# AIBluefisher/DReg-NeRF

Measured on AMD Instinct MI355X. Metric: nerf_pairs_per_sec_regtr_fwd_bwd_128, higher is better.
Workload: dtype bf16; 1 GPU; RegTR fwd+bwd+AdamW, shell-R synthetic pairs, 128^3 grids, 4 pairs (8 grids) per GPU per step, random-init weights; global_batch_pairs=4, resolution=128, fpn_head=active-set (identical results; rows around occupied voxels), parallelism=dp1

## Files before the change

### dreg_nerf_amd/csrc/executor.hip

```cpp
#include <hip/hip_runtime.h>
#include <cstdint>
#include <cstring>
#include <algorithm>
#include <vector>
#include <string>
#include <cstdio>
#include "../../include/dreg_nerf.h"
#ifndef DREG_ELAUNCH
#define DREG_ELAUNCH (-2)
#endif

namespace {

enum { OP_CONV = 0, OP_BN = 1, OP_MAXPOOL = 2, OP_CONV_ROWS = 3 };
constexpr int OP_INTS = 16;
constexpr int TENSOR_INTS = 5;
constexpr int RL = 8;
constexpr int PARAM_I64 = 5;

struct Tensor { int B, D, H, W, C; size_t bytes, off, goff; };
struct Param {
    float* val; float* grad; int d0, d1, ksz;
    size_t pk_fwd = SIZE_MAX, pk_dgrad = SIZE_MAX, pk_cls = SIZE_MAX;
    size_t pk_halo_fwd = SIZE_MAX, pk_halo_dgrad = SIZE_MAX;
    size_t pk_brick_fwd = SIZE_MAX, pk_brick_dgrad = SIZE_MAX;
    int cin_pad = 0;
};
struct Op {
    int kind, in, out, in2, w, b, p2, p3, p4, ksz, stride, pad, relu, add_same, rows_out, rows_in;
    size_t aux0 = 0, aux1 = 0;
    size_t wg_off = 0, wg_bytes = 0;
    int rd = -1;
    int ds_rows = -1;
    int sparse_gx = 0;
    size_t cl_off = 0;
    int cl_count = 0;
    int ds_sparse = 0;
    size_t cl2_off = 0;
    int cl2_count = 0;
    int pool = -1;
    int sstem = 0;
    int sstem_conv = -1, sstem_lat = -1;
    size_t xam_off = 0, pmask_off = 0;
    int halo = 0;
    int stats_bn = -1;
    size_t stats_off = 0;
    int stats_conv = -1;
    int grp = 0;
    int fold_sk_fwd = 0, fold_sk_bwd = 0;
    int fold_into = -1, res_from = -1;
    int bt = -1;
    size_t keep_var = 0, keep_sums = 0;
};
struct HaloPack { const float* w; size_t off; int Cout, Cin, transposed, brick; };
struct PackRec { const float* w; void* out; int Cout, Cin_real, inner, ntaps, for_dgrad, Kpad, dtype, row0; };
static_assert(sizeof(PackRec) == 48, "matches PackDesc of conv.hip");

struct ReduceRec { const float* part; float* dw; int nsplit, Cout, Kpad, ntaps, Cin, Cin_real, accumulate, block0; };
static_assert(sizeof(ReduceRec) == 48, "matches WgradReduceDesc of conv.hip");

struct BnTailRec { const float* a; const float* b; float* o0; float* o1; int B, V, C, block0; };
static_assert(sizeof(BnTailRec) == 48, "matches BnTailDesc of fpn_ops.hip");

struct TimedLaunch { hipEvent_t e0, e1; int op, kind, variant; };

struct Exec {
    std::vector<Tensor> t;
    std::vector<Op> ops;
    std::vector<Param> prm;
    std::vector<char> needs_grad;
    size_t act_bytes = 0, arena_bytes = 0, pack_bytes = 0;
    size_t off_bn_ws = 0, off_coef = 0, off_ks = 0, off_rd = 0, off_cs = 0, off_tmp = 0;
    size_t sz_ks = 0;
    std::vector<ReduceRec> reduce;
    const void* sparse_arena = nullptr;
    std::vector<ReduceRec> reduce_abs;
    int reduce_blocks = 0;
    const void* reduce_arena = nullptr;
    std::vector<BnTailRec> bn_fwd, bn_bwd;
    size_t off_bnf = 0, off_bnb = 0;
    int bn_blocks = 0;
    std::vector<PackRec> packs;
    std::vector<HaloPack> halo_packs;
    int pack_rows = 0, pack_max_floats = 0;
    int out_slot = -1;
    bool timing = false;
    std::vector<TimedLaunch> timed;
    size_t timed_used = 0;
    hipStream_t aux = nullptr;
    std::vector<hipEvent_t> ev;
    hipEvent_t ev_done = nullptr;
    bool use_aux = true;
    const uint8_t* in_rowocc = nullptr;
    char* pack_base = nullptr;
    std::vector<char> written;
    bool aux_used = false;
    struct GrpLaunch { size_t off; int n, variant, blocks; };
    std::vector<int> grp_ops;
    std::vector<GrpLaunch> grp_launch;
    size_t off_grp = 0;
    bool grp_ready = false;
    int pend_sk_bn = -1, pend_sk_n = 0;
    size_t pend_sk_slice = 0;
    const void* fwd_rows_arena = nullptr;
    struct Band { size_t off; const char* tag; int idx; };
    std::vector<Band> bands;
    size_t off_guard_tab = 0, off_guard_res = 0;
    const void* guard_arena = nullptr;
    int guard_op = -1, guard_pass = 0; long long guard_band = -1;
    dreg_exec_opts opt;
};

inline size_t align256(size_t v) { return (v + 255) / 256 * 256; }
constexpr size_t GUARD_BYTES = 64 * 1024;
struct Bump {
    size_t v = 0;
    std::vector<Exec::Band>* bands = nullptr;
    const char* tag = "?"; int idx = -1;
    operator size_t() const { return v; }
    Bump& operator+=(size_t n) { v += n; if (bands && n) { bands->push_back(Exec::Band{v, tag, idx}); v += GUARD_BYTES; } return *this; }
    void name(const char* t, int i) { tag = t; idx = i; }
};
inline int out_dim(int i, int k, int s, int p) { return (i + 2 * p - k) / s + 1; }

struct Scope {
    Exec* e; hipStream_t st; TimedLaunch* tl = nullptr;
    Scope(Exec* ex, hipStream_t s, int op, int kind) : e(ex), st(s) {
        if (!e->timing) return;
        if (e->timed_used == e->timed.size()) {
            TimedLaunch n{}; n.op = op; n.kind = kind;
            if (hipEventCreate(&n.e0) != hipSuccess || hipEventCreate(&n.e1) != hipSuccess) return;
            e->timed.push_back(n);
        }
        tl = &e->timed[e->timed_used++];
        tl->op = op; tl->kind = kind; tl->variant = 0;
        (void)hipEventRecord(tl->e0, st);
    }
    ~Scope() { if (tl) (void)hipEventRecord(tl->e1, st); }
    void variant(int v) { if (tl) tl->variant = v; }
};

#define CK(expr) do { int rc_ = (expr); if (rc_) return rc_; } while (0)

bool s2_class_ok(const Param& p, int ksz, int stride, int pad)
{
    return stride == 2 && ((ksz == 3 && pad == 1) || (ksz == 1 && pad == 0)) && p.d0 % 64 == 0 && p.d1 % 64 == 0 && dreg_conv_get_glds();
}

}

extern "C" {

void dreg_exec_default_opts(dreg_exec_opts* o)
{
    std::memset(o, 0, sizeof(*o));
    o->sparse_grads = 1; o->bn_batch_tails = 1; o->fuse_stem = 1; o->sparse_stem = 1; o->fold_res_bn = 1; o->fold_splitk = 1;
    o->group_wgrad = 1; o->s2_accumulate = 1; o->fuse_bn_stats = 1; o->brick = 1; o->defer_head_pg = 0;
}
void* dreg_exec_create(const int* tensors, int nt, const int* ops, int nops, const int64_t* params, int np)
{
    return dreg_exec_create_opts(tensors, nt, ops, nops, params, np, nullptr);
}
void* dreg_exec_create_opts(const int* tensors, int nt, const int* ops, int nops, const int64_t* params, int np, const dreg_exec_opts* opts)
{
    Exec* e = new Exec();
    if (opts) e->opt = *opts; else dreg_exec_default_opts(&e->opt);
    e->opt.brick &= 3;
    const int g_sparse_grads = e->opt.sparse_grads, g_bn_batch_tails = e->opt.bn_batch_tails, g_fuse_stem = e->opt.fuse_stem, g_sparse_stem = e->opt.sparse_stem,
              g_fold_res_bn = e->opt.fold_res_bn, g_fold_splitk = e->opt.fold_splitk, g_group_wgrad = e->opt.group_wgrad, g_fuse_bn_stats = e->opt.fuse_bn_stats,
              g_brick = e->opt.brick;
    e->t.resize(nt);
    for (int i = 0; i < nt; ++i) {
        Tensor& t = e->t[i];
        t.B = tensors[i * TENSOR_INTS]; t.D = tensors[i * TENSOR_INTS + 1]; t.H = tensors[i * TENSOR_INTS + 2];
        t.W = tensors[i * TENSOR_INTS + 3]; t.C = tensors[i * TENSOR_INTS + 4];
        t.bytes = align256((size_t)t.B * t.D * t.H * t.W * t.C * 2);
    }
    e->prm.resize(np);
    for (int i = 0; i < np; ++i) {
        Param& p = e->prm[i];
        p.val = (float*)params[i * PARAM_I64]; p.grad = (float*)params[i * PARAM_I64 + 1];
        p.d0 = (int)params[i * PARAM_I64 + 2]; p.d1 = (int)params[i * PARAM_I64 + 3]; p.ksz = (int)params[i * PARAM_I64 + 4];
    }
    e->ops.resize(nops);
    for (int i = 0; i < nops; ++i) {
        const int* r = ops + i * OP_INTS;
        Op& o = e->ops[i];
        o.kind = r[0]; o.in = r[1]; o.out = r[2]; o.in2 = r[3]; o.w = r[4]; o.b = r[5]; o.p2 = r[6]; o.p3 = r[7]; o.p4 = r[8];
        o.ksz = r[9]; o.stride = r[10]; o.pad = r[11]; o.relu = r[12]; o.add_same = r[13]; o.rows_out = r[14]; o.rows_in = r[15];
        if (o.in < 0 || o.in >= nt || o.out <= 0 || o.out >= nt || o.in2 >= nt) { delete e; return nullptr; }
    }
    e->out_slot = nops ? e->ops.back().out : -1;

    e->needs_grad.assign(nt, 0);
    for (const Op& o : e->ops) {
        bool g = e->needs_grad[o.in] || (o.in2 >= 0 && e->needs_grad[o.in2]);
        if (o.kind == OP_CONV || o.kind == OP_CONV_ROWS) g = g || e->prm[o.w].grad || (o.b >= 0 && e->prm[o.b].grad);
        if (o.kind == OP_BN) g = g || e->prm[o.w].grad || e->prm[o.b].grad;
        e->needs_grad[o.out] = g;
    }

    for (size_t i = 0; i + 1 < e->ops.size(); ++i) {
        Op& o = e->ops[i];
        if (o.kind != OP_BN || o.in2 >= 0 || o.out == e->out_slot) continue;
        int users = 0, pool = -1;
        for (size_t j = 0; j < e->ops.size(); ++j) {
            const Op& q = e->ops[j];
            if (q.in == o.out || q.in2 == o.out) { ++users; if (q.kind == OP_MAXPOOL && q.in == o.out && j > i) pool = (int)j; }
        }
        if (users == 1 && pool >= 0 && e->t[o.out].C % 8 == 0 && g_fuse_stem) { o.pool = pool; e->ops[pool].pool = (int)i; }
        if (o.pool < 0 && pool >= 0 && o.relu && e->t[o.out].C % 8 == 0 && g_sparse_stem && g_fuse_stem) {
            int prod = -1, writers = 0, lat = -1, others = 0;
            for (size_t j = 0; j < e->ops.size(); ++j) {
                const Op& q = e->ops[j];
                if (q.out == o.in) { prod = (int)j; ++writers; }
                if ((int)j == pool) continue;
                if (q.in2 == o.out) ++others;
                else if (q.in == o.out) { if (q.kind == OP_CONV_ROWS && q.rows_in >= 0 && lat < 0) lat = (int)j; else ++others; }
            }
            if (writers == 1 && others == 0 && e->ops[prod].kind == OP_CONV && e->ops[prod].rows_out >= 0 && o.b >= 0) {
                o.pool = pool; e->ops[pool].pool = (int)i; o.sstem = 1; o.sstem_conv = prod; o.sstem_lat = lat;
            }
        }
    }

    if (g_fold_res_bn)
        for (size_t j = 0; j < e->ops.size(); ++j) {
            Op& bj = e->ops[j];
            const Tensor& xj = e->t[bj.in];
            if (bj.kind != OP_BN || bj.in2 >= 0 || bj.relu || bj.pool >= 0 || bj.out == e->out_slot || dreg_bn_small(xj.B, xj.D * xj.H * xj.W, xj.C, 0)) continue;
            int users = 0, k = -1;
            for (size_t q = 0; q < e->ops.size(); ++q) {
                const Op& o = e->ops[q];
                if (o.in == bj.out) ++users;
                if (o.in2 == bj.out) { ++users; if (o.kind == OP_BN && q > j && o.pool < 0) k = (int)q; }
            }
            if (users != 1 || k < 0 || e->ops[k].res_from >= 0) continue;
            bj.fold_into = k; e->ops[k].res_from = (int)j;
        }

    if (g_fold_splitk)
        for (size_t i = 0; i < e->ops.size(); ++i) {
            Op& o = e->ops[i];
            if (o.kind != OP_CONV || o.b >= 0 || o.in2 >= 0 || o.relu || o.rows_out >= 0) continue;
            auto users = [&](int slot) { int u = 0; for (const Op& q : e->ops) u += (q.in == slot) + (q.in2 == slot); return u; };
            const Tensor& y = e->t[o.out];
            if (i + 1 < e->ops.size() && o.out != e->out_slot) {
                const Op& bn = e->ops[i + 1];
                if (bn.kind == OP_BN && bn.in == o.out && bn.pool < 0 && users(o.out) == 1 && dreg_bn_small_in_regs(y.B, y.D * y.H * y.W, y.C, 0)) o.fold_sk_fwd = 1;
            }
            const Tensor& x = e->t[o.in];
            if (i >= 1 && o.in != 0) {
                const Op& bn = e->ops[i - 1];
                if (bn.kind == OP_BN && bn.out == o.in && bn.pool < 0 && users(o.in) == 1 && dreg_bn_small_in_regs(x.B, x.D * x.H * x.W, x.C, 0) && o.stride == 1) o.fold_sk_bwd = 1;
            }
        }

    Bump off;
    if (e->opt.guard) { off.bands = &e->bands; off.name("arena start", 0); off += 256; }
    for (int i = 1; i < nt; ++i) { off.name("activation", i); e->t[i].off = off; off += e->t[i].bytes; }
    size_t max_tensor = 0, bn_ws = 0, coef = 0, cs = 0;
    for (Op& o : e->ops) {
        const Tensor& x = e->t[o.in];
        off.name(o.kind == OP_BN ? "BatchNorm statistics / stem scratch of op" : (o.kind == OP_MAXPOOL ? "max-pool argmax of op" : "conv op"), (int)(&o - e->ops.data()));
        if (o.kind == OP_BN) {
            const size_t sb = align256((size_t)x.B * x.C * 2 * sizeof(float));
            o.aux0 = off; off += sb; o.aux1 = off; off += sb;
            const size_t V = (size_t)x.D * x.H * x.W;
            size_t w = (size_t)x.B * dreg_bn_num_chunks((int)V) * x.C * 2 * sizeof(float);
            if (o.sstem) {
                const Tensor& p = e->t[e->ops[o.pool].out];
                const size_t w2 = dreg_sparse_stem_workspace_floats(p.B, p.D, p.H, p.W, p.C) * sizeof(float);
                if (w2 > w) w = w2;
                o.xam_off = off; off += align256((size_t)p.B * p.D * p.H * p.W * p.C * 2);
                o.pmask_off = off; off += align256((size_t)p.B * p.D * p.H * p.W);
            }
            if (w > bn_ws) bn_ws = w;
            if (sb > coef) coef = sb;
            bool shared = false;
            for (const Op& q : e->ops) shared = shared || (&q != &o && q.kind == OP_BN && (q.w == o.w || q.b == o.b || q.p2 == o.p2 || q.p3 == o.p3));
            if (g_bn_batch_tails && o.pool < 0 && !shared && dreg_bn_small(x.B, (int)V, x.C, 0)) {
                o.keep_var = off; off += align256((size_t)x.B * x.C * sizeof(float));
                o.keep_sums = off; off += sb;
                BnTailRec f{}, b{};
                f.a = (const float*)o.aux1; f.b = (const float*)o.keep_var; f.o0 = e->prm[o.p2].val; f.o1 = e->prm[o.p3].val;
                b.a = (const float*)o.keep_sums; b.b = nullptr; b.o0 = e->prm[o.w].grad; b.o1 = e->prm[o.b].grad;
                f.B = b.B = x.B; f.V = b.V = (int)V; f.C = b.C = x.C; f.block0 = b.block0 = e->bn_blocks;
                e->bn_blocks += (x.C + 255) / 256;
                o.bt = (int)e->bn_fwd.size();
                e->bn_fwd.push_back(f); e->bn_bwd.push_back(b);
            }
        } else if (o.kind == OP_MAXPOOL) {
            const Tensor& y = e->t[o.out];
            o.aux0 = off; off += align256((size_t)y.B * y.D * y.H * y.W * y.C);
        } else {
            const Param& w = e->prm[o.w];
            const Tensor& y = e->t[o.out];
            const size_t k1 = dreg_conv3d_igemm_workspace_bytes(x.B, x.D, x.H, x.W, x.C, y.D, y.H, y.W, w.d0, o.ksz, o.stride, o.pad, 0, o.in2 >= 0, 0);
            const size_t k2 = dreg_conv3d_igemm_workspace_bytes(x.B, y.D, y.H, y.W, w.d0, x.D, x.H, x.W, w.d1, o.ksz, o.stride, o.pad, 1, 0, 0);
            if (k1 > e->sz_ks) e->sz_ks = k1;
            if (k2 > e->sz_ks) e->sz_ks = k2;
            if (w.grad) {
                o.wg_bytes = dreg_conv3d_wgrad_workspace_bytes(x.B, y.D, y.H, y.W, x.C, w.d0, o.ksz, 0);
                bool shared = false;
                for (const ReduceRec& q : e->reduce) shared = shared || q.dw == w.grad;
                if (shared) o.rd = -2;
                else {
                    ReduceRec r{};
                    r.dw = w.grad; r.nsplit = dreg_conv3d_wgrad_splits(x.B, y.D, y.H, y.W, x.C, w.d0, o.ksz, 0);
                    r.Cout = w.d0; r.Kpad = dreg_conv3d_kpad(o.ksz, x.C, 0); r.ntaps = o.ksz * o.ksz * o.ksz; r.Cin = x.C; r.Cin_real = w.d1;
                    r.accumulate = (o.kind == OP_CONV_ROWS || o.rows_out >= 0) ? 3 : 1;
                    r.block0 = e->reduce_blocks;
                    e->reduce_blocks += dreg_wgrad_reduce_blocks(w.d0, w.d1, o.ksz, r.nsplit);
                    o.rd = (int)e->reduce.size();
                    e->reduce.push_back(r);
                }
            }
            const size_t c = dreg_colsum_workspace_bytes((size_t)y.B * y.D * y.H * y.W, w.d0);
            if (c > cs) cs = c;
        }
    }
    if (g_fuse_bn_stats) {
        for (size_t j = 0; j < e->ops.size(); ++j) {
            Op& bn = e->ops[j];
            if (bn.kind != OP_BN || bn.pool >= 0) continue;
            const Tensor& x = e->t[bn.in];
            const int V = x.D * x.H * x.W;
            if (V % 128 != 0 || dreg_bn_small(x.B, V, x.C, 0)) continue;
            int prod = -1, writers = 0;
            for (size_t i = 0; i < j; ++i) if (e->ops[i].out == bn.in) { prod = (int)i; ++writers; }
            if (writers != 1 || e->ops[prod].kind != OP_CONV || e->ops[prod].stats_bn >= 0) continue;
            {
                const Op& pc = e->ops[prod];
                const Tensor& px = e->t[pc.in];
                const Param& pp = e->prm[pc.w];
                if (!pc.relu && pp.d1 == px.C && pp.d0 != 64 && dreg_conv3_halo_use(px.B, px.D, px.H, px.W, px.C, pp.d0, pc.ksz, pc.stride, pc.pad)) continue;
            }
            e->ops[prod].stats_bn = (int)j;
            bn.stats_conv = prod;
            off.name("epilogue chunk sums of BatchNorm op", (int)j);
            bn.stats_off = off; off += align256((size_t)x.B * (V / 128) * x.C * 2 * sizeof(float));
        }
    }
    e->act_bytes = off;
    for (int i = 1; i < nt; ++i) {
        if (e->t[i].bytes > max_tensor) max_tensor = e->t[i].bytes;
        off.name("gradient of activation", i);
        if (e->needs_grad[i] && i != e->out_slot) { e->t[i].goff = off; off += e->t[i].bytes; } else e->t[i].goff = SIZE_MAX;
    }
    for (Op& o : e->ops) {
        if (o.kind != OP_CONV_ROWS || o.in2 < 0 || o.add_same || !e->needs_grad[o.in2] || !g_sparse_grads) continue;
        for (const Op& q : e->ops) if (q.out == o.in2 && q.kind == OP_CONV_ROWS) o.ds_rows = q.rows_out;
    }
    for (Op& o : e->ops) {
        if (o.kind != OP_CONV_ROWS || !e->needs_grad[o.in] || o.in == 0 || e->t[o.in].goff == SIZE_MAX) continue;
        int writers = 0;
        for (const Op& q : e->ops) {
            if (q.kind == OP_MAXPOOL && q.pool >= 0 && e->ops[q.pool].sstem) continue;
            if ((q.in == o.in || q.in2 == o.in) && e->needs_grad[q.out]) ++writers;
        }
        if (writers != 1 || !g_sparse_grads) continue;
        const Tensor& x = e->t[o.in];
        off.name("row-list copy (sparse_gx) of op", (int)(&o - e->ops.data()));
        o.sparse_gx = 1; o.cl_off = off; off += align256((size_t)x.B * x.D * x.H * x.W * sizeof(int));
    }
    for (Op& o : e->ops) {
        if (o.kind != OP_CONV_ROWS || o.ds_rows < 0 || e->t[o.in2].goff == SIZE_MAX || !g_sparse_grads) continue;
        int writers = 0;
        for (const Op& q : e->ops) if ((q.in == o.in2 || q.in2 == o.in2) && e->needs_grad[q.out]) ++writers;
        if (writers != 1) continue;
        const Tensor& ta = e->t[o.in2];
        off.name("row-list copy (ds_sparse) of op", (int)(&o - e->ops.data()));
        o.ds_sparse = 1; o.cl2_off = off; off += align256((size_t)ta.B * ta.D * ta.H * ta.W * sizeof(int));
    }
    for (Op& o : e->ops) {
        if (o.kind != OP_CONV || o.rows_out < 0) continue;
        const Tensor& y = e->t[o.out];
        off.name("row-list copy (stem output) of op", (int)(&o - e->ops.data()));
        o.cl_off = off; off += align256((size_t)y.B * y.D * y.H * y.W * sizeof(int));
    }
    off.name("BatchNorm workspace", 0);
    e->off_bn_ws = off; off += align256(bn_ws);
    off.name("BatchNorm coefficients", 0);
    e->off_coef = off; off += align256(coef);
    off.name("split-K workspace", 0);
    e->off_ks = off; off += align256(e->sz_ks);
    for (Op& o : e->ops) if (o.rd != -1) { off.name("weight-gradient partials of op", (int)(&o - e->ops.data())); o.wg_off = off; off += align256(o.wg_bytes); if (o.rd >= 0) e->reduce[o.rd].part = (const float*)o.wg_off; }
    if (g_group_wgrad)
        for (size_t i = 0; i < e->ops.size(); ++i) {
            Op& o = e->ops[i];
            const Tensor& y = e->t[o.out];
            if (o.kind != OP_CONV || o.rd < 0 || o.rows_out >= 0 || o.in == 0 || o.b >= 0 || o.out == e->out_slot || !e->prm[o.w].grad) continue;
            if ((long)y.D * y.H * y.W > 4096) continue;
            o.grp = 1; e->grp_ops.push_back((int)i);
        }
    if (e->grp_ops.size() < 4) { for (int i : e->grp_ops) e->ops[i].grp = 0; e->grp_ops.clear(); }
    off.name("descriptor tables", 0);
    e->off_grp = off; off += align256(e->grp_ops.size() * (size_t)dreg_wgrad_group_desc_bytes() + 16);
    e->off_rd = off; off += align256(e->reduce.size() * sizeof(ReduceRec) + 16);
    e->off_bnf = off; off += align256(e->bn_fwd.size() * sizeof(BnTailRec) + 16);
    e->off_bnb = off; off += align256(e->bn_bwd.size() * sizeof(BnTailRec) + 16);
    off.name("column-sum workspace", 0);
    e->off_cs = off; off += align256(cs);
    off.name("gradient temporary", 0);
    e->off_tmp = off; off += max_tensor;
    if (e->opt.guard) {
        off.bands = nullptr;
        e->off_guard_tab = off; off += align256((e->bands.size() + 1) * sizeof(unsigned long long));
        e->off_guard_res = off; off += 256;
    }
    e->arena_bytes = off + 256;

    size_t poff = 0;
    auto add_pack = [&](Param& p, int kind, int cin_pad) {
        PackRec r{};
        const int ntaps = p.ksz * p.ksz * p.ksz;
        r.w = p.val; r.Cout = p.d0; r.Cin_real = p.d1; r.ntaps = ntaps; r.for_dgrad = kind; r.dtype = 0; r.row0 = e->pack_rows;
        int rows;
        if (kind == 0) { r.inner = cin_pad; r.Kpad = dreg_conv3d_kpad(p.ksz, cin_pad, 0); rows = p.d0; }
        else if (kind == 1) { r.inner = p.d0; r.Kpad = dreg_conv3d_kpad(p.ksz, p.d0, 0); rows = p.d1; }
        else { r.inner = p.d0; r.Kpad = dreg_conv3d_kpad(p.ksz == 1 ? 1 : 2, p.d0, 0); rows = (p.ksz == 1 ? 1 : 8) * p.d1; }
        r.out = (void*)poff;
        const size_t o = poff;
        poff += align256((size_t)rows * r.Kpad * 2);
        e->pack_rows += rows;
        const int ch = kind ? p.d0 : p.d1;
        const int fl = ntaps > 1 ? (ch < 64 ? ch : 64) * ntaps : 0;
        if (fl > e->pack_max_floats) e->pack_max_floats = fl;
        e->packs.push_back(r);
        return o;
    };
    auto add_halo_pack = [&](Param& p, int transposed) {
        HaloPack hp{p.val, poff, p.d0, p.d1, transposed, 0};
        poff += align256(dreg_conv3_halo_pack_bytes_n(transposed ? p.d0 : p.d1, transposed ? p.d1 : p.d0));
        e->halo_packs.push_back(hp);
        return hp.off;
    };
    auto add_brick_pack = [&](Param& p, int transposed) {
        HaloPack hp{p.val, poff, p.d0, p.d1, transposed, 1};
        poff += align256(dreg_conv3_brick_pack_bytes(transposed ? p.d1 : p.d0, transposed ? p.d0 : p.d1));
        e->halo_packs.push_back(hp);
        return hp.off;
    };
    for (Op& o : e->ops) {
        if (o.kind != OP_CONV && o.kind != OP_CONV_ROWS) continue;
        Param& p = e->prm[o.w];
        const Tensor& x = e->t[o.in];
        const Tensor& y = e->t[o.out];
        if (o.kind == OP_CONV && !o.relu) {
            if (dreg_conv3_halo_use(x.B, x.D, x.H, x.W, x.C, p.d0, o.ksz, o.stride, o.pad) && p.d1 == x.C) o.halo |= 1;
            if (e->needs_grad[o.in] && dreg_conv3_halo_use(y.B, y.D, y.H, y.W, p.d0, p.d1, o.ksz, o.stride, o.pad) && p.d0 % 32 == 0) o.halo |= 2;
        }
        if (o.kind == OP_CONV_ROWS && o.ksz == 3 && o.pad == 1 && p.d1 == x.C && dreg_brick_supported(x.B, x.D, x.H, x.W, 16, 256)) {
            auto on = [&](int nout) { return (nout == 64 && (g_brick & 1)) || (nout == 256 && (g_brick & 2)); };
            if (on(p.d0) && p.d1 % 16 == 0 && p.pk_brick_fwd == SIZE_MAX) p.pk_brick_fwd = add_brick_pack(p, 0);
            if (e->needs_grad[o.in] && on(p.d1) && p.d0 % 16 == 0 && p.pk_brick_dgrad == SIZE_MAX) p.pk_brick_dgrad = add_brick_pack(p, 1);
        }
        if (o.halo & 1) { if (p.pk_halo_fwd == SIZE_MAX) p.pk_halo_fwd = add_halo_pack(p, 0); }
        else if (p.pk_fwd == SIZE_MAX) { p.cin_pad = x.C; p.pk_fwd = add_pack(p, 0, x.C); }
        if (e->needs_grad[o.in]) {
            if (o.halo & 2) { if (p.pk_halo_dgrad == SIZE_MAX) p.pk_halo_dgrad = add_halo_pack(p, 1); }
            else if (o.kind == OP_CONV && s2_class_ok(p, o.ksz, o.stride, o.pad)) { if (p.pk_cls == SIZE_MAX) p.pk_cls = add_pack(p, 2, x.C); }
            else if (p.pk_dgrad == SIZE_MAX) p.pk_dgrad = add_pack(p, 1, x.C);
        }
    }
    e->pack_bytes = poff + 256;
    return e;
}

void dreg_exec_destroy(void* h)
{
    Exec* e = (Exec*)h;
    if (!e) return;
    for (auto& t : e->timed) { (void)hipEventDestroy(t.e0); (void)hipEventDestroy(t.e1); }
    for (auto& v : e->ev) if (v) (void)hipEventDestroy(v);
    if (e->ev_done) (void)hipEventDestroy(e->ev_done);
    delete e;
}

size_t dreg_exec_arena_bytes(void* h) { return ((Exec*)h)->arena_bytes; }
size_t dreg_exec_pack_bytes(void* h) { return ((Exec*)h)->pack_bytes; }
int dreg_exec_num_packs(void* h) { return (int)((Exec*)h)->packs.size(); }
size_t dreg_exec_tensor_offset(void* h, int slot) { return ((Exec*)h)->t[slot].off; }
int dreg_exec_output_slot(void* h) { return ((Exec*)h)->out_slot; }

int dreg_exec_pack_rows(void* h) { return ((Exec*)h)->pack_rows; }
int dreg_exec_export_pack_table(void* h, void* host_out, int* host_row_desc, void* pack_base)
{
    Exec* e = (Exec*)h;
    e->pack_base = (char*)pack_base;
    PackRec* o = (PackRec*)host_out;
    for (size_t i = 0; i < e->packs.size(); ++i) {
        o[i] = e->packs[i]; o[i].out = (char*)pack_base + (size_t)e->packs[i].out;
        const int end = i + 1 < e->packs.size() ? e->packs[i + 1].row0 : e->pack_rows;
        for (int r = e->packs[i].row0; r < end; ++r) host_row_desc[r] = (int)i;
    }
    return DREG_OK;
}
int dreg_exec_repack(void* h, const void* descs_dev, const int* row_desc_dev, void* stream)
{
    Exec* e = (Exec*)h;
    CK(dreg_pack_conv_weights_batched(descs_dev, (int)e->packs.size(), e->pack_rows, e->pack_max_floats, row_desc_dev, stream));
    for (const HaloPack& hp : e->halo_packs) {
        if (hp.brick) CK(dreg_pack_conv_weight_brick(hp.w, e->pack_base + hp.off, hp.Cout, hp.Cin, hp.transposed, stream));
        else CK(dreg_pack_conv_weight_halo(hp.w, e->pack_base + hp.off, hp.Cout, hp.Cin, hp.transposed, stream));
    }
    return DREG_OK;
}
int dreg_exec_op_halo(void* h, int op) { Exec* e = (Exec*)h; return op >= 0 && op < (int)e->ops.size() ? e->ops[op].halo : 0; }

void dreg_exec_set_overlap(void* h, int enable) { ((Exec*)h)->use_aux = enable != 0; }
void dreg_exec_set_input_row_occupancy(void* h, const uint8_t* rowocc) { ((Exec*)h)->in_rowocc = rowocc; }
void dreg_exec_set_timing(void* h, int enable) { ((Exec*)h)->timing = enable != 0; }
int dreg_exec_read_timings(void* h, int* op_kind, float* ms, int max)
{
    Exec* e = (Exec*)h;
    int n = 0;
    for (size_t i = 0; i < e->timed_used && n < max; ++i) {
        float v = 0.f;
        if (hipEventElapsedTime(&v, e->timed[i].e0, e->timed[i].e1) != hipSuccess) continue;
        op_kind[3 * n] = e->timed[i].op; op_kind[3 * n + 1] = e->timed[i].kind; op_kind[3 * n + 2] = e->timed[i].variant; ms[n] = v; ++n;
    }
    e->timed_used = 0;
    return n;
}

static int guard_setup(Exec* e, char* A, hipStream_t st)
{
    if (!e->opt.guard || e->guard_arena == (const void*)A) return DREG_OK;
    std::vector<unsigned long long> offs(e->bands.size());
    for (size_t i = 0; i < offs.size(); ++i) offs[i] = e->bands[i].off;
    if (!offs.empty() && hipMemcpyAsync(A + e->off_guard_tab, offs.data(), offs.size() * sizeof(unsigned long long), hipMemcpyHostToDevice, st) != hipSuccess) return DREG_ELAUNCH;
    if (hipStreamSynchronize(st) != hipSuccess) return DREG_ELAUNCH;
    int rc = dreg_guard_fill(A, A + e->off_guard_tab, (int)offs.size(), (int)GUARD_BYTES, (void*)st);
    if (rc) return rc;
    e->guard_arena = A;
    return DREG_OK;
}
static int guard_scan(Exec* e, char* A, long long* out4, hipStream_t st)
{
    int rc = dreg_guard_scan(A, A + e->off_guard_tab, (int)e->bands.size(), (int)GUARD_BYTES, A + e->off_guard_res, (void*)st);
    if (rc) return rc;
    if (hipMemcpyAsync(out4, A + e->off_guard_res, 4 * sizeof(long long), hipMemcpyDeviceToHost, st) != hipSuccess) return DREG_ELAUNCH;
    if (hipStreamSynchronize(st) != hipSuccess) return DREG_ELAUNCH;
    return DREG_OK;
}
static int guard_after_op(Exec* e, char* A, int op, int pass, hipStream_t st, hipStream_t aux)
{
    if (e->opt.guard < 2) return DREG_OK;
    if (aux && hipStreamSynchronize(aux) != hipSuccess) return DREG_ELAUNCH;
    long long r[4];
    int rc = guard_scan(e, A, r, st);
    if (rc) return rc;
    if (r[0] > 0) { e->guard_op = op; e->guard_pass = pass; e->guard_band = r[1]; return DREG_EGUARD; }
    return DREG_OK;
}
static int upload_tables(Exec* e, char* A, hipStream_t st)
{
    { int rc = guard_setup(e, A, st); if (rc) return rc; }
    if (e->reduce_arena == (const void*)A) return DREG_OK;
    e->reduce_abs = e->reduce;
    for (ReduceRec& r : e->reduce_abs) r.part = (const float*)(A + (size_t)r.part);
    std::vector<BnTailRec> f = e->bn_fwd, b = e->bn_bwd;
    for (BnTailRec& r : f) { r.a = (const float*)(A + (size_t)r.a); r.b = (const float*)(A + (size_t)r.b); }
    for (BnTailRec& r : b) r.a = (const float*)(A + (size_t)r.a);
    if (!e->reduce_abs.empty() && hipMemcpyAsync(A + e->off_rd, e->reduce_abs.data(), e->reduce_abs.size() * sizeof(ReduceRec), hipMemcpyHostToDevice, st) != hipSuccess) return DREG_ELAUNCH;
    if (!f.empty() && (hipMemcpyAsync(A + e->off_bnf, f.data(), f.size() * sizeof(BnTailRec), hipMemcpyHostToDevice, st) != hipSuccess ||
                       hipMemcpyAsync(A + e->off_bnb, b.data(), b.size() * sizeof(BnTailRec), hipMemcpyHostToDevice, st) != hipSuccess)) return DREG_ELAUNCH;
    const int gd = dreg_wgrad_group_desc_bytes();
    struct Rec { std::vector<char> d; int variant, nblocks, op; };
    std::vector<Rec> recs;
    e->grp_launch.clear(); e->grp_ready = false;
    bool all_ok = !e->grp_ops.empty();
    for (int i : e->grp_ops) {
        const Op& o = e->ops[i];
        const Tensor& x = e->t[o.in];
        const Tensor& y = e->t[o.out];
        const Param& w = e->prm[o.w];
        Rec r; r.d.resize(gd); r.op = i;
        if (e->t[o.out].goff == SIZE_MAX ||
            dreg_conv3d_wgrad_group_fill(r.d.data(), A + y.goff, A + x.off, A + o.wg_off, o.wg_bytes, x.B, x.D, x.H, x.W, x.C, y.D, y.H, y.W, w.d0,
                                         o.ksz, o.stride, o.pad, &r.variant, &r.nblocks) != DREG_OK || w.d1 != x.C) { all_ok = false; break; }
        recs.push_back(std::move(r));
    }
    std::vector<char> gtab;
    if (all_ok) {
        std::stable_sort(recs.begin(), recs.end(), [](const Rec& a, const Rec& b) { return a.variant < b.variant; });
        gtab.resize(recs.size() * (size_t)gd);
        for (size_t k = 0; k < recs.size(); ++k) {
            if (e->grp_launch.empty() || e->grp_launch.back().variant != recs[k].variant) e->grp_launch.push_back(Exec::GrpLaunch{e->off_grp + k * (size_t)gd, 0, recs[k].variant, 0});
            const int b0 = e->grp_launch.back().blocks;
            std::memcpy(recs[k].d.data() + gd - (int)sizeof(int), &b0, sizeof(int));
            std::memcpy(gtab.data() + k * (size_t)gd, recs[k].d.data(), (size_t)gd);
            e->grp_launch.back().n += 1; e->grp_launch.back().blocks += recs[k].nblocks;
        }
        if (hipMemcpyAsync(A + e->off_grp, gtab.data(), gtab.size(), hipMemcpyHostToDevice, st) != hipSuccess) return DREG_ELAUNCH;
        e->grp_ready = true;
    }
    if (hipStreamSynchronize(st) != hipSuccess) return DREG_ELAUNCH;
    e->reduce_arena = A;
    return DREG_OK;
}
static int flush_bn_tails(Exec* e, char* A, std::vector<char>& done, int what, hipStream_t st)
{
    for (int lo = 0, nrec = (int)done.size(); lo < nrec;) {
        if (!done[lo]) { ++lo; continue; }
        int hi = lo;
        while (hi + 1 < nrec && done[hi + 1]) ++hi;
        Scope sc(e, st, -1, 4 + what);
        const int b0 = e->bn_fwd[lo].block0;
        const int b1 = hi + 1 < nrec ? e->bn_fwd[hi + 1].block0 : e->bn_blocks;
        if (what == 0) CK(dreg_bn_running_update_batched((const BnTailRec*)(A + e->off_bnf) + lo, hi - lo + 1, b0, b1 - b0, 0.1f, (void*)st));
        else CK(dreg_bn_param_grad_batched((const BnTailRec*)(A + e->off_bnb) + lo, hi - lo + 1, b0, b1 - b0, 1, (void*)st));
        for (int q = lo; q <= hi; ++q) done[q] = 0;
        lo = hi + 1;
    }
    return DREG_OK;
}

int dreg_exec_forward(void* h, void* arena, size_t arena_bytes, const void* pack_base, const void* x_in,
                      const int64_t* rowlists, int nlists, int train, void* stream)
{
    Exec* e = (Exec*)h;
    if (arena_bytes < e->arena_bytes) return DREG_EINVAL;
    char* A = (char*)arena;
    const char* PK = (const char*)pack_base;
    hipStream_t st = (hipStream_t)stream;
    CK(upload_tables(e, (char*)arena, st));
    std::vector<char> bn_done(e->bn_fwd.size(), 0);
    std::vector<int> sums_rpc(e->ops.size(), 0);
    int fwd_sk_bn = -1, fwd_sk_n = 0;
    size_t fwd_sk_slice = 0;
    struct ArenaMark { Exec* e; const void* a; bool ok = false;
                       ~ArenaMark() { if (ok) e->fwd_rows_arena = a; else { e->fwd_rows_arena = nullptr; for (Op& o : e->ops) if (o.kind == OP_CONV && o.rows_out >= 0) o.cl_count = 0; } } } arena_mark{e, arena};
    auto act = [&](int s) -> void* { return s == 0 ? (void*)x_in : (void*)(A + e->t[s].off); };
    for (size_t i = 0; i < e->ops.size(); ++i) {
        if (i > 0) CK(guard_after_op(e, A, (int)i - 1, 0, st, nullptr));
        const Op& o = e->ops[i];
        const Tensor& x = e->t[o.in];
        const Tensor& y = e->t[o.out];
        if (o.kind == OP_CONV) {
            const Param& w = e->prm[o.w];
            const float* bias = o.b >= 0 ? e->prm[o.b].val : nullptr;
            const void* add = o.in2 >= 0 ? act(o.in2) : nullptr;
            const Tensor* ta = o.in2 >= 0 ? &e->t[o.in2] : nullptr;
            if (o.rows_out >= 0) {
                if (o.rows_out >= nlists || bias || add) return DREG_EINVAL;
                const int64_t* rl = rowlists + RL * o.rows_out;
                const int* r = (const int*)rl[0];
                const int n = (int)rl[1];
                Op& om = const_cast<Op&>(o);
                if (e->fwd_rows_arena != arena) CK(dreg_fill_zero(act(o.out), y.bytes, stream));
                else if (om.cl_count > 0) CK(dreg_zero_rows(act(o.out), (const int*)(A + o.cl_off), om.cl_count, y.C, 0, stream));
                if (n > 0 && hipMemcpyAsync(A + o.cl_off, r, (size_t)n * sizeof(int), hipMemcpyDeviceToDevice, st) != hipSuccess) return DREG_ELAUNCH;
                om.cl_count = n;
                if (n > 0) {
                    Scope sc(e, st, (int)i, 0);
                    CK(dreg_conv3d_igemm_rows(act(o.in), PK + w.pk_fwd, act(o.out), nullptr, nullptr, r, n, x.B, x.D, x.H, x.W, x.C, y.D, y.H, y.W, w.d0,
                                              o.ksz, o.stride, o.pad, 0, o.relu, 0, 0, 0, 0, 0, stream));
                }
                continue;
            }
            Scope sc(e, st, (int)i, 0);
            if (o.halo & 1) {
                if (train && o.stats_bn >= 0)
                    CK(dreg_conv3_halo_n_bnstats(act(o.in), PK + w.pk_halo_fwd, act(o.out), bias, add, x.B, x.D, x.H, x.W, x.C, w.d0, ta ? ta->D : 0, ta ? ta->H : 0,
                                                 ta ? ta->W : 0, o.add_same, (float*)(A + e->ops[o.stats_bn].stats_off), &sums_rpc[o.stats_bn], stream));
                else
                    CK(dreg_conv3_halo_n(act(o.in), PK + w.pk_halo_fwd, act(o.out), bias, add, x.B, x.D, x.H, x.W, x.C, w.d0, ta ? ta->D : 0, ta ? ta->H : 0, ta ? ta->W : 0,
                                         o.add_same, 0, stream));
                continue;
            }
            if (train && o.stats_bn >= 0 && !(o.in == 0 && e->in_rowocc)) {
                CK(dreg_conv3d_igemm_bnstats(act(o.in), PK + w.pk_fwd, act(o.out), bias, add, x.B, x.D, x.H, x.W, x.C, y.D, y.H, y.W, w.d0,
                                             o.ksz, o.stride, o.pad, o.relu, ta ? ta->D : 0, ta ? ta->H : 0, ta ? ta->W : 0, o.add_same,
                                             A + e->off_ks, e->sz_ks, (float*)(A + e->ops[o.stats_bn].stats_off), &sums_rpc[o.stats_bn], stream));
                continue;
            }
            if (train && o.fold_sk_fwd && !(o.halo & 1)) {
                int ns = 0; size_t sl = 0;
                CK(dreg_conv3d_igemm_defer(act(o.in), PK + w.pk_fwd, act(o.out), bias, add, x.B, x.D, x.H, x.W, x.C, y.D, y.H, y.W, w.d0,
                                           o.ksz, o.stride, o.pad, 0, o.relu, ta ? ta->D : 0, ta ? ta->H : 0, ta ? ta->W : 0, o.add_same,
                                           A + e->off_ks, e->sz_ks, o.in == 0 ? e->in_rowocc : nullptr, &ns, &sl, stream));
                if (ns > 0) { fwd_sk_bn = (int)i + 1; fwd_sk_n = ns; fwd_sk_slice = sl; }
                continue;
            }
            CK(dreg_conv3d_igemm_occ(act(o.in), PK + w.pk_fwd, act(o.out), bias, add, x.B, x.D, x.H, x.W, x.C, y.D, y.H, y.W, w.d0,
                                     o.ksz, o.stride, o.pad, 0, o.relu, ta ? ta->D : 0, ta ? ta->H : 0, ta ? ta->W : 0, o.add_same, 0, 0,
                                     A + e->off_ks, e->sz_ks, o.in == 0 ? e->in_rowocc : nullptr, stream));
        } else if (o.kind == OP_CONV_ROWS) {
            const Param& w = e->prm[o.w];
            if (o.rows_out < 0 || o.rows_out >= nlists) return DREG_EINVAL;
            const float* bias = o.b >= 0 ? e->prm[o.b].val : nullptr;
            const void* add = o.in2 >= 0 ? act(o.in2) : nullptr;
            const Tensor* ta = o.in2 >= 0 ? &e->t[o.in2] : nullptr;
            Scope sc(e, st, (int)i, 0);
            const int64_t* rl = rowlists + RL * o.rows_out;
            if ((e->opt.brick & (w.d0 == 64 ? 1 : 2)) && w.pk_brick_fwd != SIZE_MAX && rl[2] && rl[3] > 0) {
                sc.variant(2);
                CK(dreg_conv3_brick(act(o.in), PK + w.pk_brick_fwd, act(o.out), bias, add, (const void*)rl[2], (int)rl[3], (const int*)rl[4], (const void*)rl[5],
                                    (const int*)rl[6], x.B, x.D, x.H, x.W, x.C, w.d0, ta ? ta->D : 0, ta ? ta->H : 0, ta ? ta->W : 0, 0, 0, stream));
                continue;
            }
            CK(dreg_conv3d_igemm_rows(act(o.in), PK + w.pk_fwd, act(o.out), bias, add, (const int*)rl[0], (int)rl[1],
                                      x.B, x.D, x.H, x.W, x.C, y.D, y.H, y.W, w.d0, o.ksz, 1, o.pad, 0, 0, ta ? ta->D : 0, ta ? ta->H : 0, ta ? ta->W : 0,
                                      0, 0, stream));
        } else if (o.kind == OP_BN && o.pool >= 0 && o.sstem) {
            const Op& q = e->ops[o.pool];
            const Tensor& p = e->t[q.out];
            const Op& cv = e->ops[o.sstem_conv];
            if (cv.rows_out >= nlists) return DREG_EINVAL;
            const int64_t* rl = rowlists + RL * cv.rows_out;
            const int* ra = nullptr; int na = 0;
            if (o.sstem_lat >= 0) {
                const int li = e->ops[o.sstem_lat].rows_in;
                if (li < 0 || li >= nlists) return DREG_EINVAL;
                ra = (const int*)rowlists[RL * li]; na = (int)rowlists[RL * li + 1];
            }
            CK(dreg_sparse_stem_fwd(act(o.in), (const int*)rl[0], (int)rl[1], ra, na, act(o.out), act(q.out), (uint8_t*)(A + q.aux0), A + o.xam_off, (uint8_t*)(A + o.pmask_off),
                                    e->prm[o.w].val, e->prm[o.b].val, e->prm[o.p2].val, e->prm[o.p3].val, (float*)(A + o.aux0), (float*)(A + o.aux1),
                                    (float*)(A + e->off_bn_ws), x.B, x.D, x.H, x.W, p.D, p.H, p.W, x.C, 1e-5f, 0.1f, train, o.relu, stream));
        } else if (o.kind == OP_BN && o.pool >= 0) {
            const Op& q = e->ops[o.pool];
            const Tensor& p = e->t[q.out];
            CK(dreg_bn_relu_maxpool_fwd(act(o.in), act(q.out), (uint8_t*)(A + q.aux0), e->prm[o.w].val, e->prm[o.b].val, e->prm[o.p2].val, e->prm[o.p3].val,
                                        (float*)(A + o.aux0), (float*)(A + o.aux1), (float*)(A + e->off_bn_ws), x.B, x.D, x.H, x.W, p.D, p.H, p.W, x.C,
                                        1e-5f, 0.1f, train, o.relu, stream));
        } else if (o.kind == OP_MAXPOOL && o.pool >= 0) {
        } else if (o.kind == OP_BN) {
            const int V = x.D * x.H * x.W;
            const void* res_p = o.in2 >= 0 ? act(o.in2) : nullptr;
            void* out_p = o.fold_into >= 0 ? nullptr : act(o.out);
            dreg_bn_extra ex{};
            if (o.res_from >= 0) { res_p = act(e->ops[o.res_from].in); ex.res_scale_shift = (const float*)(A + e->ops[o.res_from].aux0); }
            if (train && sums_rpc[i] > 0) {
                CK(dreg_bn3d_fwd_ex(act(o.in), res_p, out_p, e->prm[o.w].val, e->prm[o.b].val, e->prm[o.p2].val, e->prm[o.p3].val,
                                    (float*)(A + o.aux0), (float*)(A + o.aux1), (float*)(A + o.stats_off), x.B, V, x.C, 1e-5f, 0.1f, 1, o.relu, 0,
                                    nullptr, nullptr, sums_rpc[i], &ex, stream));
                continue;
            }
            int deferred = 0;
            if (fwd_sk_bn == (int)i) { ex.splitk_part = (const float*)(A + e->off_ks); ex.splitk_nsplit = fwd_sk_n; ex.splitk_slice = fwd_sk_slice; fwd_sk_bn = -1; }
            CK(dreg_bn3d_fwd_ex(act(o.in), res_p, out_p, e->prm[o.w].val, e->prm[o.b].val, e->prm[o.p2].val, e->prm[o.p3].val,
                                (float*)(A + o.aux0), (float*)(A + o.aux1), (float*)(A + e->off_bn_ws), x.B, V, x.C, 1e-5f, 0.1f, train, o.relu, 0,
                                o.bt >= 0 ? (float*)(A + o.keep_var) : nullptr, &deferred, 0, &ex, stream));
            if (deferred) bn_done[o.bt] = 1;
        } else if (o.kind == OP_MAXPOOL) {
            CK(dreg_maxpool3d_fwd(act(o.in), act(o.out), (uint8_t*)(A + o.aux0), x.B, x.D, x.H, x.W, y.D, y.H, y.W, x.C, 0, stream));
        } else return DREG_EINVAL;
    }
    CK(guard_after_op(e, A, (int)e->ops.size() - 1, 0, st, nullptr));
    CK(flush_bn_tails(e, A, bn_done, 0, st));
    CK(guard_after_op(e, A, (int)e->ops.size(), 0, st, nullptr));
    arena_mark.ok = true;
    return DREG_OK;
}
int dreg_exec_guard_bands(void* h) { return (int)((Exec*)h)->bands.size(); }
int dreg_exec_guard_check(void* h, void* arena, long long* out4, void* stream)
{
    Exec* e = (Exec*)h;
    if (!e->opt.guard || !out4) return DREG_EINVAL;
    if (e->guard_arena != arena) { out4[0] = 0; out4[1] = (long long)e->bands.size(); out4[2] = 0; out4[3] = 0; return DREG_OK; }
    return guard_scan(e, (char*)arena, out4, (hipStream_t)stream);
}
int dreg_exec_guard_describe(void* h, int band, char* buf, int buf_bytes)
{
    Exec* e = (Exec*)h;
    if (band < 0 || band >= (int)e->bands.size() || !buf || buf_bytes <= 0) return DREG_EINVAL;
    const Exec::Band& b = e->bands[band];
    std::snprintf(buf, (size_t)buf_bytes, "band %d at arena offset %zu, behind: %s %d", band, b.off, b.tag, b.idx);
    return DREG_OK;
}
int dreg_exec_guard_last(void* h, int* op, int* pass, long long* band)
{
    Exec* e = (Exec*)h;
    if (op) *op = e->guard_op;
    if (pass) *pass = e->guard_pass;
    if (band) *band = e->guard_band;
    return DREG_OK;
}

int dreg_exec_backward_range(void* h, void* arena, size_t arena_bytes, const void* pack_base, const void* x_in, const void* grad_out,
                             const int64_t* rowlists, int nlists, void* stream, void* aux_stream, int op_begin, int op_end, int flags);
int dreg_exec_backward(void* h, void* arena, size_t arena_bytes, const void* pack_base, const void* x_in, const void* grad_out,
                       const int64_t* rowlists, int nlists, void* stream, void* aux_stream)
{
    return dreg_exec_backward_range(h, arena, arena_bytes, pack_base, x_in, grad_out, rowlists, nlists, stream, aux_stream,
                                    0, (int)((Exec*)h)->ops.size(), 3);
}
int dreg_exec_backward_range(void* h, void* arena, size_t arena_bytes, const void* pack_base, const void* x_in, const void* grad_out,
                             const int64_t* rowlists, int nlists, void* stream, void* aux_stream, int op_begin, int op_end, int flags)
{
    Exec* e = (Exec*)h;
    if (arena_bytes < e->arena_bytes || op_begin < 0 || op_end > (int)e->ops.size() || op_begin > op_end) return DREG_EINVAL;
    char* A = (char*)arena;
    const char* PK = (const char*)pack_base;
    hipStream_t st = (hipStream_t)stream;
    auto act = [&](int s) -> void* { return s == 0 ? (void*)x_in : (void*)(A + e->t[s].off); };
    if (flags & 1) { e->written.assign(e->t.size(), 0); e->aux_used = false; e->pend_sk_bn = -1; }
    if (e->written.size() != e->t.size()) return DREG_EINVAL;
    std::vector<char>& written = e->written;
    auto grad = [&](int s) -> void* { return s == e->out_slot ? (void*)grad_out : (void*)(A + e->t[s].goff); };
    auto dst_for = [&](int s) -> void* { return written[s] ? (void*)(A + e->off_tmp) : grad(s); };
    auto commit = [&](int s) -> int {
        if (written[s]) {
            const Tensor& t = e->t[s];
            return dreg_add_inplace(grad(s), A + e->off_tmp, (size_t)t.B * t.D * t.H * t.W * t.C, 0, stream);
        }
        written[s] = 1;
        return DREG_OK;
    };
    written[e->out_slot] = 1;
    bool aux_on = e->use_aux && aux_stream != nullptr && aux_stream != stream;
    e->aux = (hipStream_t)aux_stream;
    if (aux_on && e->ev.empty()) {
        e->ev.assign(e->ops.size(), nullptr);
        if (hipEventCreateWithFlags(&e->ev_done, hipEventDisableTiming) != hipSuccess) aux_on = false;
    }
    bool& aux_used = e->aux_used;
    CK(upload_tables(e, A, st));
    std::vector<char> bn_done(e->bn_bwd.size(), 0);
    if (flags & 1) {
        const bool fresh = e->sparse_arena != arena;
        for (Op& o : e->ops) {
            if (!o.sparse_gx) continue;
            const Tensor& x = e->t[o.in];
            if (fresh) { if (hipMemsetAsync(A + x.goff, 0, (size_t)x.B * x.D * x.H * x.W * x.C * 2, st) != hipSuccess) return DREG_ELAUNCH; }
            else if (o.cl_count > 0) CK(dreg_zero_rows(A + x.goff, (const int*)(A + o.cl_off), o.cl_count, x.C, 0, stream));
            o.cl_count = 0;
        }
        for (Op& o : e->ops) {
            if (!o.ds_sparse) continue;
            const Tensor& ta = e->t[o.in2];
            if (fresh) { if (hipMemsetAsync(A + ta.goff, 0, (size_t)ta.B * ta.D * ta.H * ta.W * ta.C * 2, st) != hipSuccess) return DREG_ELAUNCH; }
            else if (o.cl2_count > 0) CK(dreg_zero_rows(A + ta.goff, (const int*)(A + o.cl2_off), o.cl2_count, ta.C, 0, stream));
            o.cl2_count = 0;
        }
        e->sparse_arena = arena;
    }
    const int g_s2_accumulate = e->opt.s2_accumulate, g_group_wgrad = e->opt.group_wgrad, g_brick = e->opt.brick, g_defer_head_pg = e->opt.defer_head_pg;
    std::vector<char> rd_done(e->reduce.size(), 0);
    hipStream_t rd_stream = st;
    size_t rd_pending = 0;
    auto flush_reduce = [&]() -> int {
        for (int lo = 0, nrec = (int)rd_done.size(); lo < nrec;) {
            if (!rd_done[lo]) { ++lo; continue; }
            int hi = lo;
            while (hi + 1 < nrec && rd_done[hi + 1]) ++hi;
            Scope sc(e, rd_stream, -1, 3);
            const int b0 = e->reduce[lo].block0;
            const int b1 = hi + 1 < nrec ? e->reduce[hi + 1].block0 : e->reduce_blocks;
            CK(dreg_wgrad_reduce_batched((const ReduceRec*)(A + e->off_rd) + lo, hi - lo + 1, b0, b1 - b0, (void*)rd_stream));
            for (int q = lo; q <= hi; ++q) rd_done[q] = 0;
            lo = hi + 1;
        }
        return DREG_OK;
    };
    const bool grp_active = g_group_wgrad && e->grp_ready && aux_on && !e->timing && op_begin == 0 && op_end == (int)e->ops.size() && (flags & 3) == 3;
    std::vector<int> grp_seen;
    auto param_grads = [&](int i, bool event_recorded) -> int {
        const Op& o = e->ops[i];
        const Tensor& x = e->t[o.in];
        const Tensor& y = e->t[o.out];
        const Param& w = e->prm[o.w];
        const void* gy = grad(o.out);
        const bool rows = o.kind == OP_CONV_ROWS;
        const bool lrows = rows || (o.kind == OP_CONV && o.rows_out >= 0 && o.rows_out < nlists);
        const int* r_out = lrows ? (const int*)rowlists[RL * o.rows_out] : nullptr;
        const int n_out = lrows ? (int)rowlists[RL * o.rows_out + 1] : 0;
        hipStream_t ws = st;
        if (aux_on && !(grp_active && o.grp && !(o.b >= 0 && e->prm[o.b].grad))) {
            if (!e->ev[i] && hipEventCreateWithFlags(&e->ev[i], hipEventDisableTiming) != hipSuccess) return DREG_ELAUNCH;
            if (!event_recorded && hipEventRecord(e->ev[i], st) != hipSuccess) return DREG_ELAUNCH;
            if (hipStreamWaitEvent(e->aux, e->ev[i], 0) != hipSuccess) return DREG_ELAUNCH;
            ws = e->aux;
            aux_used = true;
        }
        hipStream_t bs = ws;
        bool flush_now = false;
        if (w.grad && grp_active && o.grp) {
            grp_seen.push_back(i);
        } else
        if (w.grad) {
            Scope sc(e, ws, i, 2);
            if (o.rd >= 0) {
                CK(dreg_conv3d_wgrad_partials(gy, act(o.in), A + o.wg_off, o.wg_bytes, lrows ? r_out : nullptr, n_out, x.B, x.D, x.H, x.W, x.C, w.d1,
                                              y.D, y.H, y.W, w.d0, o.ksz, rows ? 1 : o.stride, o.pad, (!lrows && o.in == 0) ? e->in_rowocc : nullptr, (void*)ws));
                rd_done[o.rd] = 1;
                rd_stream = ws;
                rd_pending += o.wg_bytes;
                flush_now = rd_pending >= ((size_t)192 << 20);
            } else if (lrows) {
                CK(dreg_conv3d_wgrad_rows(gy, act(o.in), w.grad, A + o.wg_off, o.wg_bytes, r_out, n_out, x.B, x.D, x.H, x.W, x.C, w.d1,
                                          y.D, y.H, y.W, w.d0, o.ksz, rows ? 1 : o.stride, o.pad, 1, (void*)ws));
            } else {
                CK(dreg_conv3d_wgrad_occ(gy, act(o.in), w.grad, A + o.wg_off, o.wg_bytes, x.B, x.D, x.H, x.W, x.C, w.d1, y.D, y.H, y.W, w.d0,
                                         o.ksz, o.stride, o.pad, 1, 0, 1, o.in == 0 ? e->in_rowocc : nullptr, (void*)ws));
            }
        }
        if (flush_now) { CK(flush_reduce()); rd_pending = 0; }
        if (o.b >= 0 && e->prm[o.b].grad) {
            if (rows) CK(dreg_colsum_rows(gy, r_out, n_out, e->prm[o.b].grad, (float*)(A + e->off_cs), w.d0, 1, 0, (void*)bs));
            else CK(dreg_colsum(gy, e->prm[o.b].grad, (float*)(A + e->off_cs), (size_t)y.B * y.D * y.H * y.W, w.d0, 1, 0, (void*)bs));
        }
        return DREG_OK;
    };
    auto flush_group = [&](int ev_op) -> int {
        if (grp_seen.empty()) return DREG_OK;
        if (!e->ev[ev_op] && hipEventCreateWithFlags(&e->ev[ev_op], hipEventDisableTiming) != hipSuccess) return DREG_ELAUNCH;
        if (hipEventRecord(e->ev[ev_op], st) != hipSuccess || hipStreamWaitEvent(e->aux, e->ev[ev_op], 0) != hipSuccess) return DREG_ELAUNCH;
        aux_used = true;
        if (grp_seen.size() == e->grp_ops.size()) {
            for (const Exec::GrpLaunch& q : e->grp_launch) CK(dreg_wgrad_group_launch(A + q.off, q.n, q.variant, q.blocks, (void*)e->aux));
        } else {
            for (int j : grp_seen) {
                const Op& oj = e->ops[j]; const Tensor& xj = e->t[oj.in]; const Tensor& yj = e->t[oj.out]; const Param& wj = e->prm[oj.w];
                CK(dreg_conv3d_wgrad_partials(grad(oj.out), act(oj.in), A + oj.wg_off, oj.wg_bytes, nullptr, 0, xj.B, xj.D, xj.H, xj.W, xj.C, wj.d1,
                                              yj.D, yj.H, yj.W, wj.d0, oj.ksz, oj.stride, oj.pad, nullptr, (void*)e->aux));
            }
        }
        for (int j : grp_seen) { rd_done[e->ops[j].rd] = 1; rd_pending += e->ops[j].wg_bytes; }
        rd_stream = e->aux;
        grp_seen.clear();
        return DREG_OK;
    };
    std::vector<int> deferred_pg;
    bool deep_reached = false;
    auto run_deferred = [&]() -> int {
        for (int j : deferred_pg) CK(param_grads(j, true));
        deferred_pg.clear();
        return DREG_OK;
    };
    for (int i = op_end - 1; i >= op_begin; --i) {
        if (i < op_end - 1) CK(guard_after_op(e, A, i + 1, 1, st, aux_on ? e->aux : nullptr));
        const Op& o = e->ops[i];
        const Tensor& x = e->t[o.in];
        const Tensor& y = e->t[o.out];
        if (o.kind == OP_MAXPOOL && o.pool >= 0) continue;
        if (o.kind == OP_BN && o.pool >= 0) {
            const Op& q = e->ops[o.pool];
            const Tensor& p = e->t[q.out];
            if (!e->needs_grad[q.out] || !written[q.out]) continue;
            if (!e->prm[o.w].grad || !e->prm[o.b].grad) return DREG_EINVAL;
            if (o.sstem) {
                const Op& cv = e->ops[o.sstem_conv];
                if (cv.rows_out >= nlists) return DREG_EINVAL;
                const int64_t* rl = rowlists + RL * cv.rows_out;
                const int* ra = nullptr; int na = 0;
                const bool lat = o.sstem_lat >= 0 && written[o.out];
                if (lat) { const int li = e->ops[o.sstem_lat].rows_in; ra = (const int*)rowlists[RL * li]; na = (int)rowlists[RL * li + 1]; }
                CK(dreg_sparse_stem_bwd(act(o.in), grad(q.out), (const uint8_t*)(A + q.aux0), A + o.xam_off, lat ? grad(o.out) : nullptr, ra, na,
                                        (const int*)rl[0], (int)rl[1], (float*)(A + o.aux0), (float*)(A + o.aux1), dst_for(o.in), e->prm[o.w].grad, e->prm[o.b].grad,
                                        (float*)(A + e->off_coef), (float*)(A + e->off_bn_ws), x.B, x.D, x.H, x.W, p.D, p.H, p.W, x.C, o.relu, 1, stream));
                CK(commit(o.in));
                continue;
            }
            CK(dreg_bn_relu_maxpool_bwd(act(o.in), grad(q.out), (const uint8_t*)(A + q.aux0), (float*)(A + o.aux0), (float*)(A + o.aux1), dst_for(o.in),
                                        e->prm[o.w].grad, e->prm[o.b].grad, (float*)(A + e->off_coef), (float*)(A + e->off_bn_ws),
                                        x.B, x.D, x.H, x.W, p.D, p.H, p.W, x.C, o.relu, 1, stream));
            CK(commit(o.in));
            continue;
        }
        if (!e->needs_grad[o.out] || !written[o.out]) continue;
        const void* gy = grad(o.out);
        if (o.kind == OP_CONV || o.kind == OP_CONV_ROWS) {
            const Param& w = e->prm[o.w];
            const bool rows = o.kind == OP_CONV_ROWS;
            const int* r_out = rows ? (const int*)rowlists[RL * o.rows_out] : nullptr;
            const int n_out = rows ? (int)rowlists[RL * o.rows_out + 1] : 0;
            const bool pg = w.grad || (o.b >= 0 && e->prm[o.b].grad);
            const long vox_out = (long)y.D * y.H * y.W;
            if (pg && aux_on && g_defer_head_pg && !deep_reached && vox_out >= 32768) {
                if (!e->ev[i] && hipEventCreateWithFlags(&e->ev[i], hipEventDisableTiming) != hipSuccess) return DREG_ELAUNCH;
                if (hipEventRecord(e->ev[i], st) != hipSuccess) return DREG_ELAUNCH;
                deferred_pg.push_back(i);
            } else if (pg) {
                if (vox_out <= 512 && !deep_reached) { deep_reached = true; CK(run_deferred()); }
                CK(param_grads(i, false));
                if (grp_active && !e->grp_ops.empty() && i == e->grp_ops.front()) CK(flush_group(i));
            }
            if (o.in2 >= 0 && e->needs_grad[o.in2]) {
                const Tensor& ta = e->t[o.in2];
                if (o.add_same) { CK(hipMemcpyAsync(dst_for(o.in2), gy, (size_t)y.B * y.D * y.H * y.W * y.C * 2, hipMemcpyDeviceToDevice, st) == hipSuccess ? 0 : DREG_ELAUNCH); }
                else if (rows && o.ds_rows >= 0 && o.ds_rows < nlists) {
                    void* dst = dst_for(o.in2);
                    const int nds = (int)rowlists[RL * o.ds_rows + 1];
                    if (o.ds_sparse && dst == grad(o.in2)) {
                        if (nds > 0 && hipMemcpyAsync(A + o.cl2_off, (const int*)rowlists[RL * o.ds_rows], (size_t)nds * sizeof(int), hipMemcpyDeviceToDevice, st) != hipSuccess) return DREG_ELAUNCH;
                        const_cast<Op&>(o).cl2_count = nds;
                    } else
                    CK(dreg_fill_zero(dst, (size_t)ta.B * ta.D * ta.H * ta.W * ta.C * 2, stream));
                    CK(dreg_downsample_sum_rows(gy, dst, (const int*)rowlists[RL * o.ds_rows], (int)rowlists[RL * o.ds_rows + 1],
                                                y.D, y.H, y.W, ta.D, ta.H, ta.W, y.C, 0, stream));
                }
                else CK(dreg_downsample_sum(gy, dst_for(o.in2), y.B, y.D, y.H, y.W, ta.D, ta.H, ta.W, y.C, 0, stream));
                CK(commit(o.in2));
            }
            bool fused_add = false;
            if (e->needs_grad[o.in]) {
                const bool halo_d = (o.halo & 2) != 0;
                const bool s2_cls = w.pk_cls != SIZE_MAX && s2_class_ok(w, o.ksz, o.stride, o.pad);
                fused_add = written[o.in] && !rows && (halo_d || (s2_cls && g_s2_accumulate) || (!s2_cls && w.pk_dgrad != SIZE_MAX));
                void* gx = fused_add ? grad(o.in) : dst_for(o.in);
                Scope sc(e, st, i, 1);
                if (halo_d) {
                    CK(dreg_conv3_halo_n(gy, PK + w.pk_halo_dgrad, gx, nullptr, fused_add ? gx : nullptr, y.B, y.D, y.H, y.W, w.d0, w.d1,
                                         fused_add ? x.D : 0, fused_add ? x.H : 0, fused_add ? x.W : 0, 1, 0, stream));
                } else if (fused_add && s2_cls) {
                    CK(dreg_conv3d_dgrad_s2_acc(gy, PK + w.pk_cls, gx, x.B, x.D, x.H, x.W, x.C, y.D, y.H, y.W, w.d0, o.ksz, o.pad, stream));
                } else if (fused_add) {
                    sc.variant(1);
                    CK(dreg_conv3d_igemm_ws(gy, PK + w.pk_dgrad, gx, nullptr, gx, x.B, y.D, y.H, y.W, w.d0, x.D, x.H, x.W, w.d1,
                                            o.ksz, o.stride, o.pad, 1, 0, x.D, x.H, x.W, 1, 0, 0, A + e->off_ks, e->sz_ks, stream));
                } else if (rows) {
                    if (o.rows_in < 0 || o.rows_in >= nlists) return DREG_EINVAL;
                    const int64_t* rl = rowlists + RL * o.rows_in;
                    const int* r_in = (const int*)rl[0];
                    const int n_in = (int)rl[1];
                    if (o.sparse_gx && gx == grad(o.in)) {
                        if (n_in > 0 && hipMemcpyAsync(A + o.cl_off, r_in, (size_t)n_in * sizeof(int), hipMemcpyDeviceToDevice, st) != hipSuccess) return DREG_ELAUNCH;
                        const_cast<Op&>(o).cl_count = n_in;
                    } else CK(dreg_fill_zero(gx, (size_t)x.B * x.D * x.H * x.W * x.C * 2, stream));
                    if ((g_brick & (w.d1 == 64 ? 1 : 2)) && w.pk_brick_dgrad != SIZE_MAX && rl[2] && rl[3] > 0) {
                        sc.variant(2);
                        CK(dreg_conv3_brick(gy, PK + w.pk_brick_dgrad, gx, nullptr, nullptr, (const void*)rl[2], (int)rl[3], (const int*)rl[4], (const void*)rl[5],
                                            (const int*)rl[6], x.B, x.D, x.H, x.W, w.d0, w.d1, 0, 0, 0, 0, 0, stream));
                    } else
                        CK(dreg_conv3d_igemm_rows(gy, PK + w.pk_dgrad, gx, nullptr, nullptr, r_in, n_in,
                                                  x.B, y.D, y.H, y.W, w.d0, x.D, x.H, x.W, x.C, o.ksz, 1, o.pad, 1, 0, 0, 0, 0, 0, 0, stream));
                } else if (w.pk_cls != SIZE_MAX && s2_class_ok(w, o.ksz, o.stride, o.pad)) {
                    CK(dreg_conv3d_dgrad_s2(gy, PK + w.pk_cls, gx, x.B, x.D, x.H, x.W, x.C, y.D, y.H, y.W, w.d0, o.ksz, o.pad, stream));
                } else {
                    if (w.pk_dgrad == SIZE_MAX) return DREG_EINVAL;
                    if (o.fold_sk_bwd && gx == grad(o.in) && i - 1 >= 0) {
                        int ns = 0; size_t sl = 0;
                        CK(dreg_conv3d_igemm_defer(gy, PK + w.pk_dgrad, gx, nullptr, nullptr, x.B, y.D, y.H, y.W, w.d0, x.D, x.H, x.W, w.d1,
                                                   o.ksz, o.stride, o.pad, 1, 0, 0, 0, 0, 0, A + e->off_ks, e->sz_ks, nullptr, &ns, &sl, stream));
                        if (ns > 0) { e->pend_sk_bn = i - 1; e->pend_sk_n = ns; e->pend_sk_slice = sl; }
                    } else
                    CK(dreg_conv3d_igemm_ws(gy, PK + w.pk_dgrad, gx, nullptr, nullptr, x.B, y.D, y.H, y.W, w.d0, x.D, x.H, x.W, w.d1,
                                            o.ksz, o.stride, o.pad, 1, 0, 0, 0, 0, 0, 0, 0, A + e->off_ks, e->sz_ks, stream));
                }
            }
            if (e->needs_grad[o.in] && !fused_add) CK(commit(o.in));
        } else if (o.kind == OP_BN) {
            const int V = x.D * x.H * x.W;
            const bool res_g = o.in2 >= 0 && e->needs_grad[o.in2];
            void* dx = dst_for(o.in);
            void* dres = nullptr;
            bool res_via_copy = false;
            if (res_g) {
                if (!written[o.in2]) dres = grad(o.in2);
                else if (dx != (void*)(A + e->off_tmp)) dres = A + e->off_tmp;
                else res_via_copy = true;
            }
            if (!e->prm[o.w].grad || !e->prm[o.b].grad) return DREG_EINVAL;
            int deferred = 0;
            if (res_via_copy) {
                CK(dreg_bn3d_bwd_defer_params(act(o.in), gy, act(o.out), (float*)(A + o.aux0), (float*)(A + o.aux1), dx, nullptr, e->prm[o.w].grad, e->prm[o.b].grad,
                                              (float*)(A + e->off_coef), (float*)(A + e->off_bn_ws), x.B, V, x.C, o.relu, 1, 0,
                                              o.bt >= 0 ? (float*)(A + o.keep_sums) : nullptr, &deferred, stream));
                if (deferred) bn_done[o.bt] = 1;
                CK(commit(o.in));
                if (o.relu) CK(dreg_relu_bwd(act(o.out), gy, A + e->off_tmp, (size_t)x.B * V * x.C, 0, 0, 0, stream));
                else if (hipMemcpyAsync(A + e->off_tmp, gy, (size_t)x.B * V * x.C * 2, hipMemcpyDeviceToDevice, st) != hipSuccess) return DREG_ELAUNCH;
                CK(commit(o.in2));
            } else {
                dreg_bn_extra ex{};
                if (e->pend_sk_bn == i) { ex.splitk_part = (const float*)(A + e->off_ks); ex.splitk_nsplit = e->pend_sk_n; ex.splitk_slice = e->pend_sk_slice; e->pend_sk_bn = -1; }
                CK(dreg_bn3d_bwd_ex(act(o.in), gy, o.in2 >= 0 ? act(o.out) : nullptr, (float*)(A + o.aux0), (float*)(A + o.aux1), dx, dres, e->prm[o.w].grad, e->prm[o.b].grad,
                                    (float*)(A + e->off_coef), (float*)(A + e->off_bn_ws), x.B, V, x.C, o.relu, 1, 0,
                                    o.bt >= 0 ? (float*)(A + o.keep_sums) : nullptr, &deferred, &ex, stream));
                if (deferred) bn_done[o.bt] = 1;
                if (res_g && dres == (void*)(A + e->off_tmp)) { CK(commit(o.in2)); CK(commit(o.in)); }
                else { CK(commit(o.in)); if (res_g) CK(commit(o.in2)); }
            }
        } else if (o.kind == OP_MAXPOOL) {
            if (!e->needs_grad[o.in]) continue;
            CK(dreg_maxpool3d_bwd_acc(gy, (const uint8_t*)(A + o.aux0), grad(o.in), x.B, x.D, x.H, x.W, y.D, y.H, y.W, x.C, written[o.in] ? 1 : 0, 0, stream));
            written[o.in] = 1;
        }
    }
    CK(guard_after_op(e, A, op_begin, 1, st, aux_on ? e->aux : nullptr));
    CK(run_deferred());
    if (!grp_seen.empty()) CK(flush_group(e->grp_ops.front()));
    CK(flush_reduce());
    CK(flush_bn_tails(e, A, bn_done, 1, st));
    CK(guard_after_op(e, A, -1, 1, st, aux_on ? e->aux : nullptr));
    if ((flags & 2) && aux_used) {
        if (hipEventRecord(e->ev_done, e->aux) != hipSuccess || hipStreamWaitEvent(st, e->ev_done, 0) != hipSuccess) return DREG_ELAUNCH;
    }
    return DREG_OK;
}

}
```

### dreg_nerf_amd/lib.py

```python
import ctypes
import os
from ctypes import c_float, c_int, c_size_t, c_void_p

import torch

_HERE = os.path.dirname(os.path.abspath(__file__))
LIB_PATH = os.path.join(_HERE, "libdreg_nerf_hip.so")

DT_BF16 = 0
DT_F32 = 1

_lib = None


class DregError(RuntimeError):
    pass


def _sig(lib, name, restype, argtypes):
    fn = getattr(lib, name)
    fn.restype = restype
    fn.argtypes = argtypes
    return fn


P, I, F, Z = c_void_p, c_int, c_float, c_size_t

SIGNATURES = {
    "dreg_conv3d_igemm": (I, [P, P, P, P, P] + [I] * 18 + [I, I, P]),
    "dreg_conv3d_igemm_workspace_bytes": (Z, [I] * 15),
    "dreg_conv3d_igemm_ws": (I, [P, P, P, P, P] + [I] * 18 + [I, I, P, Z, P]),
    "dreg_conv3d_igemm_occ": (I, [P, P, P, P, P] + [I] * 18 + [I, I, P, Z, P, P]),
    "dreg_conv3d_igemm_bnstats": (I, [P, P, P, P, P] + [I] * 17 + [P, Z, P, P, P]),
    "dreg_conv3d_kpad": (I, [I, I, I]),
    "dreg_gemm_f32_desc_bytes": (I, []),
    "dreg_gemm_f32_batched": (I, [P, I, I, P, P]),
    "dreg_infonce_wsym": (I, [P, P, I, P]),
    "dreg_conv3d_igemm_defer": (I, [P, P, P, P, P] + [I] * 18 + [P, Z, P, P, P, P]),
    "dreg_bn3d_fwd_ex": (I, [P] * 10 + [I, I, I, F, F, I, I, I, P, P, I, P, P]),
    "dreg_bn3d_bwd_ex": (I, [P] * 11 + [I] * 6 + [P, P, P, P]),
    "dreg_exec_default_opts": (None, [P]),
    "dreg_exec_guard_bands": (I, [P]),
    "dreg_exec_guard_check": (I, [P, P, P, P]),
    "dreg_exec_guard_describe": (I, [P, I, P, I]),
    "dreg_exec_guard_last": (I, [P, P, P, P]),
    "dreg_guard_fill": (I, [P, P, I, I, P]),
    "dreg_guard_scan": (I, [P, P, I, I, P, P]),
    "dreg_exec_create_opts": (P, [P, I, P, I, P, I, P]),
    "dreg_ps_set_group_wgrad": (None, [P, I]),
    "dreg_conv_get_glds": (I, []),
    "dreg_conv3d_dgrad_s2": (I, [P, P, P] + [I] * 11 + [P]),
    "dreg_conv3d_dgrad_s2_acc": (I, [P, P, P] + [I] * 11 + [P]),
    "dreg_pack_conv_weight": (I, [P, P, I, I, I, I, I, I, P]),
    "dreg_pack_conv_weights_batched": (I, [P, I, I, I, P, P]),
    "dreg_conv3d_wgrad_splits": (I, [I] * 8),
    "dreg_conv3d_wgrad_workspace_bytes": (Z, [I] * 8),
    "dreg_conv3d_wgrad": (I, [P, P, P, P, Z] + [I] * 16 + [P]),
    "dreg_conv3d_wgrad_occ": (I, [P, P, P, P, Z] + [I] * 16 + [P, P]),
    "dreg_conv3d_igemm_rows": (I, [P] * 5 + [P, I] + [I] * 18 + [I, P]),
    "dreg_conv3d_wgrad_rows": (I, [P, P, P, P, Z] + [P, I] + [I] * 14 + [P]),
    "dreg_conv3d_wgrad_partials": (I, [P, P, P, Z, P, I] + [I] * 13 + [P, P]),
    "dreg_wgrad_reduce_blocks": (I, [I, I, I, I]),
    "dreg_wgrad_reduce_batched": (I, [P, I, I, I, P]),
    "dreg_conv3_halo_supported": (I, [I] * 6),
    "dreg_conv3_halo_use": (I, [I] * 9),
    "dreg_conv3_halo_pack_bytes": (Z, [I]),
    "dreg_pack_conv_weight_halo": (I, [P, P, I, I, I, P]),
    "dreg_conv3_halo": (I, [P, P, P, P, P] + [I] * 10 + [P]),
    "dreg_conv3_halo_pack_bytes_n": (Z, [I, I]),
    "dreg_conv3_halo_n": (I, [P, P, P, P, P] + [I] * 11 + [P]),
    "dreg_conv3_halo_n_bnstats": (I, [P, P, P, P, P] + [I] * 10 + [P, P, P]),
    "dreg_conv3d_wgrad_variant": (I, [I] * 10),
    "dreg_conv3d_igemm_variant": (I, [I] * 17),
    "dreg_conv3d_wgrad_group_fill": (I, [P, P, P, P, Z] + [I] * 12 + [P, P]),
    "dreg_bn_small_in_regs": (I, [I, I, I, I]),
    "dreg_wgrad_group_desc_bytes": (I, []),
    "dreg_linear_wgrad_group_fill": (I, [P, P, P, P, Z, I, I, I, P, P]),
    "dreg_wgrad_group_launch": (I, [P, I, I, I, P]),
    "dreg_bn_num_chunks": (I, [I]),
    "dreg_bn_relu_maxpool_fwd": (I, [P] * 10 + [I] * 8 + [F, F, I, I, P]),
    "dreg_bn_relu_maxpool_bwd": (I, [P] * 10 + [I] * 10 + [P]),
    "dreg_sparse_stem_workspace_floats": (Z, [I] * 5),
    "dreg_sparse_stem_fwd": (I, [P, P, I, P, I] + [P] * 12 + [I] * 8 + [F, F, I, I, P]),
    "dreg_sparse_stem_bwd": (I, [P] * 6 + [I, P, I] + [P] * 7 + [I] * 10 + [P]),
    "dreg_bn3d_fwd": (I, [P] * 10 + [I, I, I, F, F, I, I, I, P]),
    "dreg_bn3d_bwd": (I, [P] * 11 + [I, I, I, I, I, I, P]),
    "dreg_bn_small": (I, [I, I, I, I]),
    "dreg_bn3d_fwd_defer_update": (I, [P] * 10 + [I, I, I, F, F, I, I, I, P, P, P]),
    "dreg_bn3d_fwd_from_sums": (I, [P] * 10 + [I, I, I, I, F, F, I, I, P]),
    "dreg_bn3d_bwd_defer_params": (I, [P] * 11 + [I, I, I, I, I, I, P, P, P]),
    "dreg_bn_running_update_batched": (I, [P, I, I, I, F, P]),
    "dreg_bn_param_grad_batched": (I, [P, I, I, I, I, P]),
    "dreg_maxpool3d_fwd": (I, [P, P, P] + [I] * 9 + [P]),
    "dreg_maxpool3d_bwd": (I, [P, P, P] + [I] * 9 + [P]),
    "dreg_maxpool3d_bwd_acc": (I, [P, P, P] + [I] * 10 + [P]),
    "dreg_downsample_sum": (I, [P, P] + [I] * 9 + [P]),
    "dreg_downsample_sum_rows": (I, [P, P, P] + [I] * 9 + [P]),
    "dreg_colsum_workspace_bytes": (Z, [Z, I]),
    "dreg_colsum": (I, [P, P, P, Z, I, I, I, P]),
    "dreg_trilinear_gather_fwd": (I, [P, P, P, P] + [I] * 10 + [P]),
    "dreg_trilinear_gather_bwd": (I, [P, P, P, P] + [I] * 8 + [P]),
    "dreg_cast_from_f32": (I, [P, P, Z, I, P]),
    "dreg_fill_zero": (I, [P, Z, P]),
    "dreg_active_sets_workspace_bytes": (Z, [I] * 4),
    "dreg_active_sets": (I, [P, P] + [I] * 8 + [P, P, P, P, Z, P]),
    "dreg_active_sets_level2_workspace_bytes": (Z, [I] * 4),
    "dreg_active_sets_level2": (I, [P] + [I] * 7 + [P, P, P, Z, P]),
    "dreg_conv_rows_workspace_bytes": (Z, [I, I, I, I]),
    "dreg_conv_rows": (I, [P, P, I, I, I, I, I, I, I, I, I, I, I, P, P, P, Z, P]),
    "dreg_trilinear_gather_bwd_rows": (I, [P, P, P, P, I, P, P, P] + [I] * 10 + [P]),
    "dreg_colsum_rows": (I, [P, P, I, P, P, I, I, I, P]),
    "dreg_trilinear_gather_bwd_gather": (I, [P, P, P, P, I, P, P] + [I] * 10 + [P]),
    "dreg_trilinear_gather_bwd_gather_rows_only": (I, [P, P, P, P, I, P, P] + [I] * 10 + [P]),
    "dreg_trilinear_gather_bwd_gather_seg": (I, [P, P, P, P, P, I, P, P] + [I] * 11 + [P]),
    "dreg_gather_segment_mean": (I, [P, P, P, I, P, P, P, P] + [I] * 9 + [P]),
    "dreg_zero_rows": (I, [P, P, I, I, I, P]),
    "dreg_add_inplace": (I, [P, P, Z, I, P]),
    "dreg_pack_rgba_grids": (I, [P, P, I, I, I, I, I, P]),
    "dreg_pack_rgba_grids_occ": (I, [P, P, P, I, I, I, I, I, P]),
    "dreg_pack_rgba_sparse": (I, [P, P, P, P, I, I, I, I, I, I, P]),
    "dreg_pack_rgba_sparse_occ": (I, [P, P, P, P, P, I, I, I, I, I, I, P]),
    "dreg_conv_row_occupancy": (I, [P, P, I, I, I, I, I, I, I, I, P]),
    "dreg_gather_grid_xyz": (I, [P, P, P, P, I, I, I, I, P]),
    "dreg_exec_create": (P, [P, I, P, I, P, I]),
    "dreg_exec_destroy": (None, [P]),
    "dreg_exec_op_halo": (I, [P, I]),
    "dreg_exec_arena_bytes": (Z, [P]),
    "dreg_exec_pack_bytes": (Z, [P]),
    "dreg_exec_num_packs": (I, [P]),
    "dreg_exec_tensor_offset": (Z, [P, I]),
    "dreg_exec_output_slot": (I, [P]),
    "dreg_exec_pack_rows": (I, [P]),
    "dreg_exec_export_pack_table": (I, [P, P, P, P]),
    "dreg_exec_repack": (I, [P, P, P, P]),
    "dreg_exec_set_overlap": (None, [P, I]),
    "dreg_exec_set_input_row_occupancy": (None, [P, P]),
    "dreg_exec_set_timing": (None, [P, I]),
    "dreg_exec_read_timings": (I, [P, P, P, I]),
    "dreg_exec_forward": (I, [P, P, Z, P, P, P, I, I, P]),
    "dreg_exec_backward": (I, [P, P, Z, P, P, P, P, I, P, P]),
    "dreg_exec_backward_range": (I, [P, P, Z, P, P, P, P, I, P, P, I, I, I]),
    "dreg_mha_fwd": (I, [P] * 5 + [I] * 7 + [F, I, P]),
    "dreg_mha_bwd": (I, [P] * 10 + [I] * 7 + [F, I, P]),
    "dreg_corr_attention_fwd": (I, [P] * 5 + [I] * 3 + [F, I, P]),
    "dreg_corr_attention_bwd": (I, [P] * 9 + [I] * 3 + [F, I, P]),
    "dreg_mha_varlen_fwd": (I, [P] * 6 + [I] * 9 + [F, I, P]),
    "dreg_mha_varlen_bwd": (I, [P] * 11 + [I] * 9 + [F, I, P]),
    "dreg_corr_attention_varlen_fwd": (I, [P] * 6 + [I] * 5 + [F, I, P]),
    "dreg_corr_attention_varlen_bwd": (I, [P] * 10 + [I] * 5 + [F, I, P]),
    "dreg_layernorm_fwd": (I, [P] * 6 + [I, I, F, I, P]),
    "dreg_layernorm_bwd_workspace_bytes": (Z, [I]),
    "dreg_layernorm_bwd": (I, [P] * 8 + [I] * 5 + [P]),
    "dreg_layernorm_bwd_add": (I, [P] * 9 + [I] * 4 + [P]),
    "dreg_layernorm_fwd2": (I, [P, P, P, P, I, P, P, P, I, I, F, P]),
    "dreg_layernorm_bwd_parts": (I, [P] * 10 + [I, I, I, P]),
    "dreg_layernorm_bwd_blocks": (I, [I]),
    "dreg_layernorm_bwd_final_batched": (I, [P, I, P]),
    "dreg_overlap_bwd_acc": (I, [P, P, P, P, P, P, P, P, I, P, I, P]),
    "dreg_colsum_rows_per_chunk": (I, [Z]),
    "dreg_colsum_batched": (I, [P, I, I, I, P]),
    "dreg_brick_supported": (I, [I] * 6),
    "dreg_conv3_brick_pack_bytes": (Z, [I, I]),
    "dreg_pack_conv_weight_brick": (I, [P, P, I, I, I, P]),
    "dreg_brick_tiles_workspace_bytes": (Z, [I] * 4),
    "dreg_brick_tiles_build": (I, [P, I, I, I, I, I, I, P, Z, P, P, P, P, P, P]),
    "dreg_conv3_brick": (I, [P, P, P, P, P, P, I, P, P, P] + [I] * 11 + [P]),
    "dreg_ps_num_params": (I, []),
    "dreg_ps_num_linears": (I, []),
    "dreg_ps_create": (P, [P]),
    "dreg_ps_destroy": (None, [P]),
    "dreg_ps_set_fuse": (None, [P, I]),
    "dreg_ps_set_timing": (None, [P, I]),
    "dreg_ps_read_timings": (I, [P, P, P, I]),
    "dreg_ps_arena_bytes": (Z, [P, I]),
    "dreg_ps_panel_fwd": (I, [P] * 13 + [I, I, I, I, F, P]),
    "dreg_ps_panel_bwd": (I, [P] * 12 + [I, I, I, P]),
    "dreg_ps_forward": (I, [P, P, Z, P, P, P, P, P, P, I, I, I, P, P, P, P]),
    "dreg_ps_backward": (I, [P, P, Z, P, P, P, P, P, P, I, I, I, P, P, P, P, P, P, P, P, P, I]),
    "dreg_posenc_sine": (I, [P, P, I, F, F, P]),
    "dreg_overlap_fwd": (I, [P, P, P, P, I, P]),
    "dreg_overlap_bwd_workspace_bytes": (Z, [I]),
    "dreg_overlap_bwd": (I, [P] * 8 + [I, P]),
    "dreg_relu_bwd": (I, [P, P, P, Z, I, I, I, P]),
    "dreg_weighted_kabsch": (I, [P, P, P, P, I, I, F, P]),
    "dreg_weighted_kabsch_pairs": (I, [P, P, P, P, P, I, I, I, F, P]),
    "dreg_weighted_kabsch_bwd": (I, [P] * 7 + [I, I, F, P]),
    "dreg_weighted_kabsch_pairs_bwd": (I, [P] * 7 + [I, I, I, F, P]),
    "dreg_reg_point_losses": (I, [P] * 10 + [I, I, I, I, F, F, F, P]),
    "dreg_infonce_nn": (I, [P] * 7 + [I, I, F, P]),
    "dreg_infonce_rows": (I, [P] * 10 + [I, I, F, F, I, P]),
    "dreg_reg_losses_final": (I, [P] * 6 + [I, I, F, F, F, F, F, P]),
    "dreg_nerf_cont_deferred": (I, [P] * 5 + [I, I, I, F, F, F, F, P]),
    "dreg_halfspace_labels": (I, [P, P, P, P, I, I, P]),
    "dreg_voxel_downsample_workspace_bytes": (Z, [I]),
    "dreg_voxel_downsample_fwd": (I, [P] * 11 + [Z, I, I, I, F, P]),
    "dreg_voxel_downsample_bwd": (I, [P, P, P, P, I, I, P]),
    "dreg_voxel_downsample_plan": (I, [P] * 11 + [Z, I, I, F, P]),
    "dreg_voxel_downsample_plan_frozen": (I, [P] * 11 + [Z, I, I, F, P, P]),
    "dreg_voxel_segment_mean": (I, [P] * 5 + [I, I, P]),
    "dreg_grad_norm": (I, [P, P, P, Z, P]),
    "dreg_adamw_step": (I, [P] * 5 + [Z] + [F] * 5 + [I, F, P]),
    "dreg_ngp_level_table": (ctypes.c_uint32, [F, I, I, P, P, P, P, P]),
    "dreg_f32_to_f16": (I, [P, P, Z, P]),
    "dreg_ngp_density_fwd": (I, [P] * 6 + [P] * 5 + [P, I, P]),
    "dreg_ngp_rgb_mean_fwd": (I, [P] * 6 + [I, I, P]),
    "dreg_ngp_dir_bias": (I, [P, P, P, I, P]),
    "dreg_ngp_alpha_keep": (I, [P, P, P, I, F, F, P]),
    "dreg_ngp_density_fwd_contract": (I, [P] * 6 + [P] * 5 + [P, I, I, P]),
    "dreg_ngp_density_fwd_ws": (I, [P] * 6 + [P] * 5 + [P, I, I, P, Z, P, I, P]),
    "dreg_grid_sample_points_ordered": (I, [P, P, P, P, P, I, I, I, P, I, P]),
    "dreg_grid_x_order_workspace_bytes": (Z, [I, I, I]),
    "dreg_grid_x_order": (I, [P, P, P, P, Z, I, I, I, I, P]),
    "dreg_grid_occupied_workspace_bytes": (Z, [I, I, I]),
    "dreg_grid_occupied_totals": (P, [P, I, I, I]),
    "dreg_grid_occupied_count": (I, [P, P, Z, I, I, I, P]),
    "dreg_grid_occupied_build": (I, [P, P, P, P, P, P, P, P, I, I, I, I, P]),
    "dreg_ngp_density_keep_fwd_ws": (I, [P] * 6 + [P] * 5 + [P, I, I, P, Z, P, I] + [P, P, F, F, P]),
    "dreg_grid_write_kept": (I, [P, P, P, P, P, P, P, P, I, I, I, I, P]),
    "dreg_ngp_density_workspace_bytes": (Z, [I]),
    "dreg_ngp_rgb_dir_fwd": (I, [P] * 6 + [I, P]),
    "dreg_grid_scatter7": (I, [P] * 6 + [I, P]),
    "dreg_grid_sample_points": (I, [P, P, P, I, I, I, P, I, P]),
    "dreg_surface_visibility": (I, [P] * 7 + [P] * 5 + [P, P, P] + [I] * 5 + [F, F, F, F, P]),
    "dreg_surface_visibility_queue": (I, [P] * 7 + [P] * 5 + [P, P, P] + [I] * 5 + [F, F, F, F, P, P, P]),
    "dreg_occupancy_coarse_bits": (I, [P, P, I, I, I, P]),
    "dreg_surface_visibility_desc_bytes": (Z, []),
    "dreg_surface_visibility_fill_desc": (I, [P] + [P] * 7 + [P] * 5 + [P, P, P] + [I] * 5 + [F, F, F, F, P, P]),
    "dreg_surface_visibility_multi": (I, [P, I, ctypes.c_long, P]),
    "dreg_surface_visibility_multi_waves": (I, [P, I, ctypes.c_long, I, P]),
    "dreg_ngp_render": (I, [P, P, ctypes.c_long, P, I, I, I, P] + [P] * 6 + [P] * 5 + [P, P, P] + [F] * 5 + [P] + [P] * 6),
    "dreg_ngp_render_pair": (I, [ctypes.c_long] + ([P, P, P, I, I, I, P] + [P] * 6 + [P] * 5 + [P, P, P] + [F] * 4 + [P]) * 2 + [F, F, P] + [P] * 7),
    "dreg_ngp_render_train": (I, [P, P, P, ctypes.c_long, P, I, I, I, P] + [P] * 6 + [P] * 5 + [P, P, P] + [F] * 5 + [P] + [P] * 6),
    "dreg_ngp_render_bwd_workspace_bytes": (Z, [ctypes.c_long]),
    "dreg_ngp_render_bwd": (I, [P, P, P, ctypes.c_long, P, I, I, I, P, P, P] + [P] * 5 + [P, P, P] + [F] * 5 + [P, P, P, P, P, Z, P]),
    "dreg_ngp_adam_step": (I, [P] * 5 + [Z, F, F, F, F, I, P]),
    "dreg_image_metrics_workspace_bytes": (Z, [I, I, I, I]),
    "dreg_image_metrics": (I, [P, P, I, I, I, I, P] + [P] * 6 + [P, Z, P]),
    "dreg_ngp_density_grad": (I, [P] * 7 + [P] * 5 + [P, I, I, P]),
    "dreg_icp_workspace_bytes": (Z, [I, I]),
    "dreg_icp_refine": (I, [P, I, P, P, P, P, I, P, F, I, I, I, P, F, I] + [ctypes.c_double] * 3 + [P, P, P, P, P, Z, P]),
    "dreg_pose_ransac_workspace_bytes": (Z, [I, I]),
    "dreg_pose_ransac": (I, [P, P, I, P, I, F, F, P, Z, P, P, P, P, P, P, P]),
    "dreg_pose_inliers": (I, [P, P, I, P, F, P, P, P]),
    "dreg_mc_table": (I, [P, P]),
    "dreg_mc_workspace_bytes": (Z, [I, I, I]),
    "dreg_mc_count": (I, [P, I, I, I, F, P, Z, P, P]),
    "dreg_mc_emit": (I, [P, I, I, I, F, P, P, P, Z, P, P, I, I, P]),
}


PROBE_SIGNATURES = {
    "dreg_conv1_bnrelu_a_probe": (I, [P, P, P, P, I, I, I, I, I, I, P]),
    "dreg_conv_set_glds": (None, [I]),
    "dreg_conv_set_wgrad_splits": (None, [I]),
    "dreg_conv_set_wgrad_big": (None, [I]),
    "dreg_conv_igemm_probe": (None, [I]),
    "dreg_conv_set_igemm_ap": (None, [I]),
    "dreg_conv_set_igemm_ap256": (None, [I]),
    "dreg_conv_set_pointwise_rmw_cin": (None, [I]),
    "dreg_conv_igemm_probe_read": (I, [P]),
    "dreg_conv_set_wgrad_pipe": (None, [I]),
    "dreg_conv_wgrad_probe_read": (I, [P]),
    "dreg_conv_set_wgrad_ring": (None, [I]),
    "dreg_conv_set_wgrad_rows_fast": (None, [I]),
    "dreg_conv_set_row_splits": (None, [I]),
    "dreg_conv_set_glds_stages": (None, [I]),
    "dreg_conv_set_wgrad_target_blocks": (None, [I]),
    "dreg_conv_set_narrow_small": (None, [I]),
    "dreg_bn_set_debug_skip": (None, [I]),
    "dreg_bn_set_store_g": (None, [I]),
    "dreg_bn_set_small_regs": (None, [I]),
    "dreg_sstem_set_pool_blocks": (None, [I]),
    "dreg_voxel_set_own_sort": (None, [I]),
    "dreg_conv_set_bn_stats_epilogue": (None, [I]),
    "dreg_conv3_halo_set_variant": (None, [I]),
    "dreg_conv3_halo64_set": (None, [I]),
    "dreg_conv3_halo_set_prof": (None, [P]),
    "dreg_bn_set_small_max_voxels": (None, [I]),
    "dreg_ngp_set_rgb_chunks": (None, [I]),
    "dreg_ngp_set_density_unroll": (None, [I]),
    "dreg_ngp_set_xcd_levels": (None, [I]),
    "dreg_visibility_set_waves": (None, [I]),
    "dreg_visibility_set_pass_bound": (I, [ctypes.c_long]),
    "dreg_render_set_waves": (None, [I]),
    "dreg_render_pair_set_waves": (None, [I]),
    "dreg_render_bwd_set_waves": (None, [I]),
}
PROBE_LIB_PATH = os.path.join(_HERE, "libdreg_nerf_hip_probe.so")
_probe_lib = None


class ExecOpts(ctypes.Structure):
    _fields_ = [(n, c_int) for n in ("sparse_grads", "bn_batch_tails", "fuse_stem", "sparse_stem", "fold_res_bn", "fold_splitk", "group_wgrad",
                                     "s2_accumulate", "fuse_bn_stats", "brick", "defer_head_pg", "persistent_deep", "guard")] + [("reserved", c_int * 3)]


def load_probe():
    global _probe_lib
    if _probe_lib is None:
        if not os.path.exists(PROBE_LIB_PATH):
            raise DregError(f"{PROBE_LIB_PATH} not found: build it with `python -m dreg_nerf_amd.build`")
        lib = ctypes.CDLL(PROBE_LIB_PATH)
        for name, (rt, at) in list(SIGNATURES.items()) + list(PROBE_SIGNATURES.items()):
            _sig(lib, name, rt, at)
        _probe_lib = lib
    return _probe_lib


def use_probe():
    global _lib
    _lib = load_probe()
    return _lib


class probe:

    def __init__(self):
        self._restore = []

    def __enter__(self):
        global _lib
        self._saved = _lib
        _lib = load_probe()
        self.lib = _lib
        return self

    def set(self, name, value, default):
        getattr(self.lib, name)(value)
        self._restore.append((name, default))

    def __getattr__(self, name):
        return getattr(self.__dict__["lib"], name)

    def __exit__(self, *exc):
        global _lib
        for name, default in reversed(self._restore):
            getattr(self.lib, name)(default)
        _lib = self._saved
        return False


def load():
    global _lib
    if _lib is None:
        if not os.path.exists(LIB_PATH):
            raise DregError(
                f"{LIB_PATH} not found: build it with `python -m dreg_nerf_amd.build` "
                "(hipcc --offload-arch=gfx950); dreg_nerf_amd has no CPU/eager fallback")
        lib = ctypes.CDLL(LIB_PATH)
        for name, (rt, at) in SIGNATURES.items():
            _sig(lib, name, rt, at)
        _lib = lib
    return _lib


def declared_symbols():
    return list(SIGNATURES.keys())


def probe_symbols():
    return list(PROBE_SIGNATURES.keys())


def ptr(t):
    if t is None:
        return None
    assert t.is_contiguous(), "non-contiguous tensor handed to the C ABI"
    return t.data_ptr()


def _floats(n, v):
    return (c_float * n)(*[float(t) for t in (v.reshape(-1).tolist() if torch.is_tensor(v) else v)])


def f6(v):
    return _floats(6, v)


def f3(v):
    return _floats(3, v)


_raw_stream = getattr(torch._C, "_cuda_getCurrentRawStream", None)


def stream():
    if _raw_stream is not None:
        return _raw_stream(torch.cuda.current_device())
    return torch.cuda.current_stream().cuda_stream


_DEBUG_SYNC = bool(int(os.environ.get("DREG_DEBUG_SYNC", "0")))


def check(rc, name):
    if rc != 0:
        raise DregError(f"{name} failed with code {rc}")
    if _DEBUG_SYNC:
        import sys
        print(f"[dreg] {name} launched", file=sys.stderr, flush=True)
        torch.cuda.synchronize()


def dt_of(t: torch.Tensor) -> int:
    if t.dtype == torch.bfloat16:
        return DT_BF16
    if t.dtype == torch.float32:
        return DT_F32
    raise DregError(f"unsupported dtype {t.dtype}")


def torch_dtype(dt: int):
    return torch.bfloat16 if dt == DT_BF16 else torch.float32


def to_device_async(data, dtype, device):
    t = torch.tensor(data, dtype=dtype)
    if device.type != "cuda":
        return t
    return t.pin_memory().to(device, non_blocking=True)
```

### dreg_nerf_amd/trunk_exec.py

```python
import ctypes
from typing import Dict, List, Optional

import numpy as np
import torch

from . import lib as L
from . import ops

OP_CONV, OP_BN, OP_MAXPOOL, OP_CONV_ROWS = 0, 1, 2, 3
RL_FIELDS = 8
SERIAL_STREAMS = bool(int(__import__("os").environ.get("DREG_SERIAL_STREAMS", "0")))
KIND_NAMES = {0: "fwd", 1: "dgrad", 2: "wgrad"}
OPTS: Dict[str, int] = {}


class exec_opts:

    def __init__(self, **kw):
        self.kw = kw

    def __enter__(self):
        self.saved = dict(OPTS)
        OPTS.update(self.kw)
        return self

    def __exit__(self, *exc):
        OPTS.clear()
        OPTS.update(self.saved)
        return False


class _Recorder:

    def __init__(self, P: Dict[str, torch.Tensor], x_shape):
        self.P = P
        self.tensors = [tuple(x_shape)]
        self.ops = []
        self.params = []
        self.pindex = {}

    class T:
        def __init__(self, slot, shape):
            self.slot, self.shape = slot, tuple(shape)

    def _new(self, shape):
        self.tensors.append(tuple(shape))
        return _Recorder.T(len(self.tensors) - 1, shape)

    def _p(self, t: Optional[torch.Tensor]) -> int:
        if t is None:
            return -1
        k = id(t)
        if k not in self.pindex:
            self.pindex[k] = len(self.params)
            self.params.append(t)
        return self.pindex[k]

    def conv3d(self, x, w, bias=None, addend=None, stride=1, pad=0, out_rows: int = -1):
        B, D, H, W, _ = x.shape
        k = w.shape[2]
        od = tuple((d + 2 * pad - k) // stride + 1 for d in (D, H, W))
        y = self._new((B,) + od + (w.shape[0],))
        self.ops.append([OP_CONV, x.slot, y.slot, addend.slot if addend is not None else -1, self._p(w), self._p(bias), -1, -1, -1,
                         k, stride, pad, 0, 0, out_rows if (bias is None and addend is None) else -1, -1])
        return y

    def conv3d_rows(self, x, w, bias, addend, pad, out_rows: int, in_rows: int):
        y = self._new(x.shape[:4] + (w.shape[0],))
        self.ops.append([OP_CONV_ROWS, x.slot, y.slot, addend.slot if addend is not None else -1, self._p(w), self._p(bias), -1, -1, -1,
                         w.shape[2], 1, pad, 0, 0, out_rows, in_rows])
        return y

    def batchnorm(self, x, gamma, beta, running_mean, running_var, res=None, relu=True, train=True):
        y = self._new(x.shape)
        self.ops.append([OP_BN, x.slot, y.slot, res.slot if res is not None else -1, self._p(gamma), self._p(beta),
                         self._p(running_mean), self._p(running_var), -1, 0, 0, 0, int(relu), 0, -1, -1])
        return y

    def maxpool3d(self, x):
        B, D, H, W, C = x.shape
        y = self._new((B,) + tuple((d + 2 - 3) // 2 + 1 for d in (D, H, W)) + (C,))
        self.ops.append([OP_MAXPOOL, x.slot, y.slot, -1, -1, -1, -1, -1, -1, 3, 2, 1, 0, 0, -1, -1])
        return y


class TrunkExecutor:

    def __init__(self, model, x_shape, sparse_head: int, with_grad: bool = True, stem_rows: bool = False, opts: Optional[Dict[str, int]] = None):
        self.lib = L.load()
        self.opts = L.ExecOpts()
        self.lib.dreg_exec_default_opts(ctypes.byref(self.opts))
        for k, v in {**OPTS, **(opts or {})}.items():
            if not hasattr(self.opts, k):
                raise L.DregError(f"unknown executor option {k!r}")
            setattr(self.opts, k, int(v))
        P = model._P()
        rec = _Recorder(P, x_shape)
        x0 = _Recorder.T(0, x_shape)
        self.nbt = []
        rl = None if not sparse_head else ops.RowSets((0, 1, 2, None) if sparse_head == 1 else (0, 1, 2, None, 4, 5))
        if rl is not None and stem_rows:
            rl.stem = len(rl)
        self.stem_slot = rl.stem if (rl is not None and stem_rows) else -1
        out = model._fpn_program(rec, x0, rl, self.nbt, True)
        self.out_shape = out.shape
        self.rec = rec
        dev = next(model.parameters()).device
        self.device = dev
        tens = np.asarray(rec.tensors, dtype=np.int32)
        opsa = np.asarray(rec.ops, dtype=np.int32)
        prm = np.zeros((len(rec.params), 5), dtype=np.int64)
        self._param_refs = rec.params
        self._sig = []
        for i, t in enumerate(rec.params):
            assert t.is_contiguous() and t.dtype == torch.float32, "the executor reads fp32 master parameters in place"
            g = t.grad if (with_grad and isinstance(t, torch.nn.Parameter) and t.requires_grad) else None
            if g is not None:
                assert g.is_contiguous() and g.dtype == torch.float32
            elif with_grad and isinstance(t, torch.nn.Parameter) and t.requires_grad:
                raise L.DregError("TrunkExecutor needs preallocated .grad buffers (FlatAdamW) on every trainable parameter")
            prm[i, 0] = t.data_ptr()
            prm[i, 1] = g.data_ptr() if g is not None else 0
            prm[i, 2] = t.shape[0]
            prm[i, 3] = t.shape[1] if t.dim() > 1 else 1
            prm[i, 4] = t.shape[2] if t.dim() == 5 else 1
            self._sig.append((t.data_ptr(), prm[i, 1]))
        self.h = self.lib.dreg_exec_create_opts(tens.ctypes.data, len(rec.tensors), opsa.ctypes.data, len(rec.ops), prm.ctypes.data, len(rec.params),
                                                ctypes.byref(self.opts))
        if not self.h:
            raise L.DregError("dreg_exec_create_opts rejected the op program")
        self.arena_bytes = self.lib.dreg_exec_arena_bytes(self.h)
        self.arena = torch.empty(self.arena_bytes, dtype=torch.uint8, device=dev)
        self.pack = torch.empty(self.lib.dreg_exec_pack_bytes(self.h), dtype=torch.uint8, device=dev)
        n = self.lib.dreg_exec_num_packs(self.h)
        host = np.zeros((n, 12), dtype=np.int32)
        rowmap = np.zeros(self.lib.dreg_exec_pack_rows(self.h), dtype=np.int32)
        L.check(self.lib.dreg_exec_export_pack_table(self.h, host.ctypes.data, rowmap.ctypes.data, self.pack.data_ptr()), "dreg_exec_export_pack_table")
        self.pack_table = torch.from_numpy(host).to(dev)
        self.pack_rowmap = torch.from_numpy(rowmap).to(dev)
        self.out_slot = self.lib.dreg_exec_output_slot(self.h)
        self.out_off = self.lib.dreg_exec_tensor_offset(self.h, self.out_slot)
        self.pack_stamp = None
        self._timing = False
        self.last_row_counts = []
        self.sparse_head = sparse_head
        self.with_grad = with_grad
        self.labels = self._labels()
        if SERIAL_STREAMS:
            self.lib.dreg_exec_set_overlap(self.h, 0)

    def __del__(self):
        try:
            if getattr(self, "h", None):
                self.lib.dreg_exec_destroy(self.h)
                self.h = None
        except Exception:
            pass

    def still_valid(self) -> bool:
        for t, (vp, gp) in zip(self._param_refs, self._sig):
            g = t.grad if (self.with_grad and isinstance(t, torch.nn.Parameter) and t.requires_grad) else None
            if t.data_ptr() != vp or (g.data_ptr() if g is not None else 0) != gp:
                return False
        return True

    def _labels(self):
        out = {}
        lib = self.lib
        for i, o in enumerate(self.rec.ops):
            if o[0] not in (OP_CONV, OP_CONV_ROWS):
                continue
            x, y = self.rec.tensors[o[1]], self.rec.tensors[o[2]]
            w = self.rec.params[o[4]]
            B = x[0]
            k, s = o[9], o[10]
            cout, cin = w.shape[0], w.shape[1]
            M = B * y[1] * y[2] * y[3]
            pd = o[11] if len(o) > 11 else k // 2
            is_rows = o[0] == OP_CONV_ROWS or o[14] >= 0

            def fwd_name(nr, B=B, x=x, y=y, cout=cout, k=k, s=s, pd=pd):
                return ops.igemm_kernel_name(lib, B, x[1], x[2], x[3], x[4], y[1], y[2], y[3], cout, k, s, pd, 0, nr, 0 if nr else 1, False, L.DT_BF16, False)

            def dgrad_name(nr, B=B, x=x, y=y, cout=cout, k=k, s=s, pd=pd, add=False):
                if s == 2:
                    dc = tuple((d + 1) // 2 for d in x[1:4])
                    return ops.igemm_kernel_name(lib, B, y[1], y[2], y[3], cout, dc[0], dc[1], dc[2], (1 if k == 1 else 8) * x[4], 1 if k == 1 else 2, 1, 0, 0, 0, 0, False,
                                                 L.DT_BF16, False)
                return ops.igemm_kernel_name(lib, B, y[1], y[2], y[3], cout, x[1], x[2], x[3], x[4], k, 1, pd, 1, nr, 0 if nr else 1, add, L.DT_BF16, False)
            fname, dname = (fwd_name, dgrad_name) if is_rows else (fwd_name(0), dgrad_name(0))
            dname_add = None if is_rows else dgrad_name(0, add=True)
            halo = self.lib.dreg_exec_op_halo(self.h, i)
            if halo & 1:
                fname = "conv3_halo64_kernel<bf16>" if cout == 64 else "conv3_halo_kernel<bf16>"
            if halo & 2:
                dname = "conv3_halo64_kernel<bf16>" if x[4] == 64 else "conv3_halo_kernel<bf16>"
            rows = "-rows" if is_rows else ""
            fl = 2.0 * M * cout * k ** 3 * cin
            per_row = 2.0 * cout * k ** 3 * cin
            lo, li = (o[14], o[15]) if rows else (-1, -1)
            out[(i, 0)] = (fname, f"fwd{rows} B{B} {x[1]}x{x[2]}x{x[3]}x{x[4]}->{y[1]}x{y[2]}x{y[3]}x{cout} k{k}s{s}", fl, lo, per_row, f"conv3_brick_kernel<{cout},bf16>", None)
            out[(i, 1)] = (dname, f"dgrad{rows} B{B} {y[1]}x{y[2]}x{y[3]}x{cout}->{x[1]}x{x[2]}x{x[3]}x{cin} k{k}s{s}", fl, li, per_row, f"conv3_brick_kernel<{cin},bf16>", dname_add)
            def wgrad_name(nr, B=B, x=x, y=y, cout=cout, k=k, is_rows=is_rows, first=int(o[1] == 0)):
                return ops.wgrad_kernel_name(lib, B, y[1], y[2], y[3], x[4], cout, k, is_rows, nr, first)
            wname = wgrad_name if is_rows else wgrad_name(0)
            out[(i, 2)] = (wname, f"wgrad{rows} B{B} {x[1]}x{x[2]}x{x[3]}x{x[4]} g{y[1]}x{y[2]}x{y[3]}x{cout} k{k}s{s}", fl, lo, per_row, None, None)
        out[(-1, 3)] = ("wgrad_reduce_batched_kernel", "split sums of a backward range -> torch-layout gradients", 0.0, -1, 0.0, None, None)
        out[(-1, 4)] = ("bn_tail_batched_kernel<0>", "running statistics of the small BatchNorms of a forward pass", 0.0, -1, 0.0, None, None)
        out[(-1, 5)] = ("bn_tail_batched_kernel<1>", "dgamma / dbeta of the small BatchNorms of a backward range", 0.0, -1, 0.0, None, None)
        return out

    def repack_if_stale(self):
        stamp = (ops._weight_generation, sum(t._version for t in self._param_refs))
        if self.pack_stamp != stamp:
            L.check(self.lib.dreg_exec_repack(self.h, L.ptr(self.pack_table), L.ptr(self.pack_rowmap), L.stream()), "dreg_exec_repack")
            self.pack_stamp = stamp

    def repack_after_update(self):
        with ops.pack_region():
            self.repack_if_stale()

    @staticmethod
    def _rowlist_array(rows):
        if rows is None:
            return None, 0
        n = len(rows)
        stem = getattr(rows, "stem", None)
        a = (ctypes.c_int64 * (RL_FIELDS * (n + (1 if stem is not None else 0))))()
        if stem is not None:
            a[RL_FIELDS * n], a[RL_FIELDS * n + 1] = stem.data_ptr(), stem.shape[0]
        tiles = getattr(rows, "tiles", None) or {}
        for i in range(n):
            if i == 3 or rows[i] is None:
                continue
            a[RL_FIELDS * i] = rows[i].data_ptr()
            a[RL_FIELDS * i + 1] = rows[i].shape[0]
            bt = tiles.get(i)
            if bt is not None and bt.ntiles > 0:
                a[RL_FIELDS * i + 2], a[RL_FIELDS * i + 3] = bt.tiles.data_ptr(), bt.ntiles
                a[RL_FIELDS * i + 4], a[RL_FIELDS * i + 5], a[RL_FIELDS * i + 6] = bt.halo.data_ptr(), bt.nbr.data_ptr(), bt.rows_sorted.data_ptr()
        return a, n + (1 if stem is not None else 0)

    def forward(self, x: torch.Tensor, rows, train: bool) -> torch.Tensor:
        ops.wait_packs()
        self.repack_if_stale()
        want = ops.PROFILER is not None and ops.PROFILER.enabled
        if want != self._timing:
            self.set_timing(want)
        self.last_row_counts = [int(r.shape[0]) if (r is not None and i != 3) else 0 for i, r in enumerate(rows)] if rows is not None else []
        if rows is not None and getattr(rows, "stem", None) is not None:
            self.last_row_counts.append(int(rows.stem.shape[0]))
        ra, n = self._rowlist_array(rows)
        self._guarded(self.lib.dreg_exec_forward(self.h, L.ptr(self.arena), self.arena_bytes, L.ptr(self.pack), L.ptr(x),
                                                 ctypes.addressof(ra) if ra is not None else None, n, int(train), L.stream()), "dreg_exec_forward")
        self.generation = getattr(self, "generation", 0) + 1
        nbytes = int(np.prod(self.out_shape)) * 2
        return self.arena[self.out_off:self.out_off + nbytes].view(torch.bfloat16).view(self.out_shape)

    def _guarded(self, rc: int, name: str):
        if rc == -3:
            op, ps, band = ctypes.c_int(), ctypes.c_int(), ctypes.c_longlong()
            self.lib.dreg_exec_guard_last(self.h, ctypes.byref(op), ctypes.byref(ps), ctypes.byref(band))
            raise L.DregError(f"{name}: guard band overwritten behind op {op.value} ({'backward' if ps.value else 'forward'} pass; "
                              f"{self.rec.ops[op.value] if 0 <= op.value < len(self.rec.ops) else 'pass tail'}): {self.guard_describe(band.value)}")
        L.check(rc, name)
        if self.opts.guard:
            bad = self.guard_check()
            if bad[0]:
                raise L.DregError(f"{name}: {bad[0]} guard band(s) overwritten ({bad[3]} 16-byte words); first: {self.guard_describe(bad[1])} + {bad[2]} bytes")

    def guard_check(self):
        if self.device.type == "cuda":
            aux_stream(self.device).synchronize()
        out = (ctypes.c_longlong * 4)()
        L.check(self.lib.dreg_exec_guard_check(self.h, L.ptr(self.arena), out, L.stream()), "dreg_exec_guard_check")
        return list(out)

    def guard_describe(self, band: int) -> str:
        buf = ctypes.create_string_buffer(256)
        self.lib.dreg_exec_guard_describe(self.h, int(band), buf, 256)
        return buf.value.decode()

    def backward(self, x: torch.Tensor, rows, grad_out: torch.Tensor, generation: Optional[int] = None):
        if generation is not None and generation != getattr(self, "generation", 0):
            raise L.DregError("TrunkExecutor.backward: the arena holds the activations of a LATER forward pass than the one this gradient belongs to "
                              "(two grad-mode forwards before a backward — gradient accumulation over several forwards, retain_graph — need one "
                              "executor each; the product step runs one forward and one backward per step)")
        ra, n = self._rowlist_array(rows)
        sync = ops.GRAD_SYNC
        self._flush_deferred()
        if sync is None:
            self._guarded(self.lib.dreg_exec_backward(self.h, L.ptr(self.arena), self.arena_bytes, L.ptr(self.pack), L.ptr(x), L.ptr(grad_out),
                                                      ctypes.addressof(ra) if ra is not None else None, n, L.stream(), aux_stream(self.device).cuda_stream),
                          "dreg_exec_backward")
            return
        plan = self._sync_plan(sync)
        sync.ready(plan["above"])
        hi = len(self.rec.ops)
        for k, (lo_op, done_from) in enumerate(plan["cuts"]):
            flags = (1 if k == 0 else 0) | (2 if k == len(plan["cuts"]) - 1 else 0)
            self._guarded(self.lib.dreg_exec_backward_range(self.h, L.ptr(self.arena), self.arena_bytes, L.ptr(self.pack), L.ptr(x), L.ptr(grad_out),
                                                            ctypes.addressof(ra) if ra is not None else None, n, L.stream(), aux_stream(self.device).cuda_stream,
                                                            lo_op, hi, flags), "dreg_exec_backward_range")
            hi = lo_op
            sync.ready(done_from)

    def _flush_deferred(self):
        if ops._PENDING_REDUCE:
            with torch.cuda.stream(aux_stream(self.device)):
                ops.flush_wgrad_reduce()

    def _sync_plan(self, sync):
        key = (id(sync.opt), tuple(sync.buckets))
        if getattr(self, "_plan_key", None) == key:
            return self._plan
        spans = {}
        for i, t in enumerate(self.rec.params):
            g = t.grad if (isinstance(t, torch.nn.Parameter) and t.requires_grad) else None
            off = sync.opt.offset_of(g.data_ptr()) if g is not None else -1
            if off >= 0:
                spans[i] = (off, t.numel())
        touched = [[p for p in (o[4], o[5]) if p in spans] for o in self.rec.ops]
        above = max((off + n for off, n in spans.values()), default=0)
        pending = dict(spans)
        bounds = sorted({lo for lo, _ in sync.buckets}, reverse=True)
        cuts, last_done = [], above
        for i in range(len(self.rec.ops) - 1, -1, -1):
            for p in touched[i]:
                pending.pop(p, None)
            done_from = max((off + n for off, n in pending.values()), default=0)
            crossed = [b for b in bounds if done_from <= b < last_done]
            if crossed or i == 0:
                cuts.append((i, done_from))
                last_done = done_from
        self._plan_key, self._plan = key, {"above": above, "cuts": cuts}
        return self._plan

    def set_input_row_occupancy(self, row_occ):
        self._row_occ = row_occ
        self.lib.dreg_exec_set_input_row_occupancy(self.h, L.ptr(row_occ) if row_occ is not None else None)

    def set_timing(self, on: bool):
        self._timing = bool(on)
        self.lib.dreg_exec_set_timing(self.h, int(on))
        self.lib.dreg_exec_set_overlap(self.h, int(not on and not SERIAL_STREAMS))

    def drain_timings(self, profiler: "ops.KernelTimer"):
        cap = 65536
        ok = (ctypes.c_int * (3 * cap))()
        ms = (ctypes.c_float * cap)()
        n = self.lib.dreg_exec_read_timings(self.h, ok, ms, cap)
        for i in range(n):
            name, label, fl, lid, per_row, brick_name, add_name = self.labels[(ok[3 * i], ok[3 * i + 1])]
            if lid >= 0:
                nr = self.last_row_counts[lid]
                fl, label = per_row * nr, f"{label} rows{nr}"
                if callable(name):
                    name = name(nr)
            if ok[3 * i + 2] == 2 and brick_name:
                name = brick_name
            elif ok[3 * i + 2] == 1 and add_name:
                name = add_name
            profiler.add_measured(name, label, fl, ms[i])


_AUX = {}
AUX_CU_MASK = int(__import__("os").environ.get("DREG_AUX_CU_MASK", "0"))


def aux_stream(device) -> "torch.cuda.Stream":
    key = (device.type, device.index if device.index is not None else torch.cuda.current_device())
    st = _AUX.get(key)
    if st is None:
        prio = __import__("os").environ.get("DREG_AUX_PRIORITY", "low")
        st = None
        if AUX_CU_MASK and device.type == "cuda":
            words = {1: [0xFFFFFFFF] * 4 + [0] * 4, 2: [0x55555555] * 8, 3: [0xFFFFFFFF] * 2 + [0] * 6, 4: [0x11111111] * 8, 5: [0xFFFFFFFF] * 6 + [0] * 2,
                     6: [0x0000FFFF] * 8, 7: [0x000000FF] * 8}[int(AUX_CU_MASK)]
            hip = ctypes.CDLL("libamdhip64.so")
            h = ctypes.c_void_p()
            arr = (ctypes.c_uint32 * 8)(*words)
            with torch.cuda.device(device):
                rc = hip.hipExtStreamCreateWithCUMask(ctypes.byref(h), 8, arr)
            if rc != 0 or not h.value:
                raise RuntimeError(f"hipExtStreamCreateWithCUMask failed: {rc}")
            st = torch.cuda.ExternalStream(h.value, device=device)
        if st is None and prio != "torch" and device.type == "cuda":
            try:
                hip = ctypes.CDLL("libamdhip64.so")
                least, greatest = ctypes.c_int(), ctypes.c_int()
                h = ctypes.c_void_p()
                with torch.cuda.device(device):
                    ok = hip.hipDeviceGetStreamPriorityRange(ctypes.byref(least), ctypes.byref(greatest)) == 0
                    ok = ok and hip.hipStreamCreateWithPriority(ctypes.byref(h), 1, least.value if prio == "low" else int(prio)) == 0
                if ok and h.value:
                    st = torch.cuda.ExternalStream(h.value, device=device)
            except (OSError, ValueError):
                st = None
        if st is None:
            st = torch.cuda.Stream(device=device)
        _AUX[key] = st
    return st


class _TrunkFn(torch.autograd.Function):

    @staticmethod
    def forward(ctx, x, anchor, ex: TrunkExecutor, rows, train: bool):
        ctx.ex, ctx.rows = ex, rows
        ctx.save_for_backward(x)
        y = ex.forward(x, rows, train)
        ctx.generation = ex.generation
        return y

    @staticmethod
    def backward(ctx, g):
        (x,) = ctx.saved_tensors
        ctx.ex.backward(x, ctx.rows, g.contiguous(), ctx.generation)
        return None, None, None, None, None


def run_trunk(ex: TrunkExecutor, x, anchor, rows, train):
    return _TrunkFn.apply(x, anchor, ex, rows, train)
```

### include/dreg_nerf.h

```cpp
#ifndef DREG_NERF_H
#define DREG_NERF_H
#include <stddef.h>
#include <stdint.h>

#ifdef __cplusplus
extern "C" {
#endif

#define DREG_OK 0
#define DREG_EINVAL (-1)

int dreg_conv_get_glds(void);


int dreg_conv3d_kpad(int ksz, int Cin, int dtype);

int dreg_pack_conv_weight(const float* w, void* out, int Cout, int Cin_real, int Cin, int ksz, int for_dgrad,
                          int dtype, void* stream);
int dreg_pack_conv_weights_batched(const void* descs, int n, int total_rows, int stage_floats, const int* row_desc,
                                   void* stream);

int dreg_conv3d_igemm(const void* in, const void* wt_packed, void* out, const float* bias, const void* addend,
                      int B, int Di, int Hi, int Wi, int Cin, int Do, int Ho, int Wo, int Cout,
                      int ksz, int stride, int pad, int transposed, int relu, int Da, int Ha, int Wa, int add_same,
                      int dtype, int out_f32, void* stream);
size_t dreg_conv3d_igemm_workspace_bytes(int B, int Di, int Hi, int Wi, int Cin, int Do, int Ho, int Wo, int Cout,
                                         int ksz, int stride, int pad, int transposed, int has_addend, int dtype);
int dreg_conv3d_igemm_ws(const void* in, const void* wt_packed, void* out, const float* bias, const void* addend,
                         int B, int Di, int Hi, int Wi, int Cin, int Do, int Ho, int Wo, int Cout,
                         int ksz, int stride, int pad, int transposed, int relu, int Da, int Ha, int Wa, int add_same,
                         int dtype, int out_f32, void* workspace, size_t workspace_bytes, void* stream);
int dreg_conv3d_igemm_occ(const void* in, const void* wt_packed, void* out, const float* bias, const void* addend,
                          int B, int Di, int Hi, int Wi, int Cin, int Do, int Ho, int Wo, int Cout,
                          int ksz, int stride, int pad, int transposed, int relu, int Da, int Ha, int Wa, int add_same,
                          int dtype, int out_f32, void* workspace, size_t workspace_bytes, const uint8_t* rowocc, void* stream);

int dreg_conv3d_igemm_bnstats(const void* in, const void* wt_packed, void* out, const float* bias, const void* addend,
                              int B, int Di, int Hi, int Wi, int Cin, int Do, int Ho, int Wo, int Cout,
                              int ksz, int stride, int pad, int relu, int Da, int Ha, int Wa, int add_same,
                              void* workspace, size_t workspace_bytes, float* bn_partial, int* rows_per_chunk, void* stream);
int dreg_bn3d_fwd_from_sums(const void* x, const void* res, void* y, const float* gamma, const float* beta,
                            float* running_mean, float* running_var, float* scale_shift, float* mean_rstd, float* sums,
                            int rows_per_chunk, int B, int V, int C, float eps, float momentum, int relu, int dtype, void* stream);

int dreg_conv3_halo_supported(int B, int D, int H, int W, int Cin, int Cout);
int dreg_conv3_halo_use(int B, int D, int H, int W, int Cin, int Cout, int ksz, int stride, int pad);
size_t dreg_conv3_halo_pack_bytes(int Cin_reduced);
int dreg_pack_conv_weight_halo(const float* w, void* out, int Cout, int Cin, int transposed, void* stream);
int dreg_conv3_halo(const void* in, const void* wpk, void* out, const float* bias, const void* addend,
                    int B, int D, int H, int W, int Cin, int Da, int Ha, int Wa, int add_same, int out_f32, void* stream);
size_t dreg_conv3_halo_pack_bytes_n(int Cin_reduced, int rows);
int dreg_conv3_halo_n(const void* in, const void* wpk, void* out, const float* bias, const void* addend,
                      int B, int D, int H, int W, int Cin, int Cout, int Da, int Ha, int Wa, int add_same, int out_f32, void* stream);
int dreg_conv3_halo_n_bnstats(const void* in, const void* wpk, void* out, const float* bias, const void* addend,
                              int B, int D, int H, int W, int Cin, int Cout, int Da, int Ha, int Wa, int add_same, float* bn_partial, int* rows_per_chunk, void* stream);

int dreg_conv3d_dgrad_s2(const void* gout, const void* wt_class_packed, void* din, int B, int Di, int Hi, int Wi, int Cin,
                         int Do, int Ho, int Wo, int Cout, int ksz, int pad, void* stream);
int dreg_conv3d_dgrad_s2_acc(const void* gout, const void* wt_class_packed, void* din, int B, int Di, int Hi, int Wi, int Cin,
                             int Do, int Ho, int Wo, int Cout, int ksz, int pad, void* stream);

int dreg_conv3d_igemm_variant(int B, int Di, int Hi, int Wi, int Cin, int Do, int Ho, int Wo, int Cout, int ksz, int stride, int pad,
                              int transposed, int nrows, int has_ws, int has_addend, int dtype);
int dreg_conv3d_wgrad_variant(int B, int Do, int Ho, int Wo, int Cin, int Cout, int ksz, int rows, int nrows, int occ);
int dreg_conv3d_wgrad_splits(int B, int Do, int Ho, int Wo, int Cin, int Cout, int ksz, int dtype);
size_t dreg_conv3d_wgrad_workspace_bytes(int B, int Do, int Ho, int Wo, int Cin, int Cout, int ksz, int dtype);
int dreg_conv3d_wgrad(const void* gout, const void* in, float* dw, void* workspace, size_t workspace_bytes,
                      int B, int Di, int Hi, int Wi, int Cin, int Cin_real, int Do, int Ho, int Wo, int Cout,
                      int ksz, int stride, int pad, int accumulate, int dtype, int use_tr, void* stream);
int dreg_conv3d_wgrad_occ(const void* gout, const void* in, float* dw, void* workspace, size_t workspace_bytes,
                          int B, int Di, int Hi, int Wi, int Cin, int Cin_real, int Do, int Ho, int Wo, int Cout,
                          int ksz, int stride, int pad, int accumulate, int dtype, int use_tr, const uint8_t* rowocc, void* stream);

int dreg_conv3d_igemm_rows(const void* in, const void* wt_packed, void* out, const float* bias, const void* addend,
                           const int* rows, int nrows,
                           int B, int Di, int Hi, int Wi, int Cin, int Do, int Ho, int Wo, int Cout,
                           int ksz, int stride, int pad, int transposed, int relu, int Da, int Ha, int Wa, int add_same,
                           int out_f32, void* stream);
int dreg_conv3d_wgrad_rows(const void* gout, const void* in, float* dw, void* workspace, size_t workspace_bytes,
                           const int* rows, int nrows,
                           int B, int Di, int Hi, int Wi, int Cin, int Cin_real, int Do, int Ho, int Wo, int Cout,
                           int ksz, int stride, int pad, int accumulate, void* stream);
int dreg_conv3d_wgrad_partials(const void* gout, const void* in, void* workspace, size_t workspace_bytes, const int* rows, int nrows,
                               int B, int Di, int Hi, int Wi, int Cin, int Cin_real, int Do, int Ho, int Wo, int Cout,
                               int ksz, int stride, int pad, const uint8_t* rowocc, void* stream);
int dreg_wgrad_reduce_blocks(int Cout, int Cin_real, int ksz, int nsplit);
int dreg_wgrad_reduce_batched(const void* descs_dev, int n, int block_base, int nblocks, void* stream);
int dreg_wgrad_group_desc_bytes(void);
int dreg_linear_wgrad_group_fill(void* desc_host, const void* gout, const void* in, void* workspace, size_t workspace_bytes,
                                 int rows, int Cin, int Cout, int* variant, int* nblocks);
int dreg_conv3d_wgrad_group_fill(void* desc_host, const void* gout, const void* in, void* workspace, size_t workspace_bytes,
                                 int B, int Di, int Hi, int Wi, int Cin, int Do, int Ho, int Wo, int Cout, int ksz, int stride, int pad,
                                 int* variant, int* nblocks);
int dreg_wgrad_group_launch(const void* descs_dev, int n, int variant, int total_blocks, void* stream);

int dreg_bn_num_chunks(int V);
int dreg_bn3d_fwd(const void* x, const void* res, void* y, const float* gamma, const float* beta,
                  float* running_mean, float* running_var, float* scale_shift, float* mean_rstd, float* workspace,
                  int B, int V, int C, float eps, float momentum, int train, int relu, int dtype, void* stream);
int dreg_bn3d_bwd(const void* x, const void* dy, const void* y, const float* scale_shift, const float* mean_rstd,
                  void* dx, void* dres, float* dgamma, float* dbeta, float* coef, float* workspace,
                  int B, int V, int C, int relu, int accumulate, int dtype, void* stream);
int dreg_bn_small(int B, int V, int C, int dtype);
int dreg_bn3d_fwd_defer_update(const void* x, const void* res, void* y, const float* gamma, const float* beta,
                               float* running_mean, float* running_var, float* scale_shift, float* mean_rstd, float* workspace,
                               int B, int V, int C, float eps, float momentum, int train, int relu, int dtype, float* var_keep, int* deferred, void* stream);
int dreg_bn3d_bwd_defer_params(const void* x, const void* dy, const void* y, const float* scale_shift, const float* mean_rstd,
                               void* dx, void* dres, float* dgamma, float* dbeta, float* coef, float* workspace,
                               int B, int V, int C, int relu, int accumulate, int dtype, float* sums_keep, int* deferred, void* stream);
typedef struct dreg_bn_extra {
    const float* res_scale_shift;
    const float* splitk_part;
    int splitk_nsplit;
    size_t splitk_slice;
} dreg_bn_extra;
int dreg_bn3d_fwd_ex(const void* x, const void* res, void* y, const float* gamma, const float* beta,
                     float* running_mean, float* running_var, float* scale_shift, float* mean_rstd, float* workspace,
                     int B, int V, int C, float eps, float momentum, int train, int relu, int dtype, float* var_keep, int* deferred,
                     int sums_rows_per_chunk, const dreg_bn_extra* ex, void* stream);
int dreg_bn3d_bwd_ex(const void* x, const void* dy, const void* y, const float* scale_shift, const float* mean_rstd,
                     void* dx, void* dres, float* dgamma, float* dbeta, float* coef, float* workspace,
                     int B, int V, int C, int relu, int accumulate, int dtype, float* sums_keep, int* deferred, const dreg_bn_extra* ex, void* stream);
int dreg_conv3d_igemm_defer(const void* in, const void* wt_packed, void* out, const float* bias, const void* addend,
                            int B, int Di, int Hi, int Wi, int Cin, int Do, int Ho, int Wo, int Cout,
                            int ksz, int stride, int pad, int transposed, int relu, int Da, int Ha, int Wa, int add_same,
                            void* workspace, size_t workspace_bytes, const uint8_t* rowocc, int* sk_nsplit, size_t* sk_slice, void* stream);
int dreg_bn_small_in_regs(int B, int V, int C, int dtype);
int dreg_bn_running_update_batched(const void* descs_dev, int n, int block_base, int nblocks, float momentum, void* stream);
int dreg_bn_param_grad_batched(const void* descs_dev, int n, int block_base, int nblocks, int accumulate, void* stream);

int dreg_bn_relu_maxpool_fwd(const void* x, void* pooled, uint8_t* argmax, const float* gamma, const float* beta,
                             float* running_mean, float* running_var, float* scale_shift, float* mean_rstd, float* workspace,
                             int B, int Di, int Hi, int Wi, int Do, int Ho, int Wo, int C, float eps, float momentum, int train, int relu, void* stream);
int dreg_bn_relu_maxpool_bwd(const void* x, const void* dp, const uint8_t* argmax, const float* scale_shift, const float* mean_rstd,
                             void* dx, float* dgamma, float* dbeta, float* coef, float* workspace,
                             int B, int Di, int Hi, int Wi, int Do, int Ho, int Wo, int C, int relu, int accumulate, void* stream);
size_t dreg_sparse_stem_workspace_floats(int B, int Do, int Ho, int Wo, int C);
int dreg_sparse_stem_fwd(const void* x, const int* rows, int n, const int* rows_a, int n_a, void* act, void* pooled, uint8_t* argmax, void* xam, uint8_t* pmask,
                         const float* gamma, const float* beta, float* running_mean, float* running_var, float* scale_shift, float* mean_rstd, float* workspace,
                         int B, int Di, int Hi, int Wi, int Do, int Ho, int Wo, int C, float eps, float momentum, int train, int relu, void* stream);
int dreg_sparse_stem_bwd(const void* x, const void* dp, const uint8_t* argmax, const void* xam, const void* dl, const int* rows_a, int n_a,
                         const int* rows, int n, const float* scale_shift, const float* mean_rstd, void* dx, float* dgamma, float* dbeta, float* coef, float* workspace,
                         int B, int Di, int Hi, int Wi, int Do, int Ho, int Wo, int C, int relu, int accumulate, void* stream);
int dreg_maxpool3d_fwd(const void* x, void* y, uint8_t* argmax, int B, int Di, int Hi, int Wi, int Do, int Ho, int Wo,
                       int C, int dtype, void* stream);
int dreg_maxpool3d_bwd(const void* dy, const uint8_t* argmax, void* dx, int B, int Di, int Hi, int Wi, int Do, int Ho,
                       int Wo, int C, int dtype, void* stream);
int dreg_maxpool3d_bwd_acc(const void* dy, const uint8_t* argmax, void* dx, int B, int Di, int Hi, int Wi, int Do, int Ho,
                           int Wo, int C, int accumulate, int dtype, void* stream);

int dreg_downsample_sum(const void* g, void* out, int B, int Df, int Hf, int Wf, int Dc, int Hc, int Wc, int C,
                        int dtype, void* stream);
int dreg_downsample_sum_rows(const void* g, void* out, const int* rows, int nrows, int Df, int Hf, int Wf, int Dc, int Hc, int Wc,
                             int C, int dtype, void* stream);

size_t dreg_colsum_workspace_bytes(size_t M, int C);
int dreg_colsum(const void* g, float* out, float* workspace, size_t M, int C, int accumulate, int dtype, void* stream);

int dreg_trilinear_gather_fwd(const void* p1, const int64_t* idx, const int* pt_batch, void* out, int N, int d, int h,
                              int w, int C, int Zr, int Xr, int Yr, int dtype, int out_f32, void* stream);
int dreg_trilinear_gather_bwd(const float* dfeat, const int64_t* idx, const int* pt_batch, float* dp1_f32, int N, int d,
                              int h, int w, int C, int Zr, int Xr, int Yr, void* stream);
int dreg_cast_from_f32(const float* in, void* out, size_t n, int dtype, void* stream);
int dreg_fill_zero(void* p, size_t bytes, void* stream);
int dreg_guard_fill(void* base, const void* offsets_dev, int n, int band_bytes, void* stream);
int dreg_guard_scan(const void* base, const void* offsets_dev, int n, int band_bytes, void* result_dev, void* stream);
int dreg_colsum_rows_per_chunk(size_t M);
int dreg_colsum_batched(const void* descs_dev, int n, int total_pblocks, int total_fblocks, void* stream);
int dreg_add_inplace(void* dst, const void* src, size_t n, int dtype, void* stream);
int dreg_pack_rgba_grids(const void* grids, void* out, int B, int Z, int X, int Y, int dtype, void* stream);
int dreg_pack_rgba_grids_occ(const void* grids, void* out, uint8_t* inocc, int B, int Z, int X, int Y, int dtype, void* stream);
int dreg_pack_rgba_sparse(const float* vals, const int64_t* idx, const int* pt_batch, void* out, int N, int B, int Z, int X,
                          int Y, int dtype, void* stream);
int dreg_pack_rgba_sparse_occ(const float* vals, const int64_t* idx, const int* pt_batch, void* out, uint8_t* inocc, int N, int B, int Z, int X,
                              int Y, int dtype, void* stream);
int dreg_conv_row_occupancy(const uint8_t* inocc, uint8_t* rowocc, int B, int Di, int Hi, int Do, int Ho, int ksz, int stride, int pad, void* stream);
int dreg_gather_grid_xyz(const void* grids, const int64_t* idx, const int* pt_batch, float* xyz, int N, int Zr, int Xr, int Yr,
                         void* stream);

size_t dreg_active_sets_workspace_bytes(int B, int d, int h, int w);
int dreg_active_sets(const int64_t* idx, const int* pt_batch, int N, int B, int Zr, int Xr, int Yr, int d, int h, int w,
                     int* rows, int* counts, int* map1, void* workspace, size_t workspace_bytes, void* stream);
size_t dreg_active_sets_level2_workspace_bytes(int B, int d2, int h2, int w2);
int dreg_active_sets_level2(const uint8_t* child_flags, int B, int d, int h, int w, int d2, int h2, int w2, int* rows2,
                            int* counts2, void* workspace, size_t workspace_bytes, void* stream);
size_t dreg_conv_rows_workspace_bytes(int B, int d, int h, int w);
int dreg_conv_rows(const int64_t* idx, const int* pt_batch, int N, int B, int Zr, int Xr, int Yr, int d, int h, int w, int ksz, int stride, int pad,
                   int* rows, int* count, void* workspace, size_t workspace_bytes, void* stream);
int dreg_trilinear_gather_bwd_rows(const float* dfeat, const int64_t* idx, const int* pt_batch, const int* rows1, int n1,
                                   const int* map1, float* comp, void* dp1, int N, int B, int d, int h, int w, int C,
                                   int Zr, int Xr, int Yr, int dtype, void* stream);
int dreg_trilinear_gather_bwd_gather(const float* dfeat, const int64_t* idx, const int* pt_batch, const int* rows1, int n1,
                                     int* fine_map, void* dp1, int N, int B, int d, int h, int w, int C, int Zr, int Xr,
                                     int Yr, int dtype, void* stream);
int dreg_trilinear_gather_bwd_gather_rows_only(const float* dfeat, const int64_t* idx, const int* pt_batch, const int* rows1, int n1,
                                               int* fine_map, void* dp1, int N, int B, int d, int h, int w, int C, int Zr, int Xr, int Yr,
                                               int dtype, void* stream);
int dreg_trilinear_gather_bwd_gather_seg(const float* g1, const void* seg_descs, const int64_t* idx, const int* pt_batch, const int* rows1, int n1,
                                         int* fine_map, void* dp1, int N, int B, int d, int h, int w, int C, int Zr, int Xr, int Yr,
                                         int dtype, int zero_dense, void* stream);
int dreg_gather_segment_mean(const void* p1, const int64_t* idx, const int* pt_batch, int point_start, const uint32_t* order, const uint32_t* starts,
                             const int* n_out, float* out, int M, int d, int h, int w, int C, int Zr, int Xr, int Yr, int dtype, void* stream);
int dreg_zero_rows(void* buf, const int* rows, int nrows, int C, int dtype, void* stream);
int dreg_colsum_rows(const void* g, const int* rows, int nrows, float* out, float* workspace, int C, int accumulate,
                     int dtype, void* stream);

void* dreg_exec_create(const int* tensors, int nt, const int* ops, int nops, const int64_t* params, int np);
typedef struct dreg_exec_opts {
    int sparse_grads;
    int bn_batch_tails;
    int fuse_stem;
    int sparse_stem;
    int fold_res_bn;
    int fold_splitk;
    int group_wgrad;
    int s2_accumulate;
    int fuse_bn_stats;
    int brick;
    int defer_head_pg;
    int persistent_deep;
    int guard;
    int reserved[3];
} dreg_exec_opts;
void dreg_exec_default_opts(dreg_exec_opts* o);
void* dreg_exec_create_opts(const int* tensors, int nt, const int* ops, int nops, const int64_t* params, int np, const dreg_exec_opts* opts);
#define DREG_EGUARD (-3)
int dreg_exec_guard_bands(void* h);
int dreg_exec_guard_check(void* h, void* arena, long long* out4, void* stream);
int dreg_exec_guard_describe(void* h, int band, char* buf, int buf_bytes);
int dreg_exec_guard_last(void* h, int* op, int* pass, long long* band);
void dreg_exec_destroy(void* h);
size_t dreg_exec_arena_bytes(void* h);
size_t dreg_exec_pack_bytes(void* h);
int dreg_exec_num_packs(void* h);
size_t dreg_exec_tensor_offset(void* h, int slot);
int dreg_exec_output_slot(void* h);
int dreg_exec_pack_rows(void* h);
int dreg_exec_export_pack_table(void* h, void* host_out, int* host_row_desc, void* pack_base);
int dreg_exec_repack(void* h, const void* descs_dev, const int* row_desc_dev, void* stream);
int dreg_exec_op_halo(void* h, int op);
void dreg_exec_set_overlap(void* h, int enable);
void dreg_exec_set_input_row_occupancy(void* h, const uint8_t* rowocc);
void dreg_exec_set_timing(void* h, int enable);
int dreg_exec_read_timings(void* h, int* op_kind, float* ms, int max);
int dreg_exec_forward(void* h, void* arena, size_t arena_bytes, const void* pack_base, const void* x_in,
                      const int64_t* rowlists, int nlists, int train, void* stream);
int dreg_exec_backward(void* h, void* arena, size_t arena_bytes, const void* pack_base, const void* x_in,
                       const void* grad_out, const int64_t* rowlists, int nlists, void* stream, void* aux_stream);
int dreg_exec_backward_range(void* h, void* arena, size_t arena_bytes, const void* pack_base, const void* x_in, const void* grad_out,
                             const int64_t* rowlists, int nlists, void* stream, void* aux_stream, int op_begin, int op_end, int flags);

int dreg_mha_fwd(const void* q, const void* k, const void* v, void* o, float* lse, int Nq, int Nk, int H,
                 int ldq, int ldk, int ldv, int ldo, float scale, int dtype, void* stream);
int dreg_mha_bwd(const void* q, const void* k, const void* v, const void* o, const void* dout, const float* lse,
                 float* dvec, void* dq, void* dk, void* dv, int Nq, int Nk, int H,
                 int ldq, int ldk, int ldv, int ldo, float scale, int dtype, void* stream);
int dreg_corr_attention_fwd(const void* q, const void* k, const float* xyz, float* out, float* lse, int L, int Nq, int Nk,
                            float scale, int dtype, void* stream);
int dreg_corr_attention_bwd(const void* q, const void* k, const float* xyz, const float* out, const float* dout,
                            const float* lse, float* dvec, void* dq, void* dk, int L, int Nq, int Nk,
                            float scale, int dtype, void* stream);

int dreg_mha_varlen_fwd(const void* q, const void* k, const void* v, void* o, float* lse, const int* probs, int nprob,
                        int max_q, int max_k, int R, int H, int ldq, int ldk, int ldv, int ldo, float scale, int dtype, void* stream);
int dreg_mha_varlen_bwd(const void* q, const void* k, const void* v, const void* o, const void* dout, const float* lse,
                        float* dvec, void* dq, void* dk, void* dv, const int* probs, int nprob, int max_q, int max_k, int R, int H,
                        int ldq, int ldk, int ldv, int ldo, float scale, int dtype, void* stream);
int dreg_corr_attention_varlen_fwd(const void* q, const void* k, const float* xyz, float* out, float* lse, const int* probs, int nprob,
                                   int max_q, int max_k, int L, int R, float scale, int dtype, void* stream);
int dreg_corr_attention_varlen_bwd(const void* q, const void* k, const float* xyz, const float* out, const float* dout,
                                   const float* lse, float* dvec, void* dq, void* dk, const int* probs, int nprob,
                                   int max_q, int max_k, int L, int R, float scale, int dtype, void* stream);

int dreg_layernorm_fwd(const float* x, const float* gamma, const float* beta, const float* pe, void* y, float* stats,
                       int N, int C, float eps, int out_dtype, void* stream);
size_t dreg_layernorm_bwd_workspace_bytes(int N);
int dreg_layernorm_bwd(const float* x, const void* dy, const float* gamma, const float* stats, float* dx, float* dgamma,
                       float* dbeta, float* workspace, int N, int C, int g_dtype, int accumulate_dx, int accumulate_w,
                       void* stream);
int dreg_layernorm_bwd_add(const float* x, const void* dy, const float* gamma, const float* stats, float* dx, const float* dx_add, float* dgamma,
                           float* dbeta, float* workspace, int N, int C, int g_dtype, int accumulate_w, void* stream);

int dreg_layernorm_fwd2(const float* x, const float* gamma, const float* beta, const float* pe, int pe_rows, float* y32, void* y16, float* stats,
                        int N, int C, float eps, void* stream);
int dreg_layernorm_bwd_parts(const float* x, const void* dy, const void* dy2_bf16, const float* gamma, const float* stats, float* dx, const float* dx_add,
                             const float* dx_add2, void* dx_bf16, float* part, int N, int C, int g_dtype, void* stream);
int dreg_layernorm_bwd_blocks(int N);
int dreg_layernorm_bwd_final_batched(const void* descs_dev, int n, void* stream);

int dreg_posenc_sine(const float* xyz, float* pe, int N, float scale, float temperature, void* stream);

int dreg_overlap_fwd(const float* f, const float* w, const float* b, float* s, int N, void* stream);
size_t dreg_overlap_bwd_workspace_bytes(int N);
int dreg_overlap_bwd(const float* f, const float* w, const float* s, const float* gy, float* df, float* dw, float* db,
                     float* workspace, int N, void* stream);

int dreg_overlap_bwd_acc(const float* f, const float* w, const float* s, const float* gy, float* df, const float* df_add, float* dw, float* db,
                         int accumulate_w, float* workspace, int N, void* stream);

int dreg_relu_bwd(const void* y, const void* g, void* out, size_t n, int y_dtype, int g_dtype, int out_dtype, void* stream);

int dreg_weighted_kabsch(const float* a, const float* b, const float* w, float* out, int P, int N, float eps, void* stream);
int dreg_weighted_kabsch_pairs(const float* xyz, const float* corr, const float* ov, const int* probs, float* out, int P, int L,
                               int R, float eps, void* stream);
int dreg_weighted_kabsch_bwd(const float* a, const float* b, const float* w, const float* g_out, float* g_a, float* g_b, float* g_w, int P, int N,
                             float eps, void* stream);
int dreg_weighted_kabsch_pairs_bwd(const float* xyz, const float* corr, const float* ov, const int* probs, const float* g_out, float* g_corr,
                                   float* g_ov, int P, int L, int R, float eps, void* stream);

int dreg_reg_point_losses(const float* gt, const float* tilde, const float* ov, const float* corr, const float* xyz,
                          const float* pose, const int* probs, float* partial, float* d_ov, float* d_corr, int L, int R, int P,
                          int robust, float eps, float w_overlap, float w_corr, void* stream);
int dreg_gemm_f32_desc_bytes(void);
int dreg_gemm_f32_batched(const void* descs_dev, int n, int total_tiles, const float* const* bases8, void* stream);
int dreg_infonce_wsym(const float* W, float* out, int E, void* stream);
int dreg_infonce_nn(const float* xyz, const float* pose, const int* probs, const int* src_off, int* nn, float* mask,
                    float* count, int P, int total_src, float r_p, void* stream);
int dreg_infonce_rows(float* logits, const float* xyz, const float* pose, const int* probs, const int* src_off,
                      const long long* logit_off, const int* nn, const float* mask, const float* count, float* loss_row, int P,
                      int total_src, float r_n, float scale, int write_grad, void* stream);
int dreg_reg_losses_final(const float* partial, const float* loss_row, const float* count, const int* probs, const int* src_off,
                          float* out, int P, int L, float eps, float w_overlap, float w_cont, float w_feat, float w_corr,
                          void* stream);
int dreg_nerf_cont_deferred(const float* gt, const float* tilde, const int* probs, float* partial, float* out, int P, int L, int R,
                            float w_overlap, float w_cont, float w_feat, float w_corr, void* stream);

int dreg_halfspace_labels(const float* xyz, const float* corr, float* gt, float* tilde, int L, int R, void* stream);

size_t dreg_voxel_downsample_workspace_bytes(int N);
int dreg_voxel_downsample_fwd(const float* pts, const float* feats, const int* pt_batch, float* out_pts, float* out_feats,
                              int* n_out, int* batch_counts, uint32_t* inv_seg, float* inv_cnt, int* err,
                              void* workspace, size_t workspace_bytes, int N, int C, int nbatch, float dl, void* stream);
int dreg_voxel_downsample_plan(const float* pts, const int* pt_batch, float* out_pts, int* n_out, int* batch_counts,
                               uint32_t* inv_seg, float* inv_cnt, int* err, uint32_t* order, uint32_t* starts,
                               void* workspace, size_t workspace_bytes, int N, int nbatch, float dl, void* stream);
int dreg_voxel_downsample_plan_frozen(const float* pts, const int* pt_batch, float* out_pts, int* n_out, int* batch_counts,
                                      uint32_t* inv_seg, float* inv_cnt, int* err, uint32_t* order, uint32_t* starts,
                                      void* workspace, size_t workspace_bytes, int N, int nbatch, float dl, const uint8_t* frozen, void* stream);
int dreg_voxel_segment_mean(const float* feats, const uint32_t* order, const uint32_t* starts, const int* n_out,
                            float* out_feats, int M, int C, void* stream);
int dreg_voxel_downsample_bwd(const float* gout, const uint32_t* inv_seg, const float* inv_cnt, float* gin, int N, int C,
                              void* stream);

int dreg_grad_norm(const float* g, float* norm_out, float* workspace, size_t n, void* stream);
int dreg_adamw_step(float* p, float* g, float* m, float* v, const float* norm, size_t n, float lr, float beta1, float beta2,
                    float eps, float weight_decay, int step, float max_norm, void* stream);

uint32_t dreg_ngp_level_table(float per_level_scale, int log2_hashmap_size, int base_resolution,
                              uint32_t* offset, uint32_t* size, uint32_t* res, float* scale, uint32_t* hashed);
int dreg_f32_to_f16(const float* in, void* out, size_t n, void* stream);
int dreg_ngp_density_fwd(const float* x, const void* table, const void* w1, const void* w2, float* density, void* raw,
                         const uint32_t* offset, const uint32_t* size, const uint32_t* res, const float* scale,
                         const uint32_t* hashed, const float* aabb, int Np, void* stream);
int dreg_ngp_dir_bias(const float* dirs, const void* w1_f16, float* out, int K, void* stream);
int dreg_ngp_alpha_keep(const float* density, float* alpha, uint8_t* keep, int N, float delta, float threshold, void* stream);
int dreg_ngp_rgb_mean_fwd(const void* raw, const void* w1, const void* w2, const void* w3, const float* dirbias, float* rgb,
                          int ndir, int Np, void* stream);
int dreg_ngp_density_fwd_contract(const float* x, const void* table, const void* w1, const void* w2, float* density, void* raw,
                                  const uint32_t* offset, const uint32_t* size, const uint32_t* res, const float* scale, const uint32_t* hashed,
                                  const float* aabb, int Np, int contract, void* stream);
size_t dreg_ngp_density_workspace_bytes(int Np);
int dreg_ngp_density_fwd_ws(const float* x, const void* table, const void* w1, const void* w2, float* density, void* raw,
                            const uint32_t* offset, const uint32_t* size, const uint32_t* res, const float* scale, const uint32_t* hashed,
                            const float* aabb, int Np, int contract, void* workspace, size_t workspace_bytes, const int* order, int x_in_slot_order, void* stream);
int dreg_grid_sample_points_ordered(const int64_t* idx, const float* jitter, const int* order, float* world, float* world_slot,
                                    int rx, int ry, int rz, const float* aabb, int Np, void* stream);
size_t dreg_grid_x_order_workspace_bytes(int rx, int ry, int rz);
int dreg_grid_x_order(const uint8_t* binary, const int64_t* idx, int* order, void* workspace, size_t workspace_bytes, int rx, int ry, int rz, int Np, void* stream);
size_t dreg_grid_occupied_workspace_bytes(int rx, int ry, int rz);
void* dreg_grid_occupied_totals(void* workspace, int rx, int ry, int rz);
int dreg_grid_occupied_count(const uint8_t* binary, void* workspace, size_t workspace_bytes, int rx, int ry, int rz, void* stream);
int dreg_grid_occupied_build(const uint8_t* binary, void* workspace, const float* jitter, const float* aabb, int64_t* indices, int* order,
                             float* world, float* world_slot, int rx, int ry, int rz, int N, void* stream);
int dreg_ngp_density_keep_fwd_ws(const float* x, const void* table, const void* w1, const void* w2, float* density, void* raw,
                                 const uint32_t* offset, const uint32_t* size, const uint32_t* res, const float* scale, const uint32_t* hashed,
                                 const float* aabb, int Np, int contract, void* workspace, size_t workspace_bytes, const int* order, int x_in_slot_order,
                                 float* alpha, uint8_t* keep, float delta, float threshold, void* stream);
int dreg_grid_write_kept(void* occ_workspace, const float* xyz, const float* rgb, const float* alpha, const int64_t* indices, const uint8_t* keep,
                         int64_t* mask, float* grid, int rx, int ry, int rz, int Np, void* stream);
int dreg_ngp_rgb_dir_fwd(const void* raw, const void* w1, const void* w2, const void* w3, const float* dirs, float* rgb, int Np, void* stream);
int dreg_grid_sample_points(const int64_t* idx, const float* jitter, float* world, int rx, int ry, int rz, const float* aabb,
                            int Np, void* stream);
int dreg_grid_scatter7(const float* xyz, const float* rgb, const float* alpha, const int64_t* idx, const uint8_t* keep,
                       float* grid, int Np, void* stream);

int dreg_surface_visibility(const float* cams, const float* pts, const uint8_t* binary, int* label,
                            const void* table, const void* w1, const void* w2,
                            const uint32_t* offset, const uint32_t* size, const uint32_t* res, const float* scale,
                            const uint32_t* hashed, const float* roi_aabb, const float* scene_aabb, const float* model_aabb,
                            int rx, int ry, int rz, int Nc, int Np, float render_step_size, float cut_off, float early_stop_eps,
                            float alpha_thre, void* stream);
int dreg_surface_visibility_queue(const float* cams, const float* pts, const uint8_t* binary, int* label,
                                  const void* table, const void* w1, const void* w2,
                                  const uint32_t* offset, const uint32_t* size, const uint32_t* res, const float* scale, const uint32_t* hashed,
                                  const float* roi_aabb, const float* scene_aabb, const float* model_aabb,
                                  int rx, int ry, int rz, int Nc, int Np, float render_step_size, float cut_off, float early_stop_eps,
                                  float alpha_thre, void* queue, const uint32_t* coarse_bits, void* stream);
int dreg_occupancy_coarse_bits(const uint8_t* binary, uint32_t* bits, int rx, int ry, int rz, void* stream);
size_t dreg_surface_visibility_desc_bytes(void);
int dreg_surface_visibility_fill_desc(void* host_desc, const float* cams, const float* pts, const uint8_t* binary, int* label,
                                      const void* table, const void* w1, const void* w2,
                                      const uint32_t* offset, const uint32_t* size, const uint32_t* res, const float* scale, const uint32_t* hashed,
                                      const float* roi_aabb, const float* scene_aabb, const float* model_aabb,
                                      int rx, int ry, int rz, int Nc, int Np, float render_step_size, float cut_off, float early_stop_eps,
                                      float alpha_thre, void* queue, const uint32_t* coarse_bits);
int dreg_surface_visibility_multi(const void* descs_dev, int n, long total_rays, void* stream);
int dreg_surface_visibility_multi_waves(const void* descs_dev, int n, long total_rays, int max_waves, void* stream);

int dreg_ngp_render(const float* origins, const float* viewdirs, long n_rays, const uint8_t* binary, int rx, int ry, int rz, const uint32_t* coarse_bits,
                    const void* table, const void* w1, const void* w2, const void* cw1, const void* cw2, const void* cw3,
                    const uint32_t* offset, const uint32_t* size, const uint32_t* res, const float* scale, const uint32_t* hashed,
                    const float* roi_aabb, const float* scene_aabb, const float* model_aabb, float near_plane, float far_plane,
                    float render_step_size, float alpha_thre, float early_stop_eps, const float* bkgd,
                    float* rgb, float* opacity, float* depth, unsigned long long* n_samples, void* queue, void* stream);

int dreg_ngp_render_pair(long n_rays,
                         const float* src_origins, const float* src_viewdirs, const uint8_t* src_binary, int src_rx, int src_ry, int src_rz,
                         const uint32_t* src_coarse_bits, const void* src_table, const void* src_w1, const void* src_w2,
                         const void* src_cw1, const void* src_cw2, const void* src_cw3,
                         const uint32_t* src_offset, const uint32_t* src_size, const uint32_t* src_res, const float* src_scale, const uint32_t* src_hashed,
                         const float* src_roi_aabb, const float* src_scene_aabb, const float* src_model_aabb,
                         float src_near_plane, float src_far_plane, float src_render_step_size, float src_alpha_thre, const float* src_center,
                         const float* tgt_origins, const float* tgt_viewdirs, const uint8_t* tgt_binary, int tgt_rx, int tgt_ry, int tgt_rz,
                         const uint32_t* tgt_coarse_bits, const void* tgt_table, const void* tgt_w1, const void* tgt_w2,
                         const void* tgt_cw1, const void* tgt_cw2, const void* tgt_cw3,
                         const uint32_t* tgt_offset, const uint32_t* tgt_size, const uint32_t* tgt_res, const float* tgt_scale, const uint32_t* tgt_hashed,
                         const float* tgt_roi_aabb, const float* tgt_scene_aabb, const float* tgt_model_aabb,
                         float tgt_near_plane, float tgt_far_plane, float tgt_render_step_size, float tgt_alpha_thre, const float* tgt_center,
                         float power, float early_stop_eps, const float* bkgd,
                         float* rgb, float* opacity, float* depth, float* weight_src, unsigned long long* n_samples, void* queue, void* stream);

int dreg_ngp_render_train(const float* origins, const float* viewdirs, const float* jitter, long n_rays, const uint8_t* binary, int rx, int ry, int rz,
                          const uint32_t* coarse_bits, const void* table, const void* w1, const void* w2, const void* cw1, const void* cw2, const void* cw3,
                          const uint32_t* offset, const uint32_t* size, const uint32_t* res, const float* scale, const uint32_t* hashed,
                          const float* roi_aabb, const float* scene_aabb, const float* model_aabb, float near_plane, float far_plane,
                          float render_step_size, float alpha_thre, float early_stop_eps, const float* bkgd,
                          float* rgb, float* opacity, float* depth, unsigned long long* n_samples, void* queue, void* stream);
size_t dreg_ngp_render_bwd_workspace_bytes(long n_rays);
int dreg_ngp_render_bwd(const float* origins, const float* viewdirs, const float* jitter, long n_rays, const uint8_t* binary, int rx, int ry, int rz,
                        const uint32_t* coarse_bits, const void* base16, const void* color16,
                        const uint32_t* offset, const uint32_t* size, const uint32_t* res, const float* scale, const uint32_t* hashed,
                        const float* roi_aabb, const float* scene_aabb, const float* model_aabb, float near_plane, float far_plane,
                        float render_step_size, float alpha_thre, float early_stop_eps,
                        const float* rgb, const float* grad_rgb, float* grad_base, float* grad_color, void* workspace, size_t workspace_bytes, void* stream);
int dreg_ngp_adam_step(float* p, float* g, float* m, float* v, void* p16, size_t n, float lr, float beta1, float beta2, float eps, int step, void* stream);

size_t dreg_image_metrics_workspace_bytes(int N, int H, int W, int C);
int dreg_image_metrics(const float* pred, const float* gt, int N, int H, int W, int C, const float* taps, float* ssim, float* mse, float* psnr,
                       float* ssim_map, uint8_t* pred_u8, uint8_t* gt_u8, void* workspace, size_t workspace_bytes, void* stream);

int dreg_ngp_density_grad(const float* x, const void* table, const void* w1, const void* w2, float* density, float* grad, unsigned long long* relu_mask,
                          const uint32_t* offset, const uint32_t* size, const uint32_t* res, const float* scale, const uint32_t* hashed,
                          const float* aabb, int Np, int contract, void* stream);

size_t dreg_icp_workspace_bytes(int Ns, int iters);
int dreg_icp_refine(const float* src, int Ns, const float* tgt_points, const float* tgt_normals, const int* perm, const int* cell_start, int Nt,
                    const float* grid_lo, float cell, int nx, int ny, int nz, double* pose, float max_dist, int iters,
                    double tol_rot, double tol_trans, double eps_cond, double* stats, double* sums, int* corr, float* dist2,
                    void* workspace, size_t workspace_bytes, void* stream);

size_t dreg_pose_ransac_workspace_bytes(int N, int H);
int dreg_pose_ransac(const float* a, const float* b, int N, const int* triplets, int H, float thresh, float eps_area, void* workspace,
                     size_t workspace_bytes, int* best, float* pose, int* status, int* counts, float* poses, unsigned char* mask, void* stream);
int dreg_pose_inliers(const float* a, const float* b, int N, const float* pose, float thresh, unsigned char* mask, int* count, void* stream);

int dreg_mc_table(signed char* tris, int* width);
size_t dreg_mc_workspace_bytes(int nx, int ny, int nz);
int dreg_mc_count(const float* values, int nx, int ny, int nz, float level, void* workspace, size_t workspace_bytes, int* counts, void* stream);
int dreg_mc_emit(const float* values, int nx, int ny, int nz, float level, const float* origin, const float* spacing, const void* workspace,
                 size_t workspace_bytes, float* verts, int* faces, int V, int F, void* stream);

int dreg_brick_supported(int B, int D, int H, int W, int Cin, int Cout);
size_t dreg_conv3_brick_pack_bytes(int rows, int red);
int dreg_pack_conv_weight_brick(const float* w, void* out, int Cout, int Cin, int transposed, void* stream);
size_t dreg_brick_tiles_workspace_bytes(int B, int D, int H, int W);
int dreg_brick_tiles_build(const uint8_t* flags, int B, int D, int H, int W, int max_rows, int max_tiles, void* workspace, size_t workspace_bytes,
                           int* meta, int* rows_sorted, void* tiles, int* halo_vox, void* nbr, void* stream);
int dreg_conv3_brick(const void* in, const void* wpk, void* out, const float* bias, const void* addend, const void* tiles, int ntiles,
                     const int* halo_vox, const void* nbr, const int* rows_sorted,
                     int B, int D, int H, int W, int Cin, int Cout, int Da, int Ha, int Wa, int add_same, int out_f32, void* stream);

int dreg_ps_num_params(void);
int dreg_ps_num_linears(void);
void* dreg_ps_create(const int64_t* params);
void dreg_ps_destroy(void* h);
void dreg_ps_set_fuse(void* h, int fuse);
void dreg_ps_set_group_wgrad(void* h, int on);
void dreg_ps_set_timing(void* h, int enable);
int dreg_ps_read_timings(void* h, int* info, float* ms, int cap);
size_t dreg_ps_arena_bytes(void* h, int R);
int dreg_ps_forward(void* h, void* arena, size_t arena_bytes, const int64_t* packs, const float* feats, const float* xyz, const float* pe,
                    const int* probs_self, const int* probs_cross, int nprob, int max_len, int R,
                    float* cond, float* corr, float* ov, void* stream);
int dreg_ps_backward(void* h, void* arena, size_t arena_bytes, const int64_t* packs, const float* feats, const float* xyz, const float* pe,
                     const int* probs_self, const int* probs_cross, int nprob, int max_len, int R,
                     const float* cond, const float* corr, const float* ov, const float* g_cond, const float* g_corr, const float* g_ov,
                     float* d_feats, void* stream, void* aux_stream, int last_only);
int dreg_ps_panel_fwd(const void* a1, const void* w1_packed, const float* bias1, const float* residual, float* x_out,
                      const float* gamma, const float* beta, const float* pe, void* h_out, float* stats,
                      const void* w2_packed, const float* bias2, void* out2, int R, int K1, int N2, int relu, float eps, void* stream);
int dreg_ps_panel_bwd(const void* g1, const void* w1t_packed, const float* x, const float* stats, const float* gamma,
                      const float* dx_add, const float* dx_add2, float* dx, void* dx_bf16, float* part,
                      const void* w2t_packed, void* out2, int R, int K1, int N2, void* stream);

#ifdef __cplusplus
}
#endif
#endif
```

Baseline: 259.8 pairs/s.

## Add streaming pointwise (1x1x1) conv kernel with LDS staging and fused BN stats

Adds a dedicated persistent kernel for 1x1x1 convolutions. It keeps the weights in registers, double-buffers input tiles into LDS with buffer_load_lds, and writes output through a swizzled LDS stage using nontemporal stores. It can also emit BatchNorm partial sums in the same pass. The executor sends forward and dgrad pointwise convs on large grids to it, replacing the generic implicit-GEMM path, with the aim of cutting memory traffic and kernel overhead for these bandwidth-bound layers. The kernel only handles a fixed set of Cin/Cout pairs, adds a new option field, and carries inline-asm and LDS-sizing risk.

After: 263.1 pairs/s, median of 6. 1.01x the previous value.

```diff
diff --git a/dreg_nerf_amd/csrc/conv_pointwise.hip b/dreg_nerf_amd/csrc/conv_pointwise.hip
--- /dev/null
+++ b/dreg_nerf_amd/csrc/conv_pointwise.hip
@@ -0,0 +1,352 @@
+#include "common.h"
+#include "../../include/dreg_nerf.h"
+
+__device__ __forceinline__ void wg_barrier() {
+    asm volatile("s_waitcnt lgkmcnt(0)" ::: "memory");
+    __builtin_amdgcn_s_barrier();
+    asm volatile("" ::: "memory");
+}
+
+typedef __attribute__((ext_vector_type(2))) uint32_t u32x2_t;
+typedef __attribute__((ext_vector_type(4))) uint32_t u32x4_t;
+__device__ __forceinline__ void lds_rd64x4(const uint32_t (&a)[4], u32x2_t (&v)[4]) {
+    asm volatile("ds_read_b64 %0, %4\n\tds_read_b64 %1, %5\n\tds_read_b64 %2, %6\n\tds_read_b64 %3, %7\n\ts_waitcnt lgkmcnt(0)"
+                 : "=&v"(v[0]), "=&v"(v[1]), "=&v"(v[2]), "=&v"(v[3]) : "v"(a[0]), "v"(a[1]), "v"(a[2]), "v"(a[3]) : "memory");
+}
+template <int OFF>
+__device__ __forceinline__ void lds_rd128x2(uint32_t a, u32x4_t& v0, u32x4_t& v1) {
+    asm volatile("ds_read_b128 %0, %2 offset:%3\n\tds_read_b128 %1, %2 offset:%4\n\ts_waitcnt lgkmcnt(0)" : "=&v"(v0), "=&v"(v1) : "v"(a), "n"(OFF), "n"(OFF + 4096) : "memory");
+}
+__device__ __forceinline__ void lds_wr64(uint32_t a, u32x2_t v) { asm volatile("ds_write_b64 %0, %1" ::"v"(a), "v"(v) : "memory"); }
+__device__ __forceinline__ void lds_wr128(uint32_t a, f32x4_t v) { asm volatile("ds_write_b128 %0, %1" ::"v"(a), "v"(v) : "memory"); }
+
+__device__ __forceinline__ float dpp_shr1(float v) { return __int_as_float(__builtin_amdgcn_update_dpp(0, __float_as_int(v), 0x111, 0xf, 0xf, true)); }
+
+template <int CIN, int BN, bool STATS>
+__global__ __launch_bounds__(256, 2) void conv1_stream_kernel(
+    const bf16_t* __restrict__ in, const bf16_t* __restrict__ wt, bf16_t* out, const float* __restrict__ bias, const bf16_t* addend,
+    uint32_t M, int Cout, int Kpad, int relu, uint32_t in_bytes, uint32_t out_bytes, uint32_t nchunks, float* __restrict__ bn_part)
+{
+    typedef __attribute__((address_space(3))) void* lds_ptr_t;
+    constexpr int TN = BN / 64, KK = CIN / 32, RB = BN * 2;
+    constexpr int SWM = (BN / 8 < 16 ? BN / 8 : 16) - 1;
+    constexpr int IN_BYTES = 64 * CIN * 2, OB_BYTES = 64 * RB;
+    constexpr int PA = CIN / 32, PO = BN / 32;
+    constexpr uint32_t OOB = 0x7fffff00u;
+    extern __shared__ __attribute__((aligned(16))) char smem[];
+
+    const bool has_add = addend != nullptr;
+    const int t = threadIdx.x, lane = t & 63;
+    const int wave = __builtin_amdgcn_readfirstlane(t >> 6);
+    const int n0 = blockIdx.y * BN;
+    const uint32_t c_begin = (uint32_t)((uint64_t)blockIdx.x * nchunks / gridDim.x);
+    const uint32_t c_end = (uint32_t)((uint64_t)(blockIdx.x + 1) * nchunks / gridDim.x);
+    const int ntiles = 2 * (int)(c_end - c_begin);
+    if (ntiles <= 0) return;
+
+    const __amdgpu_buffer_rsrc_t rs_in = __builtin_amdgcn_make_buffer_rsrc((void*)in, 0, in_bytes, 0x00020000);
+    const __amdgpu_buffer_rsrc_t rs_add = __builtin_amdgcn_make_buffer_rsrc((void*)(has_add ? addend : out), 0, out_bytes, 0x00020000);
+
+    uint32_t aoff[PA];
+#pragma unroll
+    for (int i = 0; i < PA; ++i) {
+        const int p = wave * PA + i, kb = p >> 3, r = (p & 7) * 8 + (lane >> 3);
+        const int gl = (lane & 7) ^ ((r >> 1) & 7);
+        aoff[i] = (uint32_t)(r * CIN * 2 + kb * 128 + gl * 16);
+    }
+    uint32_t ooff[PO];
+#pragma unroll
+    for (int i = 0; i < PO; ++i) {
+        const int q = (wave * PO + i) * 1024 + lane * 16, r = q / RB, lg = ((q % RB) >> 4) ^ (r & SWM);
+        ooff[i] = (uint32_t)(r * Cout * 2 + (n0 + lg * 8) * 2);
+    }
+#pragma unroll
+    for (int i = 0; i < PA; ++i) asm volatile("" : "+v"(aoff[i]));
+#pragma unroll
+    for (int i = 0; i < PO; ++i) asm volatile("" : "+v"(ooff[i]));
+
+    auto issue = [&](int ti, int buf) {
+        const uint32_t m0 = (2u * c_begin + (uint32_t)ti) * 64u;
+        const int rem = m0 < M ? (int)(M - m0 < 64u ? M - m0 : 64u) : 0;
+        char* sA = smem + buf * IN_BYTES + wave * PA * 1024;
+        const uint32_t soA = m0 * (uint32_t)(CIN * 2);
+#pragma unroll
+        for (int i = 0; i < PA; ++i) {
+            const int r = ((wave * PA + i) & 7) * 8 + (lane >> 3);
+            __builtin_amdgcn_raw_ptr_buffer_load_lds(rs_in, (lds_ptr_t)(sA + i * 1024), 16, (int)(r < rem ? aoff[i] : OOB), (int)soA, 0, 0);
+        }
+        if (has_add) {
+            char* sO = smem + 2 * IN_BYTES + buf * OB_BYTES + wave * PO * 1024;
+            const uint32_t soO = m0 * (uint32_t)(Cout * 2);
+#pragma unroll
+            for (int i = 0; i < PO; ++i) {
+                const int r = ((wave * PO + i) * 1024 + lane * 16) / RB;
+                __builtin_amdgcn_raw_ptr_buffer_load_lds(rs_add, (lds_ptr_t)(sO + i * 1024), 16, (int)(r < rem ? ooff[i] : OOB), (int)soO, 0, 0);
+            }
+        }
+    };
+
+    issue(0, 0);
+    const int fr = lane & 15, kg = lane >> 4;
+    bf16x8_t bw[TN][KK];
+#pragma unroll
+    for (int j = 0; j < TN; ++j)
+#pragma unroll
+        for (int kk = 0; kk < KK; ++kk)
+            bw[j][kk] = *reinterpret_cast<const bf16x8_t*>(wt + (size_t)(n0 + wave * (BN / 4) + j * 16 + fr) * Kpad + kk * 32 + kg * 8);
+    float b4[TN][4];
+#pragma unroll
+    for (int j = 0; j < TN; ++j)
+#pragma unroll
+        for (int r = 0; r < 4; ++r) b4[j][r] = bias ? bias[n0 + wave * (BN / 4) + j * 16 + kg * 4 + r] : 0.f;
+
+    const uint32_t lds0 = (uint32_t)(uintptr_t)(__attribute__((address_space(3))) char*)smem;
+    u32x2_t keep[STATS ? TN : 1][4];
+#pragma unroll
+    for (int j = 0; j < (STATS ? TN : 1); ++j)
+#pragma unroll
+        for (int i = 0; i < 4; ++i) keep[j][i] = (u32x2_t){0u, 0u};
+
+    for (int ti = 0; ti < ntiles; ++ti) {
+        const int cur = ti & 1;
+        if (ti + 1 < ntiles) {
+            issue(ti + 1, cur ^ 1);
+            if (has_add) asm volatile("s_waitcnt vmcnt(%0)" ::"n"(PA + PO) : "memory");
+            else asm volatile("s_waitcnt vmcnt(%0)" ::"n"(PA) : "memory");
+        } else asm volatile("s_waitcnt vmcnt(0)" ::: "memory");
+        wg_barrier();
+
+        f32x4_t acc[4][TN];
+#pragma unroll
+        for (int i = 0; i < 4; ++i)
+#pragma unroll
+            for (int j = 0; j < TN; ++j) acc[i][j] = (f32x4_t){0.f, 0.f, 0.f, 0.f};
+        const char* sA = smem + cur * IN_BYTES;
+#pragma unroll
+        for (int kk = 0; kk < KK; ++kk) {
+            bf16x8_t af[4];
+#pragma unroll
+            for (int i = 0; i < 4; ++i) {
+                const int row = i * 16 + fr, slot = (kk & 1) * 4 + kg;
+                af[i] = *reinterpret_cast<const bf16x8_t*>(sA + (kk >> 1) * 8192 + row * 128 + ((slot ^ ((row >> 1) & 7)) << 4));
+            }
+#pragma unroll
+            for (int i = 0; i < 4; ++i)
+#pragma unroll
+                for (int j = 0; j < TN; ++j)
+                    acc[i][j] = __builtin_amdgcn_mfma_f32_16x16x32_bf16(bw[j][kk], af[i], acc[i][j], 0, 0, 0);
+        }
+
+        const uint32_t oO = lds0 + 2 * IN_BYTES + (has_add ? cur : 0) * OB_BYTES;
+        const bool second = STATS && (ti & 1) != 0;
+#pragma unroll
+        for (int j = 0; j < TN; ++j) {
+            const int lg = wave * (BN / 32) + 2 * j + (kg >> 1);
+            uint32_t pa[4];
+            u32x2_t ad[4];
+#pragma unroll
+            for (int i = 0; i < 4; ++i) {
+                const int row = i * 16 + fr;
+                pa[i] = oO + row * RB + ((lg ^ (row & SWM)) << 4) + (kg & 1) * 8;
+            }
+            if (has_add) lds_rd64x4(pa, ad);
+#pragma unroll
+            for (int i = 0; i < 4; ++i) {
+                float v[4] = {acc[i][j][0], acc[i][j][1], acc[i][j][2], acc[i][j][3]};
+                if (bias) {
+#pragma unroll
+                    for (int r = 0; r < 4; ++r) v[r] += b4[j][r];
+                }
+                if (has_add) {
+                    v[0] += __uint_as_float(ad[i][0] << 16); v[1] += __uint_as_float(ad[i][0] & 0xffff0000u);
+                    v[2] += __uint_as_float(ad[i][1] << 16); v[3] += __uint_as_float(ad[i][1] & 0xffff0000u);
+                }
+                if (relu) {
+#pragma unroll
+                    for (int r = 0; r < 4; ++r) v[r] = fmaxf(v[r], 0.f);
+                }
+                const u32x2_t w = {f2bf2(v[0], v[1]), f2bf2(v[2], v[3])};
+                lds_wr64(pa[i], w);
+                if constexpr (STATS) { if (!second) keep[j][i] = w; }
+            }
+        }
+        wg_barrier();
+
+        {
+            const uint32_t m0 = (2u * c_begin + (uint32_t)ti) * 64u;
+            constexpr int NIT = OB_BYTES / 4096;
+            u32x4_t v[NIT];
+            static_assert(NIT == 2 || NIT == 4 || NIT == 8, "staged tile: pairs of 4 KiB read phases");
+            lds_rd128x2<0>(oO + t * 16, v[0], v[1]);
+            if constexpr (NIT >= 4) lds_rd128x2<8192>(oO + t * 16, v[2], v[3]);
+            if constexpr (NIT >= 8) { lds_rd128x2<16384>(oO + t * 16, v[4], v[5]); lds_rd128x2<24576>(oO + t * 16, v[6], v[7]); }
+#pragma unroll
+            for (int it = 0; it < NIT; ++it) {
+                const int q = it * 4096 + t * 16, r = q / RB, lg = ((q % RB) >> 4) ^ (r & SWM);
+                if (m0 + (uint32_t)r < M) __builtin_nontemporal_store(v[it], reinterpret_cast<u32x4_t*>(out + (size_t)(m0 + r) * Cout + n0 + lg * 8));
+            }
+        }
+
+        if (second) {
+            float s1[TN][4], s2[TN][4], a1[TN][4], a2[TN][4];
+#pragma unroll
+            for (int j = 0; j < TN; ++j) {
+                const int lg = wave * (BN / 32) + 2 * j + (kg >> 1);
+                float c1[4][4], c2[4][4];
+                u32x2_t kb[4];
+                uint32_t pa[4];
+#pragma unroll
+                for (int i = 0; i < 4; ++i) {
+                    const int row = i * 16 + fr;
+                    pa[i] = oO + row * RB + ((lg ^ (row & SWM)) << 4) + (kg & 1) * 8;
+                }
+                lds_rd64x4(pa, kb);
+#pragma unroll
+                for (int i = 0; i < 4; ++i) {
+                    const u32x2_t ka = keep[j][i];
+                    const float xa[4] = {__uint_as_float(ka[0] << 16), __uint_as_float(ka[0] & 0xffff0000u), __uint_as_float(ka[1] << 16), __uint_as_float(ka[1] & 0xffff0000u)};
+                    const float xb[4] = {__uint_as_float(kb[i][0] << 16), __uint_as_float(kb[i][0] & 0xffff0000u), __uint_as_float(kb[i][1] << 16), __uint_as_float(kb[i][1] & 0xffff0000u)};
+#pragma unroll
+                    for (int r = 0; r < 4; ++r) { c1[i][r] = xa[r] + xb[r]; c2[i][r] = xa[r] * xa[r] + xb[r] * xb[r]; }
+                }
+#pragma unroll
+                for (int r = 0; r < 4; ++r) {
+                    s1[j][r] = (c1[0][r] + c1[2][r]) + (c1[1][r] + c1[3][r]);
+                    s2[j][r] = (c2[0][r] + c2[2][r]) + (c2[1][r] + c2[3][r]);
+                }
+            }
+#pragma unroll
+            for (int j = 0; j < TN; ++j)
+#pragma unroll
+                for (int r = 0; r < 4; ++r) { a1[j][r] = 0.f + s1[j][r]; a2[j][r] = 0.f + s2[j][r]; }
+#pragma unroll
+            for (int k = 1; k < 16; ++k)
+#pragma unroll
+                for (int j = 0; j < TN; ++j)
+#pragma unroll
+                    for (int r = 0; r < 4; ++r) { a1[j][r] = dpp_shr1(a1[j][r]) + s1[j][r]; a2[j][r] = dpp_shr1(a2[j][r]) + s2[j][r]; }
+            if (fr == 15) {
+                const size_t chunk = (size_t)c_begin + (size_t)(ti >> 1);
+#pragma unroll
+                for (int j = 0; j < TN; ++j) {
+                    float* o = bn_part + (chunk * Cout + n0 + wave * (BN / 4) + j * 16 + kg * 4) * 2;
+                    *reinterpret_cast<float4*>(o) = make_float4(a1[j][0], a2[j][0], a1[j][1], a2[j][1]);
+                    *reinterpret_cast<float4*>(o + 4) = make_float4(a1[j][2], a2[j][2], a1[j][3], a2[j][3]);
+                }
+            }
+        }
+        if (has_add) wg_barrier();
+    }
+}
+
+static int pw_bn(int Cin, int Cout)
+{
+    if (Cin == 64) return Cout == 64 ? 64 : (Cout % 128 == 0 ? 128 : 0);
+    if (Cin == 128) return Cout % 128 == 0 ? 128 : 0;
+    if (Cin == 256) return Cout == 64 ? 64 : (Cout % 128 == 0 ? 128 : 0);
+    return 0;
+}
+static size_t pw_lds(int Cin, int bn, bool two_tiles) { return (size_t)2 * 64 * Cin * 2 + (size_t)(two_tiles ? 2 : 1) * 64 * bn * 2; }
+
+template <int CIN, int BN, bool STATS>
+static void pw_launch1(dim3 grid, size_t lds, hipStream_t st, const void* in, const void* wt, void* out, const float* bias, const void* addend,
+                      uint32_t M, int Cout, int Kpad, int relu, uint32_t nchunks, float* bn_part)
+{
+    if (lds > 65536) (void)hipFuncSetAttribute((const void*)conv1_stream_kernel<CIN, BN, STATS>, hipFuncAttributeMaxDynamicSharedMemorySize, (int)lds);
+    hipLaunchKernelGGL((conv1_stream_kernel<CIN, BN, STATS>), grid, dim3(256), lds, st, (const bf16_t*)in, (const bf16_t*)wt, (bf16_t*)out, bias, (const bf16_t*)addend,
+                       M, Cout, Kpad, relu, (uint32_t)((uint64_t)M * CIN * 2), (uint32_t)((uint64_t)M * Cout * 2), nchunks, bn_part);
+}
+
+template <int CIN, int BN>
+static void pw_launch(dim3 grid, size_t lds, hipStream_t st, const void* in, const void* wt, void* out, const float* bias, const void* addend,
+                      uint32_t M, int Cout, int Kpad, int relu, uint32_t nchunks, float* bn_part)
+{
+    if (bn_part) pw_launch1<CIN, BN, true>(grid, lds, st, in, wt, out, bias, addend, M, Cout, Kpad, relu, nchunks, bn_part);
+    else pw_launch1<CIN, BN, false>(grid, lds, st, in, wt, out, bias, addend, M, Cout, Kpad, relu, nchunks, nullptr);
+}
+
+static int pw_run(const void* in, const void* wt, void* out, const float* bias, const void* addend, uint32_t M, int Cin, int Cout, int relu,
+                  float* bn_part, int max_blocks, hipStream_t st)
+{
+    const int bn = pw_bn(Cin, Cout);
+    if (!bn) return DREG_EINVAL;
+    if (M == 0) return DREG_OK;
+    const size_t lds = pw_lds(Cin, bn, addend != nullptr);
+    const uint32_t nchunks = (M + 127) / 128;
+    const int slices = Cout / bn;
+    int per_cu = (int)(163840 / lds);
+    per_cu = per_cu > 4 ? 4 : (per_cu < 1 ? 1 : per_cu);
+    uint32_t nblk = (uint32_t)(256 * per_cu / slices);
+    if (max_blocks > 0) nblk = (uint32_t)max_blocks;
+    if (nblk > nchunks) nblk = nchunks;
+    if (nblk < 1) nblk = 1;
+    const dim3 grid(nblk, slices);
+    const int Kpad = dreg_conv3d_kpad(1, Cin, 0);
+#define PW_CASE(C, N) if (Cin == C && bn == N) pw_launch<C, N>(grid, lds, st, in, wt, out, bias, addend, M, Cout, Kpad, relu, nchunks, bn_part); else
+    PW_CASE(64, 64) PW_CASE(64, 128) PW_CASE(128, 128) PW_CASE(256, 64) PW_CASE(256, 128) return DREG_EINVAL;
+#undef PW_CASE
+    DREG_LAUNCH_CHECK();
+    return DREG_OK;
+}
+
+static bool pw_faster(long V, int Cin, int Cout)
+{
+    if (V >= 32 * 32 * 32) return true;
+    return V >= 16 * 16 * 16 && Cout == 512 && (Cin == 128 || Cin == 256);
+}
+
+extern "C" {
+
+int dreg_conv1_stream_variant(int Cin, int Cout) { return pw_bn(Cin, Cout); }
+
+int dreg_conv1_stream_supported(int B, int D, int H, int W, int Cin, int Cout, int ksz, int stride, int pad, int relu,
+                                int has_addend, int add_same, int dtype, int nrows)
+{
+    if (dtype != 0 || nrows != 0 || ksz != 1 || stride != 1 || pad != 0 || !(relu == 0 || relu == 1)) return 0;
+    if (has_addend && !add_same) return 0;
+    if (B <= 0 || D <= 0 || H <= 0 || W <= 0 || !pw_bn(Cin, Cout)) return 0;
+    const uint64_t M = (uint64_t)B * D * H * W;
+    if (M * (uint64_t)Cin * 2 >= 0x7fffff00ull || M * (uint64_t)Cout * 2 >= 0x7fffff00ull) return 0;
+    return 1;
+}
+int dreg_conv1_stream_use(int B, int D, int H, int W, int Cin, int Cout, int ksz, int stride, int pad, int relu,
+                          int has_addend, int add_same, int dtype, int nrows)
+{
+    if (!dreg_conv1_stream_supported(B, D, H, W, Cin, Cout, ksz, stride, pad, relu, has_addend, add_same, dtype, nrows)) return 0;
+    return pw_faster((long)D * H * W, Cin, Cout) ? 1 : 0;
+}
+
+int dreg_conv1_stream(const void* in, const void* wt_packed, void* out, const float* bias, const void* addend,
+                      int B, int Di, int Hi, int Wi, int Cin, int Do, int Ho, int Wo, int Cout,
+                      int ksz, int stride, int pad, int transposed, int relu, int Da, int Ha, int Wa, int add_same,
+                      int dtype, int out_f32, void* workspace, size_t workspace_bytes, void* stream, int max_blocks)
+{
+    const bool same = !addend || (add_same && Da == Do && Ha == Ho && Wa == Wo);
+    if (out_f32 || !same || Di != Do || Hi != Ho || Wi != Wo ||
+        !dreg_conv1_stream_supported(B, Do, Ho, Wo, Cin, Cout, ksz, stride, pad, relu, addend != nullptr, add_same, dtype, 0))
+        return dreg_conv3d_igemm_ws(in, wt_packed, out, bias, addend, B, Di, Hi, Wi, Cin, Do, Ho, Wo, Cout, ksz, stride, pad, transposed, relu,
+                                    Da, Ha, Wa, add_same, dtype, out_f32, workspace, workspace_bytes, stream);
+    (void)transposed;
+    return pw_run(in, wt_packed, out, bias, addend, (uint32_t)((uint64_t)B * Do * Ho * Wo), Cin, Cout, relu, nullptr, max_blocks, (hipStream_t)stream);
+}
+
+int dreg_conv1_stream_bnstats(const void* in, const void* wt_packed, void* out, const float* bias, const void* addend,
+                              int B, int Di, int Hi, int Wi, int Cin, int Do, int Ho, int Wo, int Cout,
+                              int ksz, int stride, int pad, int relu, int Da, int Ha, int Wa, int add_same,
+                              void* workspace, size_t workspace_bytes, float* bn_partial, int* rows_per_chunk, void* stream, int max_blocks)
+{
+    if (!rows_per_chunk) return DREG_EINVAL;
+    const bool same = !addend || (add_same && Da == Do && Ha == Ho && Wa == Wo);
+    if (!same || Di != Do || Hi != Ho || Wi != Wo ||
+        !dreg_conv1_stream_supported(B, Do, Ho, Wo, Cin, Cout, ksz, stride, pad, relu, addend != nullptr, add_same, 0, 0))
+        return dreg_conv3d_igemm_bnstats(in, wt_packed, out, bias, addend, B, Di, Hi, Wi, Cin, Do, Ho, Wo, Cout, ksz, stride, pad, relu,
+                                         Da, Ha, Wa, add_same, workspace, workspace_bytes, bn_partial, rows_per_chunk, stream);
+    *rows_per_chunk = 0;
+    const long V = (long)Do * Ho * Wo;
+    const bool emit = bn_partial && V % 128 == 0;
+    const int rc = pw_run(in, wt_packed, out, bias, addend, (uint32_t)((uint64_t)B * V), Cin, Cout, relu, emit ? bn_partial : nullptr, max_blocks, (hipStream_t)stream);
+    if (rc == DREG_OK && emit) *rows_per_chunk = 128;
+    return rc;
+}
+
+}
diff --git a/dreg_nerf_amd/csrc/executor.hip b/dreg_nerf_amd/csrc/executor.hip
--- a/dreg_nerf_amd/csrc/executor.hip
+++ b/dreg_nerf_amd/csrc/executor.hip
@@ -43,6 +43,7 @@
     int sstem_conv = -1, sstem_lat = -1;
     size_t xam_off = 0, pmask_off = 0;
     int halo = 0;
+    int pointwise = 0;
     int stats_bn = -1;
     size_t stats_off = 0;
     int stats_conv = -1;
@@ -155,7 +156,7 @@
 {
     std::memset(o, 0, sizeof(*o));
     o->sparse_grads = 1; o->bn_batch_tails = 1; o->fuse_stem = 1; o->sparse_stem = 1; o->fold_res_bn = 1; o->fold_splitk = 1;
-    o->group_wgrad = 1; o->s2_accumulate = 1; o->fuse_bn_stats = 1; o->brick = 1; o->defer_head_pg = 0;
+    o->group_wgrad = 1; o->s2_accumulate = 1; o->fuse_bn_stats = 1; o->brick = 1; o->defer_head_pg = 0; o->pointwise_stream = 1;
 }
 void* dreg_exec_create(const int* tensors, int nt, const int* ops, int nops, const int64_t* params, int np)
 {
@@ -456,6 +457,16 @@
             if (on(p.d0) && p.d1 % 16 == 0 && p.pk_brick_fwd == SIZE_MAX) p.pk_brick_fwd = add_brick_pack(p, 0);
             if (e->needs_grad[o.in] && on(p.d1) && p.d0 % 16 == 0 && p.pk_brick_dgrad == SIZE_MAX) p.pk_brick_dgrad = add_brick_pack(p, 1);
         }
+        if (o.kind == OP_CONV && e->opt.pointwise_stream && o.rows_out < 0 && !o.halo) {
+            const bool same = x.D == y.D && x.H == y.H && x.W == y.W;
+            const bool add_ok = o.in2 < 0 || (o.add_same && e->t[o.in2].D == y.D && e->t[o.in2].H == y.H && e->t[o.in2].W == y.W);
+            if (same && add_ok && !o.fold_sk_fwd && p.d1 == x.C &&
+                dreg_conv1_stream_use(x.B, y.D, y.H, y.W, x.C, p.d0, o.ksz, o.stride, o.pad, o.relu, o.in2 >= 0, o.add_same, 0, 0)) o.pointwise |= 1;
+            if (same && e->needs_grad[o.in] && !s2_class_ok(p, o.ksz, o.stride, o.pad)) {
+                if (!o.fold_sk_bwd && dreg_conv1_stream_use(x.B, x.D, x.H, x.W, p.d0, p.d1, o.ksz, o.stride, o.pad, 0, 0, 1, 0, 0)) o.pointwise |= 2;
+                if (dreg_conv1_stream_use(x.B, x.D, x.H, x.W, p.d0, p.d1, o.ksz, o.stride, o.pad, 0, 1, 1, 0, 0)) o.pointwise |= 4;
+            }
+        }
         if (o.halo & 1) { if (p.pk_halo_fwd == SIZE_MAX) p.pk_halo_fwd = add_halo_pack(p, 0); }
         else if (p.pk_fwd == SIZE_MAX) { p.cin_pad = x.C; p.pk_fwd = add_pack(p, 0, x.C); }
         if (e->needs_grad[o.in]) {
@@ -508,6 +519,8 @@
     return DREG_OK;
 }
 int dreg_exec_op_halo(void* h, int op) { Exec* e = (Exec*)h; return op >= 0 && op < (int)e->ops.size() ? e->ops[op].halo : 0; }
+int dreg_exec_op_wgrad_grouped(void* h, int op) { Exec* e = (Exec*)h; return op >= 0 && op < (int)e->ops.size() ? e->ops[op].grp : 0; }
+int dreg_exec_op_pointwise(void* h, int op) { Exec* e = (Exec*)h; return op >= 0 && op < (int)e->ops.size() ? e->ops[op].pointwise : 0; }
 
 void dreg_exec_set_overlap(void* h, int enable) { ((Exec*)h)->use_aux = enable != 0; }
 void dreg_exec_set_input_row_occupancy(void* h, const uint8_t* rowocc) { ((Exec*)h)->in_rowocc = rowocc; }
@@ -671,6 +684,17 @@
                                          o.add_same, 0, stream));
                 continue;
             }
+            if (o.pointwise & 1) {
+                if (train && o.stats_bn >= 0)
+                    CK(dreg_conv1_stream_bnstats(act(o.in), PK + w.pk_fwd, act(o.out), bias, add, x.B, x.D, x.H, x.W, x.C, y.D, y.H, y.W, w.d0,
+                                                 o.ksz, o.stride, o.pad, o.relu, ta ? ta->D : 0, ta ? ta->H : 0, ta ? ta->W : 0, o.add_same,
+                                                 A + e->off_ks, e->sz_ks, (float*)(A + e->ops[o.stats_bn].stats_off), &sums_rpc[o.stats_bn], stream, 0));
+                else
+                    CK(dreg_conv1_stream(act(o.in), PK + w.pk_fwd, act(o.out), bias, add, x.B, x.D, x.H, x.W, x.C, y.D, y.H, y.W, w.d0,
+                                         o.ksz, o.stride, o.pad, 0, o.relu, ta ? ta->D : 0, ta ? ta->H : 0, ta ? ta->W : 0, o.add_same, 0, 0,
+                                         A + e->off_ks, e->sz_ks, stream, 0));
+                continue;
+            }
             if (train && o.stats_bn >= 0 && !(o.in == 0 && e->in_rowocc)) {
                 CK(dreg_conv3d_igemm_bnstats(act(o.in), PK + w.pk_fwd, act(o.out), bias, add, x.B, x.D, x.H, x.W, x.C, y.D, y.H, y.W, w.d0,
                                              o.ksz, o.stride, o.pad, o.relu, ta ? ta->D : 0, ta ? ta->H : 0, ta ? ta->W : 0, o.add_same,
@@ -1010,6 +1034,10 @@
                     CK(dreg_conv3d_dgrad_s2_acc(gy, PK + w.pk_cls, gx, x.B, x.D, x.H, x.W, x.C, y.D, y.H, y.W, w.d0, o.ksz, o.pad, stream));
                 } else if (fused_add) {
                     sc.variant(1);
+                    if (o.pointwise & 4)
+                        CK(dreg_conv1_stream(gy, PK + w.pk_dgrad, gx, nullptr, gx, x.B, y.D, y.H, y.W, w.d0, x.D, x.H, x.W, w.d1,
+                                             o.ksz, o.stride, o.pad, 1, 0, x.D, x.H, x.W, 1, 0, 0, A + e->off_ks, e->sz_ks, stream, 0));
+                    else
                     CK(dreg_conv3d_igemm_ws(gy, PK + w.pk_dgrad, gx, nullptr, gx, x.B, y.D, y.H, y.W, w.d0, x.D, x.H, x.W, w.d1,
                                             o.ksz, o.stride, o.pad, 1, 0, x.D, x.H, x.W, 1, 0, 0, A + e->off_ks, e->sz_ks, stream));
                 } else if (rows) {
@@ -1037,7 +1065,10 @@
                         CK(dreg_conv3d_igemm_defer(gy, PK + w.pk_dgrad, gx, nullptr, nullptr, x.B, y.D, y.H, y.W, w.d0, x.D, x.H, x.W, w.d1,
                                                    o.ksz, o.stride, o.pad, 1, 0, 0, 0, 0, 0, A + e->off_ks, e->sz_ks, nullptr, &ns, &sl, stream));
                         if (ns > 0) { e->pend_sk_bn = i - 1; e->pend_sk_n = ns; e->pend_sk_slice = sl; }
-                    } else
+                    } else if (o.pointwise & 2)
+                        CK(dreg_conv1_stream(gy, PK + w.pk_dgrad, gx, nullptr, nullptr, x.B, y.D, y.H, y.W, w.d0, x.D, x.H, x.W, w.d1,
+                                             o.ksz, o.stride, o.pad, 1, 0, 0, 0, 0, 0, 0, 0, A + e->off_ks, e->sz_ks, stream, 0));
+                    else
                     CK(dreg_conv3d_igemm_ws(gy, PK + w.pk_dgrad, gx, nullptr, nullptr, x.B, y.D, y.H, y.W, w.d0, x.D, x.H, x.W, w.d1,
                                             o.ksz, o.stride, o.pad, 1, 0, 0, 0, 0, 0, 0, 0, A + e->off_ks, e->sz_ks, stream));
                 }
diff --git a/dreg_nerf_amd/lib.py b/dreg_nerf_amd/lib.py
--- a/dreg_nerf_amd/lib.py
+++ b/dreg_nerf_amd/lib.py
@@ -70,6 +70,11 @@
     "dreg_conv3_halo_pack_bytes_n": (Z, [I, I]),
     "dreg_conv3_halo_n": (I, [P, P, P, P, P] + [I] * 11 + [P]),
     "dreg_conv3_halo_n_bnstats": (I, [P, P, P, P, P] + [I] * 10 + [P, P, P]),
+    "dreg_conv1_stream_variant": (I, [I, I]),
+    "dreg_conv1_stream_supported": (I, [I] * 14),
+    "dreg_conv1_stream_use": (I, [I] * 14),
+    "dreg_conv1_stream": (I, [P, P, P, P, P] + [I] * 20 + [P, Z, P, I]),
+    "dreg_conv1_stream_bnstats": (I, [P, P, P, P, P] + [I] * 17 + [P, Z, P, P, P, I]),
     "dreg_conv3d_wgrad_variant": (I, [I] * 10),
     "dreg_conv3d_igemm_variant": (I, [I] * 17),
     "dreg_conv3d_wgrad_group_fill": (I, [P, P, P, P, Z] + [I] * 12 + [P, P]),
@@ -125,6 +130,8 @@
     "dreg_exec_create": (P, [P, I, P, I, P, I]),
     "dreg_exec_destroy": (None, [P]),
     "dreg_exec_op_halo": (I, [P, I]),
+    "dreg_exec_op_pointwise": (I, [P, I]),
+    "dreg_exec_op_wgrad_grouped": (I, [P, I]),
     "dreg_exec_arena_bytes": (Z, [P]),
     "dreg_exec_pack_bytes": (Z, [P]),
     "dreg_exec_num_packs": (I, [P]),
@@ -292,7 +299,7 @@
 
 class ExecOpts(ctypes.Structure):
     _fields_ = [(n, c_int) for n in ("sparse_grads", "bn_batch_tails", "fuse_stem", "sparse_stem", "fold_res_bn", "fold_splitk", "group_wgrad",
-                                     "s2_accumulate", "fuse_bn_stats", "brick", "defer_head_pg", "persistent_deep", "guard")] + [("reserved", c_int * 3)]
+                                     "s2_accumulate", "fuse_bn_stats", "brick", "defer_head_pg", "persistent_deep", "guard", "pointwise_stream")] + [("reserved", c_int * 2)]
 
 
 def load_probe():
diff --git a/dreg_nerf_amd/trunk_exec.py b/dreg_nerf_amd/trunk_exec.py
--- a/dreg_nerf_amd/trunk_exec.py
+++ b/dreg_nerf_amd/trunk_exec.py
@@ -195,6 +195,13 @@
                 fname = "conv3_halo64_kernel<bf16>" if cout == 64 else "conv3_halo_kernel<bf16>"
             if halo & 2:
                 dname = "conv3_halo64_kernel<bf16>" if x[4] == 64 else "conv3_halo_kernel<bf16>"
+            pw = self.lib.dreg_exec_op_pointwise(self.h, i)
+            if pw & 1:
+                fname = f"conv1_stream_kernel<{x[4]},{lib.dreg_conv1_stream_variant(x[4], cout)}>"
+            if pw & 2:
+                dname = f"conv1_stream_kernel<{cout},{lib.dreg_conv1_stream_variant(cout, x[4])}>"
+            if pw & 4:
+                dname_add = f"conv1_stream_kernel<{cout},{lib.dreg_conv1_stream_variant(cout, x[4])}>"
             rows = "-rows" if is_rows else ""
             fl = 2.0 * M * cout * k ** 3 * cin
             per_row = 2.0 * cout * k ** 3 * cin
@@ -204,6 +211,8 @@
             def wgrad_name(nr, B=B, x=x, y=y, cout=cout, k=k, is_rows=is_rows, first=int(o[1] == 0)):
                 return ops.wgrad_kernel_name(lib, B, y[1], y[2], y[3], x[4], cout, k, is_rows, nr, first)
             wname = wgrad_name if is_rows else wgrad_name(0)
+            if not is_rows and self.lib.dreg_exec_op_wgrad_grouped(self.h, i):
+                wname = wname + "+grouped"
             out[(i, 2)] = (wname, f"wgrad{rows} B{B} {x[1]}x{x[2]}x{x[3]}x{x[4]} g{y[1]}x{y[2]}x{y[3]}x{cout} k{k}s{s}", fl, lo, per_row, None, None)
         out[(-1, 3)] = ("wgrad_reduce_batched_kernel", "split sums of a backward range -> torch-layout gradients", 0.0, -1, 0.0, None, None)
         out[(-1, 4)] = ("bn_tail_batched_kernel<0>", "running statistics of the small BatchNorms of a forward pass", 0.0, -1, 0.0, None, None)
diff --git a/include/dreg_nerf.h b/include/dreg_nerf.h
--- a/include/dreg_nerf.h
+++ b/include/dreg_nerf.h
@@ -54,6 +54,20 @@
                       int B, int D, int H, int W, int Cin, int Cout, int Da, int Ha, int Wa, int add_same, int out_f32, void* stream);
 int dreg_conv3_halo_n_bnstats(const void* in, const void* wpk, void* out, const float* bias, const void* addend,
                               int B, int D, int H, int W, int Cin, int Cout, int Da, int Ha, int Wa, int add_same, float* bn_partial, int* rows_per_chunk, void* stream);
+
+int dreg_conv1_stream_variant(int Cin, int Cout);
+int dreg_conv1_stream_supported(int B, int D, int H, int W, int Cin, int Cout, int ksz, int stride, int pad, int relu,
+                                int has_addend, int add_same, int dtype, int nrows);
+int dreg_conv1_stream_use(int B, int D, int H, int W, int Cin, int Cout, int ksz, int stride, int pad, int relu,
+                          int has_addend, int add_same, int dtype, int nrows);
+int dreg_conv1_stream(const void* in, const void* wt_packed, void* out, const float* bias, const void* addend,
+                      int B, int Di, int Hi, int Wi, int Cin, int Do, int Ho, int Wo, int Cout,
+                      int ksz, int stride, int pad, int transposed, int relu, int Da, int Ha, int Wa, int add_same,
+                      int dtype, int out_f32, void* workspace, size_t workspace_bytes, void* stream, int max_blocks);
+int dreg_conv1_stream_bnstats(const void* in, const void* wt_packed, void* out, const float* bias, const void* addend,
+                              int B, int Di, int Hi, int Wi, int Cin, int Do, int Ho, int Wo, int Cout,
+                              int ksz, int stride, int pad, int relu, int Da, int Ha, int Wa, int add_same,
+                              void* workspace, size_t workspace_bytes, float* bn_partial, int* rows_per_chunk, void* stream, int max_blocks);
 
 int dreg_conv3d_dgrad_s2(const void* gout, const void* wt_class_packed, void* din, int B, int Di, int Hi, int Wi, int Cin,
                          int Do, int Ho, int Wo, int Cout, int ksz, int pad, void* stream);
@@ -220,7 +234,8 @@
     int defer_head_pg;
     int persistent_deep;
     int guard;
-    int reserved[3];
+    int pointwise_stream;
+    int reserved[2];
 } dreg_exec_opts;
 void dreg_exec_default_opts(dreg_exec_opts* o);
 void* dreg_exec_create_opts(const int* tensors, int nt, const int* ops, int nops, const int64_t* params, int np, const dreg_exec_opts* opts);
@@ -239,6 +254,8 @@
 int dreg_exec_export_pack_table(void* h, void* host_out, int* host_row_desc, void* pack_base);
 int dreg_exec_repack(void* h, const void* descs_dev, const int* row_desc_dev, void* stream);
 int dreg_exec_op_halo(void* h, int op);
+int dreg_exec_op_wgrad_grouped(void* h, int op);
+int dreg_exec_op_pointwise(void* h, int op);
 void dreg_exec_set_overlap(void* h, int enable);
 void dreg_exec_set_input_row_occupancy(void* h, const uint8_t* rowocc);
 void dreg_exec_set_timing(void* h, int enable);
```
